# Orion-AI-Lab/KuroSiwo

Hardware: AMD Instinct MI355X
Metric: SAR tiles/sec (224x224, SNUNet-ECAM change-detection train step) (higher is better)
Workload: dtype bf16; 1 GPU; BASELINE.json configs[1]: SNUNet-ECAM CD, 2 dates x 2-ch GRD 224x224, per-GPU batch 32, ce+dice loss, Adam lr 1e-3, fwd+loss+bwd+optimizer; global_batch=32, base_channel=32, parallelism=dp1, hip_streams=3

## Files before the change

include/ksmi.h:

```cpp
#ifndef KSMI_H
#define KSMI_H
#include <stddef.h>
#include <stdint.h>

#ifdef __cplusplus
extern "C" {
#endif

#define KSMI_ABI_VERSION 8
#define KSMI_F32 0
#define KSMI_BF16 1
#define KSMI_E_ARG (-1)
#define KSMI_E_UNSUPPORTED (-2)
#define KSMI_MAX_SRC 6
#define KSMI_MAX_CHUNKS 72

int ksmi_abi_version(void);
const char* ksmi_last_error(void);
int ksmi_set_knob(const char* name, const char* value);
int ksmi_chunk_elems(int dtype);

#define KSMI_OP_CALL 0
#define KSMI_OP_ORDER 1
#define KSMI_OP_WAIT_SIDE 2
// ... 80 lines not shown
  int64_t sK, sN, sD, sT;
  int32_t flip;
  int32_t k_off[KSMI_MAX_CHUNKS];
  int32_t k_len[KSMI_MAX_CHUNKS];
  int32_t use_tap_map;
  int32_t tap_map[16];
  int32_t uniform_kc, k_total;
} ksmi_pack_desc;
int ksmi_pack_weights(const ksmi_pack_desc* d, int dtype, void* stream);
int ksmi_pack_weights_batched(const ksmi_pack_desc* descs_device, int n, int dtype, void* stream);

typedef struct ksmi_wgrad_desc {
  ksmi_src src[KSMI_MAX_SRC];
  int32_t nsrc;
  const void* dy; int32_t dyC; int32_t dy_c_off;
  int32_t B, Hin, Win, Hout, Wout;
  int32_t KH, KW, stride, pad;
  int32_t TH, TW;
  int32_t N;
  int32_t nchunks;
  int32_t nsplit;
  float* partial;
  float* grad; int64_t gK, gN, gT; int32_t accumulate;
  int32_t k_off[KSMI_MAX_CHUNKS];
  int32_t k_len[KSMI_MAX_CHUNKS];
  uint16_t chunk_c0[KSMI_MAX_CHUNKS];
  uint8_t chunk_src[KSMI_MAX_CHUNKS];
  int32_t uniform_kc, k_total;
  int32_t in_sy, in_sx, in_oy, in_ox, in_H, in_W;
  int32_t pad_x_set, pad_x;
  int32_t use_tap_off;
  int32_t tap_off[16];
  float* bias_grad; int32_t bias_accumulate;
} ksmi_wgrad_desc;
size_t ksmi_conv_wgrad_workspace(const ksmi_wgrad_desc* d, int dtype);
int ksmi_conv_wgrad(const ksmi_wgrad_desc* d, int dtype, void* stream);
int ksmi_conv_wgrad_fuses_bias(const ksmi_wgrad_desc* d, int dtype);

int ksmi_conv_first_forward(const float* x_nchw, const float* w, const float* bias, void* out, float* stats,
                            int B, int Cin, int H, int W, int Cout, int dtype, void* stream);
int ksmi_conv_first_forward_raw(const float* x_nchw, const float* x_tail, int c_head, const float* w, const float* bias,
                                void* out, float* stats, int B, int Cin, int H, int W, int Cout, const float* mean,
                                const float* stdv, const float* clamp, int dtype, void* stream);
int ksmi_conv_first_stats_rows(int B, int H, int W);
int ksmi_im2col3x3(const float* x_nchw, void* out, int B, int Cin, int H, int W, int Kpad, int dtype, void* stream);
int ksmi_im2col3x3_raw(const float* x_nchw, const float* x_tail, int c_head, void* out, int B, int Cin, int H, int W,
                       int Kpad, const float* mean, const float* stdv, const float* clamp, int dtype, void* stream);
int ksmi_conv_first_wgrad(const float* x_nchw, const void* dy, float* dw, float* workspace, size_t ws_bytes,
                          int B, int Cin, int H, int W, int Cout, int accumulate, int dtype, void* stream);
size_t ksmi_conv_first_wgrad_workspace(int B, int Cin, int H, int W, int Cout);

int ksmi_bn_finalize(const float* partial, int rows, int Cpad, int C, double count,
                     const float* gamma, const float* beta, float* running_mean, float* running_var,
                     int64_t* num_batches_tracked, float momentum, float eps, int training,
                     float* mean, float* rstd, float* scale, float* shift, void* stream);
int ksmi_bn_add_relu(const void* z, const void* identity, const float* scale, const float* shift, void* out,
                     int64_t npix, int C, int dtype, void* stream);
int ksmi_bnrelu_bwd_reduce(const void* dout, const void* out, const void* z, const float* mean, const float* rstd,
                           float* partial, int rows, int64_t npix, int C, int dtype, void* stream);
int ksmi_reduce_rows(const float* partial, int rows, int K, int Cstride, int C, float* sums,
                     float* dgamma, float* dbeta, int accumulate, void* stream);
typedef struct ksmi_rowsum_desc {
  const float* partial;
  float* dst;
  int32_t rows, K, k, Cstride, C, accumulate;
  int32_t head, next;
} ksmi_rowsum_desc;
int ksmi_reduce_rows_batched(const ksmi_rowsum_desc* descs_device, int n, void* stream);
int ksmi_reduce_rows_batched_wide(const ksmi_rowsum_desc* descs_device, int n, int max_c, void* stream);
int ksmi_bnrelu_bwd_apply(void* dout_g, const void* out, const void* z, const float* mean, const float* rstd,
                          const float* gamma, const float* sums, void* dz, double count,
                          int64_t npix, int C, int dtype, void* stream);
int ksmi_bn_bwd_apply_gated(const void* g, const void* z, const float* mean, const float* rstd, const float* gamma, const float* sums,
                            void* dz, double count, int64_t npix, int C, int dtype, void* stream);
int ksmi_bn_bwd_apply_add(void* r_di, const void* g, const void* i, const float* mean, const float* rstd,
                          const float* gamma, const float* sums, float* partial, int rows, double count,
                          int64_t npix, int C, int dtype, void* stream);
int ksmi_bn_fused_supported(int C, int Cstride, int dtype);
int ksmi_bn_fused_max_rows(void);
int ksmi_bn_fin_add_relu(float* partial, int rows, int Cpad, int C, double count, const float* gamma, const float* beta,
                         float* running_mean, float* running_var, int64_t* num_batches_tracked, float momentum, float eps,
                         float* mean, float* rstd, float* scale, float* shift, const void* z, const void* identity, void* out,
                         void* pooled, int B, int H, int W, int dtype, void* stream);
int ksmi_bn_bwd_fin_apply_gated(float* partial, int rows, int Cstride, float* sums, float* dgamma, float* dbeta, int accumulate,
                                const void* g, const void* z, const float* mean, const float* rstd, const float* gamma, void* dz,
                                double count, int64_t npix, int C, int dtype, void* stream);
int ksmi_bnrelu_bwd_fin_apply(float* partial, int rows, int Cstride, float* sums, float* dgamma, float* dbeta, int accumulate,
                              void* dout_g, const void* out, const void* z, const float* mean, const float* rstd, const float* gamma,
                              void* dz, double count, int64_t npix, int C, int dtype, void* stream);
int ksmi_bn_bwd_fin_apply_add(float* partial, int rows, int Cstride, float* sums, float* dgamma, float* dbeta, int accumulate,
                              void* r_di, const void* g, const void* i, const float* mean, const float* rstd, const float* gamma,
                              float* bias_partial, int bias_rows, double count, int64_t npix, int C, int dtype, void* stream);
int ksmi_channel_sum(const void* x, float* partial, int rows, int64_t npix, int C, int dtype, void* stream);
int ksmi_colsum(const void* x, int64_t rows, int C, float* out, int accumulate, int dtype, void* stream);

int ksmi_maxpool2x2_forward(const void* x, void* y, int B, int H, int W, int C, int dtype, void* stream);
int ksmi_maxpool2x2_backward(const void* x, const void* dy, void* dx, int accumulate,
                             int B, int H, int W, int C, int dtype, void* stream);

int ksmi_ecam_pool(const void* const x[4], float* avg, float* mx, int32_t* argmax,
                   float* workspace, int B, int HW, int C, int dtype, void* stream);
size_t ksmi_ecam_pool_workspace(int B, int HW, int C);
int ksmi_ecam_mlp(const float* avg, const float* mx, const float* ca_fc1, const float* ca_fc2,
                  const float* ca1_fc1, const float* ca1_fc2, float* ca, float* ca1,
                  float* hidden , int B, int C, void* stream);
int ksmi_ecam_final_forward(const void* const x[4], const float* ca, const float* ca1, const float* wf,
                            const float* bias, float* logits, int B, int HW, int C, int ncls, int dtype, void* stream);
int ksmi_ecam_final_backward_reduce(const void* const x[4], const float* dlogits, const float* ca, const float* ca1,
                                    const float* wf, float* dca, float* dca1, float* dwf, float* dbias,
                                    float* workspace, int B, int HW, int C, int ncls, int dtype, void* stream);
size_t ksmi_ecam_bwd_workspace(int B, int HW, int C, int ncls);
int ksmi_ecam_mlp_backward(const float* avg, const float* mx, const float* hidden, const float* ca, const float* ca1,
                           const float* dca, const float* dca1, const float* ca_fc1, const float* ca_fc2,
                           const float* ca1_fc1, const float* ca1_fc2, float* davg, float* dmax,
                           float* g_ca_fc1, float* g_ca_fc2, float* g_ca1_fc1, float* g_ca1_fc2,
                           float* workspace, int B, int C, void* stream);
size_t ksmi_ecam_mlp_bwd_workspace(int B, int C);
int ksmi_ecam_final_backward_dx(void* const dx[4], const float* dlogits, const float* ca, const float* wf,
                                const float* davg, const float* dmax, const int32_t* argmax,
                                int B, int HW, int C, int ncls, int dtype, void* stream);

size_t ksmi_loss_workspace(int B, int HW);
int ksmi_ce_dice_forward(const float* logits, const int64_t* labels, const float* class_w, int with_dice,
                         float* out3, float* workspace, int B, int HW, int ignore_index, void* stream);
int ksmi_ce_dice_backward(const float* logits, const int64_t* labels, const float* class_w, int with_dice,
                          const float* workspace, const float* grad_scale ,
                          float* dlogits, int B, int HW, int ignore_index, void* stream);

#define KSMI_LOSS_DICE 1
#define KSMI_LOSS_LOVASZ 2
#define KSMI_LOSS_FOCAL 3
size_t ksmi_seg_loss_workspace(int kind, int B, int HW);
int ksmi_seg_loss_forward(int kind, const float* logits, const int64_t* labels, const float* class_w, float gamma, float* out3,
                          void* workspace, int B, int HW, int ignore_index, void* stream);
int ksmi_seg_loss_backward(int kind, const float* logits, const int64_t* labels, const float* class_w, float gamma,
                           const void* workspace, const float* grad_scale ,
                           float* dlogits, int B, int HW, int ignore_index, void* stream);

int ksmi_argmax_confusion(const float* logits, const int64_t* labels, int64_t* pred , int64_t* cm,
                          int B, int C, int HW, int ignore_index, void* stream);
int ksmi_argmax_confusion_grouped(const float* logits, const int64_t* labels, int64_t* pred , int64_t* cm ,
                                  const int32_t* slot_a, int64_t* cms_a, const int32_t* slot_b, int64_t* cms_b,
                                  int B, int C, int HW, int ignore_index, void* stream);

int ksmi_adam_step(float* p, const float* g, float* m, float* v, int64_t n, int64_t* step_count,
                   float lr, float beta1, float beta2, float eps, float weight_decay, float grad_scale, void* stream);
int ksmi_adamw_step(float* p, const float* g, float* m, float* v, int64_t n, int64_t* step_count,
                    float lr, float beta1, float beta2, float eps, float weight_decay, float grad_scale, void* stream);
int ksmi_adam_step_mirror(float* p, const float* g, float* m, float* v, int64_t n, int64_t* step_count,
                          float lr, float beta1, float beta2, float eps, float weight_decay, float grad_scale, int decoupled,
                          void* mirror_bf16, void* stream);
int ksmi_sgd_step(float* p, const float* g, float* mom, int64_t n, int64_t* step_count,
                  float lr, float momentum, float weight_decay, float grad_scale, void* stream);

int ksmi_layernorm_forward(const void* x, const float* gamma, const float* beta, void* y, float* mean, float* rstd,
                           int rows, int C, float eps, int dtype, void* stream);
int ksmi_layernorm_bwd_blocks(int rows);
int ksmi_layernorm_backward(const void* dy, const void* x, const float* mean, const float* rstd, const float* gamma,
                            void* dx, int accumulate, float* partial, int rows, int C, int dtype, void* stream);
int ksmi_gelu_forward(const void* x, void* y, int64_t n, int dtype, void* stream);
int ksmi_gelu_backward(const void* dy, const void* x, void* dx, int64_t n, int dtype, void* stream);
int ksmi_gelu_backward_drop(const void* dy, const void* x, void* dx, int64_t n, uint32_t thr, float inv_keep, uint32_t site,
                            const uint32_t* rng_state, int dtype, void* stream);
int ksmi_add(const void* a, const void* b, void* out, int64_t n, int dtype, void* stream);
int ksmi_relu_backward(const void* dy, const void* x, void* dx, int64_t n, int dtype, void* stream);
int ksmi_relu_forward(const void* x, void* y, int64_t n, int dtype, void* stream);
// ... 146 lines not shown
```

kurosiwo_amd/_lib.py:

```python
import ctypes as C
import os

_HERE = os.path.dirname(os.path.abspath(__file__))
LIB_PATH = os.path.join(_HERE, "libksmi.so")

KSMI_F32, KSMI_BF16 = 0, 1
LOSS_DICE, LOSS_LOVASZ, LOSS_FOCAL = 1, 2, 3
MAX_SRC, MAX_CHUNKS = 6, 72
ABI_VERSION = 8


class KsmiError(RuntimeError):
    pass


class Src(C.Structure):
    _fields_ = [("ptr", C.c_void_p), ("scale", C.c_void_p), ("shift", C.c_void_p),
                ("C", C.c_int32), ("c_off", C.c_int32), ("c_len", C.c_int32), ("relu", C.c_int32)]


class Dst(C.Structure):
    _fields_ = [("ptr", C.c_void_p), ("C", C.c_int32), ("c_off", C.c_int32), ("n_begin", C.c_int32),
                ("n_len", C.c_int32), ("accumulate", C.c_int32), ("pad_", C.c_int32)]

# ... 22 lines not shown
                ("nchunks", C.c_int32), ("taps", C.c_int32), ("N", C.c_int32), ("Npad", C.c_int32), ("n_mod", C.c_int32),
                ("sK", C.c_int64), ("sN", C.c_int64), ("sD", C.c_int64), ("sT", C.c_int64),
                ("flip", C.c_int32),
                ("k_off", C.c_int32 * MAX_CHUNKS), ("k_len", C.c_int32 * MAX_CHUNKS),
                ("use_tap_map", C.c_int32), ("tap_map", C.c_int32 * 16), ("uniform_kc", C.c_int32), ("k_total", C.c_int32)]


class TiffInfo(C.Structure):
    _fields_ = [(k, C.c_int32) for k in ("width", "height", "bands", "bits", "sample_format", "compression", "predictor", "tiled",
                                         "big_endian", "bigtiff", "has_geo", "has_nodata")] + [
        ("pixel_scale", C.c_double * 2), ("origin", C.c_double * 2), ("tie_pixel", C.c_double * 2), ("nodata", C.c_double)]


class RowsumDesc(C.Structure):
    _fields_ = [("partial", C.c_void_p), ("dst", C.c_void_p), ("rows", C.c_int32), ("K", C.c_int32), ("k", C.c_int32),
                ("Cstride", C.c_int32), ("C", C.c_int32), ("accumulate", C.c_int32), ("head", C.c_int32), ("next", C.c_int32)]


class WgradDesc(C.Structure):
    _fields_ = [("src", Src * MAX_SRC), ("nsrc", C.c_int32),
                ("dy", C.c_void_p), ("dyC", C.c_int32), ("dy_c_off", C.c_int32),
                ("B", C.c_int32), ("Hin", C.c_int32), ("Win", C.c_int32), ("Hout", C.c_int32), ("Wout", C.c_int32),
                ("KH", C.c_int32), ("KW", C.c_int32), ("stride", C.c_int32), ("pad", C.c_int32),
                ("TH", C.c_int32), ("TW", C.c_int32), ("N", C.c_int32), ("nchunks", C.c_int32), ("nsplit", C.c_int32),
                ("partial", C.c_void_p), ("grad", C.c_void_p),
                ("gK", C.c_int64), ("gN", C.c_int64), ("gT", C.c_int64), ("accumulate", C.c_int32),
                ("k_off", C.c_int32 * MAX_CHUNKS), ("k_len", C.c_int32 * MAX_CHUNKS),
                ("chunk_c0", C.c_uint16 * MAX_CHUNKS), ("chunk_src", C.c_uint8 * MAX_CHUNKS),
                ("uniform_kc", C.c_int32), ("k_total", C.c_int32),
                ("in_sy", C.c_int32), ("in_sx", C.c_int32), ("in_oy", C.c_int32), ("in_ox", C.c_int32), ("in_H", C.c_int32), ("in_W", C.c_int32),
                ("pad_x_set", C.c_int32), ("pad_x", C.c_int32), ("use_tap_off", C.c_int32), ("tap_off", C.c_int32 * 16),
                ("bias_grad", C.c_void_p), ("bias_accumulate", C.c_int32)]


class Op(C.Structure):
    _fields_ = [(k, C.c_int32) for k in ("kind", "sig", "lane", "side", "tag", "a", "b", "nargs")] + [("fn", C.c_void_p), ("args", C.c_void_p)]


OP_CALL, OP_ORDER, OP_WAIT_SIDE = 0, 1, 2

_vp, _i, _i64, _f, _d, _sz = C.c_void_p, C.c_int, C.c_int64, C.c_float, C.c_double, C.c_size_t
_P4 = C.c_void_p * 4

SIGNATURES = {
    "ksmi_abi_version": (_i, []),
    "ksmi_last_kernels": (_i, [C.c_char_p, _i]),
    "ksmi_hbm_probe": (_i, [_i, _vp, _vp, _vp, C.c_size_t, _vp, _vp]),
    "ksmi_last_error": (C.c_char_p, []),
    "ksmi_set_knob": (_i, [C.c_char_p, C.c_char_p]),
    "ksmi_thunk_id": (_i, [C.c_char_p]),
    "ksmi_runner_create": (_vp, []),
    "ksmi_runner_destroy": (_i, [_vp]),
    "ksmi_runner_set_streams": (_i, [_vp, _vp, _vp, _vp, _vp]),
    "ksmi_run_list": (_i, [_vp, _vp, _i, _i, _vp, C.POINTER(C.c_int32)]),
    "ksmi_runner_order": (_i, [_vp, _i, _i]),
    "ksmi_runner_fork_side": (_i, [_vp, _i, _i, C.POINTER(C.c_void_p)]),
    "ksmi_runner_mark_side": (_i, [_vp, _i, _i]),
    "ksmi_runner_wait_side": (_i, [_vp, _i, _i, _i]),
    "ksmi_runner_join": (_i, [_vp]),
    "ksmi_conv_dispatch_info": (_i, [C.POINTER(ConvDesc), _i, C.POINTER(C.c_int32)]),
    "ksmi_chunk_elems": (_i, [_i]),
    "ksmi_conv_grid_m": (_i, [C.POINTER(ConvDesc)]),
    "ksmi_conv_forward": (_i, [C.POINTER(ConvDesc), _i, _vp]),
    "ksmi_pack_weights": (_i, [C.POINTER(PackDesc), _i, _vp]),
    "ksmi_pack_weights_batched": (_i, [_vp, _i, _i, _vp]),
    "ksmi_conv_wgrad_workspace": (_sz, [C.POINTER(WgradDesc), _i]),
    "ksmi_conv_wgrad": (_i, [C.POINTER(WgradDesc), _i, _vp]),
    "ksmi_conv_wgrad_fuses_bias": (_i, [C.POINTER(WgradDesc), _i]),
    "ksmi_conv_stats_rows": (_i, [C.POINTER(ConvDesc), _i]),
    "ksmi_conv_gate_supported": (_i, [C.POINTER(ConvDesc), _i]),
    "ksmi_desc_size": (C.c_size_t, [_i]),
    "ksmi_conv_first_forward": (_i, [_vp, _vp, _vp, _vp, _vp, _i, _i, _i, _i, _i, _i, _vp]),
    "ksmi_conv_first_forward_raw": (_i, [_vp, _vp, _i, _vp, _vp, _vp, _vp, _i, _i, _i, _i, _i, _vp, _vp, _vp, _i, _vp]),
    "ksmi_conv_first_stats_rows": (_i, [_i, _i, _i]),
    "ksmi_im2col3x3": (_i, [_vp, _vp, _i, _i, _i, _i, _i, _i, _vp]),
    "ksmi_im2col3x3_raw": (_i, [_vp, _vp, _i, _vp, _i, _i, _i, _i, _i, _vp, _vp, _vp, _i, _vp]),
    "ksmi_conv_first_wgrad": (_i, [_vp, _vp, _vp, _vp, _sz, _i, _i, _i, _i, _i, _i, _i, _vp]),
    "ksmi_conv_first_wgrad_workspace": (_sz, [_i, _i, _i, _i, _i]),
    "ksmi_bn_finalize": (_i, [_vp, _i, _i, _i, _d, _vp, _vp, _vp, _vp, _vp, _f, _f, _i, _vp, _vp, _vp, _vp, _vp]),
    "ksmi_bn_add_relu": (_i, [_vp, _vp, _vp, _vp, _vp, _i64, _i, _i, _vp]),
    "ksmi_bn_fused_supported": (_i, [_i, _i, _i]),
    "ksmi_bn_fused_max_rows": (_i, []),
    "ksmi_bn_fin_add_relu": (_i, [_vp, _i, _i, _i, _d, _vp, _vp, _vp, _vp, _vp, _f, _f, _vp, _vp, _vp, _vp, _vp, _vp, _vp, _vp, _i, _i, _i, _i, _vp]),
    "ksmi_bn_bwd_fin_apply_gated": (_i, [_vp, _i, _i, _vp, _vp, _vp, _i, _vp, _vp, _vp, _vp, _vp, _vp, _d, _i64, _i, _i, _vp]),
    "ksmi_bnrelu_bwd_fin_apply": (_i, [_vp, _i, _i, _vp, _vp, _vp, _i, _vp, _vp, _vp, _vp, _vp, _vp, _vp, _d, _i64, _i, _i, _vp]),
    "ksmi_bn_bwd_fin_apply_add": (_i, [_vp, _i, _i, _vp, _vp, _vp, _i, _vp, _vp, _vp, _vp, _vp, _vp, _vp, _i, _d, _i64, _i, _i, _vp]),
    "ksmi_bnrelu_bwd_reduce": (_i, [_vp, _vp, _vp, _vp, _vp, _vp, _i, _i64, _i, _i, _vp]),
    "ksmi_reduce_rows": (_i, [_vp, _i, _i, _i, _i, _vp, _vp, _vp, _i, _vp]),
    "ksmi_reduce_rows_batched": (_i, [_vp, _i, _vp]),
    "ksmi_reduce_rows_batched_wide": (_i, [_vp, _i, _i, _vp]),
    "ksmi_bnrelu_bwd_apply": (_i, [_vp, _vp, _vp, _vp, _vp, _vp, _vp, _vp, _d, _i64, _i, _i, _vp]),
    "ksmi_bn_bwd_apply_gated": (_i, [_vp, _vp, _vp, _vp, _vp, _vp, _vp, _d, _i64, _i, _i, _vp]),
    "ksmi_bn_bwd_apply_add": (_i, [_vp, _vp, _vp, _vp, _vp, _vp, _vp, _vp, _i, _d, _i64, _i, _i, _vp]),
    "ksmi_channel_sum": (_i, [_vp, _vp, _i, _i64, _i, _i, _vp]),
    "ksmi_colsum": (_i, [_vp, _i64, _i, _vp, _i, _i, _vp]),
    "ksmi_gather_rows": (_i, [_vp, _vp, _i, _vp, _vp, _i, _i, _i, _i, _i, _i, _vp]),
    "ksmi_scatter_rows": (_i, [_vp, _vp, _vp, _i, _vp, _vp, _i, _i, _i, _i, _i, _vp]),
    "ksmi_batch_sum": (_i, [_vp, _vp, _i, _i64, _i, _i, _vp]),
    "ksmi_mse_workspace": (C.c_size_t, []),
    "ksmi_mse_loss": (_i, [_vp, _vp, _vp, _f, _vp, _vp, _vp, _i64, _i, _vp]),
    "ksmi_maxpool2x2_forward": (_i, [_vp, _vp, _i, _i, _i, _i, _i, _vp]),
    "ksmi_maxpool2x2_backward": (_i, [_vp, _vp, _vp, _i, _i, _i, _i, _i, _i, _vp]),
    "ksmi_ecam_pool": (_i, [_P4, _vp, _vp, _vp, _vp, _i, _i, _i, _i, _vp]),
    "ksmi_ecam_pool_workspace": (_sz, [_i, _i, _i]),
    "ksmi_ecam_mlp": (_i, [_vp, _vp, _vp, _vp, _vp, _vp, _vp, _vp, _vp, _i, _i, _vp]),
    "ksmi_ecam_final_forward": (_i, [_P4, _vp, _vp, _vp, _vp, _vp, _i, _i, _i, _i, _i, _vp]),
    "ksmi_ecam_final_backward_reduce": (_i, [_P4, _vp, _vp, _vp, _vp, _vp, _vp, _vp, _vp, _vp, _i, _i, _i, _i, _i, _vp]),
    "ksmi_ecam_bwd_workspace": (_sz, [_i, _i, _i, _i]),
    "ksmi_ecam_mlp_backward": (_i, [_vp] * 18 + [_i, _i, _vp]),
    "ksmi_ecam_mlp_bwd_workspace": (_sz, [_i, _i]),
    "ksmi_ecam_final_backward_dx": (_i, [_P4, _vp, _vp, _vp, _vp, _vp, _vp, _i, _i, _i, _i, _i, _vp]),
    "ksmi_loss_workspace": (_sz, [_i, _i]),
    "ksmi_ce_dice_forward": (_i, [_vp, _vp, _vp, _i, _vp, _vp, _i, _i, _i, _vp]),
    "ksmi_ce_dice_backward": (_i, [_vp, _vp, _vp, _i, _vp, _vp, _vp, _i, _i, _i, _vp]),
    "ksmi_seg_loss_workspace": (_sz, [_i, _i, _i]),
    "ksmi_seg_loss_forward": (_i, [_i, _vp, _vp, _vp, _f, _vp, _vp, _i, _i, _i, _vp]),
    "ksmi_seg_loss_backward": (_i, [_i, _vp, _vp, _vp, _f, _vp, _vp, _vp, _i, _i, _i, _vp]),
    "ksmi_argmax_confusion": (_i, [_vp, _vp, _vp, _vp, _i, _i, _i, _i, _vp]),
    "ksmi_argmax_confusion_grouped": (_i, [_vp, _vp, _vp, _vp, _vp, _vp, _vp, _vp, _i, _i, _i, _i, _vp]),
    "ksmi_adam_step": (_i, [_vp, _vp, _vp, _vp, _i64, _vp, _f, _f, _f, _f, _f, _f, _vp]),
    "ksmi_adamw_step": (_i, [_vp, _vp, _vp, _vp, _i64, _vp, _f, _f, _f, _f, _f, _f, _vp]),
    "ksmi_adam_step_mirror": (_i, [_vp, _vp, _vp, _vp, _i64, _vp, _f, _f, _f, _f, _f, _f, _i, _vp, _vp]),
    "ksmi_sgd_step": (_i, [_vp, _vp, _vp, _i64, _vp, _f, _f, _f, _f, _vp]),
    "ksmi_layernorm_forward": (_i, [_vp, _vp, _vp, _vp, _vp, _vp, _i, _i, _f, _i, _vp]),
    "ksmi_layernorm_bwd_blocks": (_i, [_i]),
    "ksmi_layernorm_backward": (_i, [_vp, _vp, _vp, _vp, _vp, _vp, _i, _vp, _i, _i, _i, _vp]),
    "ksmi_gelu_forward": (_i, [_vp, _vp, _i64, _i, _vp]),
    "ksmi_gelu_backward": (_i, [_vp, _vp, _vp, _i64, _i, _vp]),
    "ksmi_add": (_i, [_vp, _vp, _vp, _i64, _i, _vp]),
    "ksmi_relu_backward": (_i, [_vp, _vp, _vp, _i64, _i, _vp]),
    "ksmi_relu_forward": (_i, [_vp, _vp, _i64, _i, _vp]),
    "ksmi_sar_preprocess": (_i, [_vp, _vp, _vp, _vp, _i, _i, _i64, C.c_float, _vp]),
    "ksmi_augment_views": (_i, [_vp, _vp, _vp, _vp, _vp, _vp, _i, _i, _i, _i, _f, C.c_uint32, _f, _f, C.c_uint32, _f, _f, C.c_uint32, _i, _i, _i, _i, _vp, _vp]),
    "ksmi_augment_masks": (_i, [_vp, _vp, _vp, _vp, _vp, _i, _i, _i, _i, _vp]),
    "ksmi_dem_slope": (_i, [_vp, _vp, _i, _i, _i, _d, _f, _f, _i, _vp]),
    "ksmi_bmm_f32": (_i, [_vp, _vp, _vp, _vp, _i, _i, _i, _i, _i, C.POINTER(C.c_int64), C.POINTER(C.c_int64), C.POINTER(C.c_int64), C.c_float, _i, _vp]),
    "ksmi_softmax_rows_f32": (_i, [_vp, _vp, _i64, _i, C.c_float, _vp]),
    "ksmi_softmax_rows_backward_f32": (_i, [_vp, _vp, _vp, _i64, _i, C.c_float, _vp]),
    "ksmi_semantic_tokens_forward": (_i, [_vp, _vp, _vp, _vp, _vp, _i, _i, _i, _i, _i, _i, _vp]),
    "ksmi_semantic_tokens_backward": (_i, [_vp, _vp, _vp, _vp, _vp, _vp, _i, _i, _i, _i, _i, _i, _i, _vp]),
    "ksmi_token_cross_forward": (_i, [_vp, _vp, _vp, _vp, _vp, _vp, _vp, _i, _i, _i, _i, _i, _i, C.c_float, _i, _vp]),
    "ksmi_token_cross_bwd_workspace": (_sz, [_i, _i, _i]),
    "ksmi_token_cross_backward": (_i, [_vp, _vp, _vp, _vp, _vp, _vp, _vp, _vp, _vp, _vp, _vp, _i, _i, _vp, _i, _i, _i, _i, _i, _i, C.c_float, _i, _vp]),
    "ksmi_tiff_info_read": (_i, [C.c_char_p, C.POINTER(TiffInfo)]),
    "ksmi_tiff_read_f32": (_i, [C.c_char_p, _vp, _i64, C.POINTER(TiffInfo)]),
    "ksmi_tiff_read_native": (_i, [C.c_char_p, _vp, _i64, C.POINTER(TiffInfo)]),
    "ksmi_tile_batch_read": (_i, [C.POINTER(C.c_char_p), _i, _vp, _i, _i, _i]),
    "ksmi_tile_batch_read_bands": (_i, [C.POINTER(C.c_char_p), _i, _vp, _i, _i, _i, _i]),
    "ksmi_tiles_fill_nodata": (_i, [_vp, _i, _i, _i, _i]),
    "ksmi_cast_bf16": (_i, [_vp, _vp, _i64, _vp]),
    "ksmi_up_gemm_supported": (_i, [_i, _i, _i, _i, _i]),
    "ksmi_up_wgrad_supported": (_i, [_i, _i, _i, _i, _i]),
    "ksmi_up_pack_weight": (_i, [_vp, _vp, _i, _vp]),
    "ksmi_up_pack_weights_batched": (_i, [_vp, _vp, _vp, _i, _vp]),
    "ksmi_up_forward": (_i, [_vp, _vp, _vp, _vp, _i, _i, _i, _i, _vp]),
    "ksmi_up_dgrad": (_i, [_vp, _vp, _vp, _i, _i, _i, _i, _i, _vp]),
    "ksmi_up_wgrad_workspace": (C.c_size_t, [_i, _i, _i, _i]),
    "ksmi_up_wgrad": (_i, [_vp, _vp, _vp, _vp, _i, _i, _i, _i, _i, _vp]),
    "ksmi_gemm_nt": (_i, [_vp, _i, _vp, _i, _vp, _vp, _i, _vp, _i, _i, _i, _i, _vp]),
    "ksmi_gemm_nn": (_i, [_vp, _i, _vp, _i, _vp, _i, _i, _i, _i, _i, _vp]),
    "ksmi_im2col": (_i, [_vp, _vp] + [_i] * 11 + [_i, _i, _vp]),
    "ksmi_col2im": (_i, [_vp, _vp, _i] + [_i] * 11 + [_i, _vp]),
    "ksmi_im2col_tc": (_i, [_vp, _vp] + [_i] * 11 + [_i, _vp]),
    "ksmi_col2im_tc": (_i, [_vp, _vp, _i] + [_i] * 11 + [_i, _vp]),
    "ksmi_weight_to_tc": (_i, [_vp, _vp, _i, _i, _i, _i, _i, _vp]),
    "ksmi_grad_from_tc": (_i, [_vp, _vp, _i, _i, _i, _i, _i, _vp]),
# ... 108 lines not shown
```

kurosiwo_amd/csrc/bnfused.hip:

```cpp
#include <stdlib.h>
#include "common.h"
#include "../../include/ksmi.h"
#include "errors.h"

int ksmi_internal_fold_rows(float* partial, int rows, int K, int Cstride, int C, hipStream_t st);

namespace {

constexpr int kFat = 1024;
constexpr int kMaxC = 512;
constexpr int kMaxRows = 512;

__device__ __forceinline__ void block_rows_sum(const float* __restrict__ partial, int rows, int Cstride, int C, double* red, double* sums) {
  const int Cq = C >> 2, G = Cq * 2;
  const int lpc = kFat / G;
  const int t = threadIdx.x;
  const int g = t % G, rl = t / G;
  if (rl < lpc) {
    const int k = g / Cq, c4 = g - k * Cq;
    const float* p = partial + (size_t)k * Cstride + c4 * 4;
    double a0 = 0.0, a1 = 0.0, a2 = 0.0, a3 = 0.0;
#pragma unroll 4
    for (int r = rl; r < rows; r += lpc) {
      const f32x4 v = *(const f32x4*)(p + (size_t)r * 2 * Cstride);
// ... 20 lines not shown
  float* mean_o; float* rstd_o; float* scale_o; float* shift_o;
};

template <typename T, bool POOL>
__global__ __launch_bounds__(kFat) void bn_fin_add_relu_kernel(FinArgs f, const T* __restrict__ z, const T* __restrict__ idn, T* __restrict__ out,
                                                               T* __restrict__ pooled, int B, int H, int W) {
  constexpr int VEC = ElemTraits<T>::kVec;
  __shared__ double red[kFat * 4];
  __shared__ double sums[2 * kMaxC];
  __shared__ float s_scale[kMaxC], s_shift[kMaxC];
  const int C = f.C;
  block_rows_sum(f.partial, f.rows, f.Cstride, C, red, sums);
  for (int c = threadIdx.x; c < C; c += kFat) {
    const double mean = sums[c] / f.count;
    double var = sums[C + c] / f.count - mean * mean;
    if (var < 0.0) var = 0.0;
    const float rs = (float)(1.0 / sqrt(var + (double)f.eps));
    const float sc = f.gamma[c] * rs;
    const float sh = f.beta[c] - (float)mean * sc;
    s_scale[c] = sc; s_shift[c] = sh;
    if (blockIdx.x == 0) {
      f.mean_o[c] = (float)mean; f.rstd_o[c] = rs; f.scale_o[c] = sc; f.shift_o[c] = sh;
      const double unb = f.count > 1.0 ? var * f.count / (f.count - 1.0) : var;
      f.rmean[c] = (1.f - f.momentum) * f.rmean[c] + f.momentum * (float)mean;
      f.rvar[c] = (1.f - f.momentum) * f.rvar[c] + f.momentum * (float)unb;
    }
  }
  if (blockIdx.x == 0 && threadIdx.x == 0 && f.nbt) *f.nbt += 1;
  __syncthreads();
  const int CV = C / VEC;
  const int64_t stride = (int64_t)gridDim.x * kFat;
  if (!POOL) {
    const int64_t nvec = (int64_t)B * H * W * CV;
    for (int64_t v = (int64_t)blockIdx.x * kFat + threadIdx.x; v < nvec; v += 2 * stride) {
      const int64_t v1 = v + stride;
      const bool two = v1 < nvec;
      const u32x4 rz0 = *(const u32x4*)(z + v * VEC), ri0 = *(const u32x4*)(idn + v * VEC);
      const u32x4 rz1 = *(const u32x4*)(z + (two ? v1 : v) * VEC), ri1 = *(const u32x4*)(idn + (two ? v1 : v) * VEC);
      float a[VEC], b[VEC];
      int c = (int)(v % CV) * VEC;
      vec_unpack<T>(rz0, a); vec_unpack<T>(ri0, b);
#pragma unroll
      for (int j = 0; j < VEC; ++j) a[j] = fmaxf(a[j] * s_scale[c + j] + s_shift[c + j] + b[j], 0.f);
      *(u32x4*)(out + v * VEC) = vec_pack<T>(a);
      if (two) {
        c = (int)(v1 % CV) * VEC;
        vec_unpack<T>(rz1, a); vec_unpack<T>(ri1, b);
#pragma unroll
        for (int j = 0; j < VEC; ++j) a[j] = fmaxf(a[j] * s_scale[c + j] + s_shift[c + j] + b[j], 0.f);
        *(u32x4*)(out + v1 * VEC) = vec_pack<T>(a);
      }
    }
  } else {
    const int Ho = H / 2, Wo = W / 2;
    const int64_t n = (int64_t)B * Ho * Wo * CV;
    for (int64_t v = (int64_t)blockIdx.x * kFat + threadIdx.x; v < n; v += stride) {
      const int cv = (int)(v % CV); int64_t r = v / CV;
      const int ox = (int)(r % Wo); r /= Wo;
      const int oy = (int)(r % Ho); const int b = (int)(r / Ho);
      const int64_t base = (((int64_t)b * H + 2 * oy) * W + 2 * ox) * C + cv * VEC;
      const int64_t offs[4] = {base, base + C, base + (int64_t)W * C, base + (int64_t)W * C + C};
      u32x4 rz[4], ri[4];
#pragma unroll
      for (int q = 0; q < 4; ++q) { rz[q] = *(const u32x4*)(z + offs[q]); ri[q] = *(const u32x4*)(idn + offs[q]); }
      const int c = cv * VEC;
      float m[VEC];
#pragma unroll
      for (int q = 0; q < 4; ++q) {
        float a[VEC], bb[VEC];
        vec_unpack<T>(rz[q], a); vec_unpack<T>(ri[q], bb);
#pragma unroll
        for (int j = 0; j < VEC; ++j) a[j] = fmaxf(a[j] * s_scale[c + j] + s_shift[c + j] + bb[j], 0.f);
        const u32x4 pk = vec_pack<T>(a);
        *(u32x4*)(out + offs[q]) = pk;
        vec_unpack<T>(pk, a);
#pragma unroll
        for (int j = 0; j < VEC; ++j) m[j] = (q == 0 || a[j] > m[j]) ? a[j] : m[j];
      }
      *(u32x4*)(pooled + v * VEC) = vec_pack<T>(m);
    }
  }
}

struct BwdFinArgs {
  const float* partial; int rows, Cstride, C;
  float* sums_o; float* dgamma; float* dbeta; int accumulate;
  const float* mean; const float* rstd; const float* gamma;
};

__device__ __forceinline__ void bwd_finish(const BwdFinArgs& f, double* red, double* sums, float* s_sum, float* s_mean, float* s_rstd, float* s_gamma) {
  const int C = f.C;
  block_rows_sum(f.partial, f.rows, f.Cstride, C, red, sums);
  for (int v = threadIdx.x; v < 2 * C; v += kFat) {
    const float s = (float)sums[v];
    s_sum[v] = s;
    if (blockIdx.x == 0) {
      if (f.sums_o) f.sums_o[v] = s;
      const int k = v / C, c = v - k * C;
      float* tgt = k == 0 ? f.dbeta : f.dgamma;
      if (tgt) tgt[c] = f.accumulate ? tgt[c] + 1.f * s : 1.f * s;
    }
  }
  for (int c = threadIdx.x; c < C; c += kFat) { s_mean[c] = f.mean[c]; s_rstd[c] = f.rstd[c]; s_gamma[c] = f.gamma[c]; }
  __syncthreads();
}

template <typename T, int MODE>
__global__ __launch_bounds__(kFat) void bn_bwd_fin_apply_kernel(BwdFinArgs f, T* __restrict__ g, const T* __restrict__ outp, const T* __restrict__ z,
                                                                T* __restrict__ dz, float inv_n, int64_t nvec) {
  constexpr int VEC = ElemTraits<T>::kVec;
  __shared__ double red[kFat * 4];
  __shared__ double sums[2 * kMaxC];
  __shared__ float s_sum[2 * kMaxC], s_mean[kMaxC], s_rstd[kMaxC], s_gamma[kMaxC];
  bwd_finish(f, red, sums, s_sum, s_mean, s_rstd, s_gamma);
  const int C = f.C, CV = C / VEC;
  const int64_t stride = (int64_t)gridDim.x * kFat;
  for (int64_t v = (int64_t)blockIdx.x * kFat + threadIdx.x; v < nvec; v += 2 * stride) {
    const int64_t v1 = v + stride;
    const bool two = v1 < nvec;
    const int64_t w1 = two ? v1 : v;
    const u32x4 rg0 = *(const u32x4*)(g + v * VEC), rz0 = *(const u32x4*)(z + v * VEC);
    const u32x4 rg1 = *(const u32x4*)(g + w1 * VEC), rz1 = *(const u32x4*)(z + w1 * VEC);
    u32x4 ro0, ro1;
    if (MODE == 1) { ro0 = *(const u32x4*)(outp + v * VEC); ro1 = *(const u32x4*)(outp + w1 * VEC); }
#pragma unroll
    for (int u = 0; u < 2; ++u) {
      if (u == 1 && !two) break;
      const int64_t vv = u ? v1 : v;
      const int c = (int)(vv % CV) * VEC;
      float gg[VEC], zz[VEC], o[VEC];
      vec_unpack<T>(u ? rg1 : rg0, gg); vec_unpack<T>(u ? rz1 : rz0, zz);
      if (MODE == 1) vec_unpack<T>(u ? ro1 : ro0, o);
#pragma unroll
      for (int j = 0; j < VEC; ++j) {
        if (MODE == 1) gg[j] = o[j] > 0.f ? gg[j] : 0.f;
        const float zh = (zz[j] - s_mean[c + j]) * s_rstd[c + j];
        zz[j] = s_gamma[c + j] * s_rstd[c + j] * (gg[j] - s_sum[c + j] * inv_n - zh * s_sum[C + c + j] * inv_n);
      }
      if (MODE == 1) *(u32x4*)(g + vv * VEC) = vec_pack<T>(gg);
      *(u32x4*)(dz + vv * VEC) = vec_pack<T>(zz);
    }
  }
}

template <typename T>
__global__ __launch_bounds__(kFat) void bn_bwd_fin_apply_add_kernel(BwdFinArgs f, T* __restrict__ r, const T* __restrict__ g, const T* __restrict__ iv,
                                                                    float* __restrict__ bias_partial, float inv_n, int64_t npix) {
  constexpr int VEC = ElemTraits<T>::kVec;
  __shared__ double red[kFat * 4];
  __shared__ double sums[2 * kMaxC];
  __shared__ float s_sum[2 * kMaxC], s_mean[kMaxC], s_rstd[kMaxC], s_gamma[kMaxC];
  bwd_finish(f, red, sums, s_sum, s_mean, s_rstd, s_gamma);
  const int C = f.C, CV = C / VEC;
  const int npl = kFat / CV;
  const int cv = threadIdx.x % CV, pl = threadIdx.x / CV;
  const bool active = pl < npl;
  float acc[VEC];
#pragma unroll
  for (int j = 0; j < VEC; ++j) acc[j] = 0.f;
  if (active) {
    float mu[VEC], rs[VEC], k0[VEC], k1[VEC], gr[VEC];
#pragma unroll
    for (int j = 0; j < VEC; ++j) {
      const int c = cv * VEC + j;
      mu[j] = s_mean[c]; rs[j] = s_rstd[c]; gr[j] = s_gamma[c] * s_rstd[c];
      k0[j] = s_sum[c] * inv_n; k1[j] = s_sum[C + c] * inv_n;
    }
    const int64_t per = (npix + gridDim.x - 1) / gridDim.x;
    const int64_t p0 = per * blockIdx.x, p1 = p0 + per < npix ? p0 + per : npix;
    for (int64_t p = p0 + pl; p < p1; p += 2 * npl) {
      const bool two = p + npl < p1;
      const int64_t offs[2] = {p * C + cv * VEC, two ? (p + npl) * C + cv * VEC : p * C + cv * VEC};
      u32x4 raw[2][3];
#pragma unroll
      for (int u = 0; u < 2; ++u) {
        raw[u][0] = *(const u32x4*)(r + offs[u]); raw[u][1] = *(const u32x4*)(g + offs[u]); raw[u][2] = *(const u32x4*)(iv + offs[u]);
      }
#pragma unroll
      for (int u = 0; u < 2; ++u) {
        if (u == 1 && !two) break;
        float rr[VEC], gg[VEC], ii[VEC];
        vec_unpack<T>(raw[u][0], rr); vec_unpack<T>(raw[u][1], gg); vec_unpack<T>(raw[u][2], ii);
#pragma unroll
        for (int j = 0; j < VEC; ++j) {
          const float xh = (ii[j] - mu[j]) * rs[j];
          rr[j] = gg[j] + gr[j] * (rr[j] - k0[j] - xh * k1[j]);
        }
        const u32x4 pk = vec_pack<T>(rr);
        *(u32x4*)(r + offs[u]) = pk;
        vec_unpack<T>(pk, rr);
#pragma unroll
        for (int j = 0; j < VEC; ++j) acc[j] += rr[j];
      }
    }
  }
  float* fred = (float*)red;
  __syncthreads();
#pragma unroll
  for (int j = 0; j < VEC; ++j) fred[(size_t)threadIdx.x * VEC + j] = active ? acc[j] : 0.f;
  __syncthreads();
  for (int c = threadIdx.x; c < C; c += kFat) {
    const int cvv = c / VEC, j = c - cvv * VEC;
    float s = 0.f;
    for (int l = 0; l < npl; ++l) s += fred[((size_t)l * CV + cvv) * VEC + j];
    bias_partial[(size_t)blockIdx.x * C + c] = s;
  }
}

bool fused_ok(int C, int dtype, int Cstride) {
  if (dtype != KSMI_BF16 && dtype != KSMI_F32) return false;
  const int vec = dtype == KSMI_BF16 ? 8 : 4;
  return C >= vec && C % vec == 0 && C % 4 == 0 && C <= kMaxC && Cstride >= C && Cstride % 4 == 0 && C / vec <= 256;
}

int fat_grid(int64_t work_items) {
  static const int cap = ksmi_knob_int("KSMI_BN_FAT_GRID", 256);
  int64_t b = (work_items + kFat - 1) / kFat;
  return (int)(b < 1 ? 1 : (b > cap ? cap : b));
}

}

extern "C" {

int ksmi_bn_fused_supported(int C, int Cstride, int dtype) { return fused_ok(C, dtype, Cstride) ? 1 : 0; }
int ksmi_bn_fused_max_rows(void) { return 256; }

int ksmi_bn_fin_add_relu(float* partial, int rows, int Cpad, int C, double count, const float* gamma, const float* beta,
                         float* running_mean, float* running_var, int64_t* num_batches_tracked, float momentum, float eps,
                         float* mean, float* rstd, float* scale, float* shift, const void* z, const void* identity, void* out,
                         void* pooled, int B, int H, int W, int dtype, void* stream) {
  if (!fused_ok(C, dtype, Cpad) || !partial || rows < 1 || B < 1 || H < 1 || W < 1) return ksmi_fail(KSMI_E_ARG, "bn_fin_add_relu: bad args");
  if (pooled && ((H & 1) || (W & 1))) return ksmi_fail(KSMI_E_ARG, "bn_fin_add_relu: pooling needs even H, W");
  if (rows > kMaxRows) rows = ksmi_internal_fold_rows(partial, rows, 2, Cpad, C, (hipStream_t)stream);
  FinArgs f{partial, rows, Cpad, C, count, gamma, beta, running_mean, running_var, num_batches_tracked, momentum, eps, mean, rstd, scale, shift};
  const int vec = dtype == KSMI_BF16 ? 8 : 4;
  const int64_t items = pooled ? (int64_t)B * (H / 2) * (W / 2) * (C / vec) : ((int64_t)B * H * W * (C / vec) + 1) / 2;
  const dim3 grid(fat_grid(items));
#define KSMI_FAR(TT, PP) hipLaunchKernelGGL((bn_fin_add_relu_kernel<TT, PP>), grid, dim3(kFat), 0, (hipStream_t)stream, f, (const TT*)z, \
                                            (const TT*)identity, (TT*)out, (TT*)pooled, B, H, W)
  if (dtype == KSMI_BF16) { if (pooled) KSMI_FAR(bf16_t, true); else KSMI_FAR(bf16_t, false); }
  else { if (pooled) KSMI_FAR(float, true); else KSMI_FAR(float, false); }
#undef KSMI_FAR
  return ksmi_check_launch("bn_fin_add_relu");
}

static int bwd_apply(int mode, float* partial, int rows, int Cstride, float* sums, float* dgamma, float* dbeta, int accumulate,
                     void* g, const void* outp, const void* z, const float* mean, const float* rstd, const float* gamma, void* dz,
                     double count, int64_t npix, int C, int dtype, void* stream, const char* what) {
  if (!fused_ok(C, dtype, Cstride) || !partial || rows < 1 || npix < 1) return ksmi_fail(KSMI_E_ARG, what);
  if (rows > kMaxRows) rows = ksmi_internal_fold_rows(partial, rows, 2, Cstride, C, (hipStream_t)stream);
  BwdFinArgs f{partial, rows, Cstride, C, sums, dgamma, dbeta, accumulate, mean, rstd, gamma};
  const int vec = dtype == KSMI_BF16 ? 8 : 4;
  const int64_t nvec = npix * C / vec;
  const float inv_n = (float)(1.0 / count);
  const dim3 grid(fat_grid((nvec + 1) / 2));
#define KSMI_BFA(TT, MM) hipLaunchKernelGGL((bn_bwd_fin_apply_kernel<TT, MM>), grid, dim3(kFat), 0, (hipStream_t)stream, f, (TT*)g, \
                                            (const TT*)outp, (const TT*)z, (TT*)dz, inv_n, nvec)
  if (dtype == KSMI_BF16) { if (mode) KSMI_BFA(bf16_t, 1); else KSMI_BFA(bf16_t, 0); }
  else { if (mode) KSMI_BFA(float, 1); else KSMI_BFA(float, 0); }
#undef KSMI_BFA
  return ksmi_check_launch(what);
}

int ksmi_bn_bwd_fin_apply_gated(float* partial, int rows, int Cstride, float* sums, float* dgamma, float* dbeta, int accumulate,
                                const void* g, const void* z, const float* mean, const float* rstd, const float* gamma, void* dz,
                                double count, int64_t npix, int C, int dtype, void* stream) {
  return bwd_apply(0, partial, rows, Cstride, sums, dgamma, dbeta, accumulate, (void*)g, nullptr, z, mean, rstd, gamma, dz, count, npix, C,
                   dtype, stream, "bn_bwd_fin_apply_gated");
}

int ksmi_bnrelu_bwd_fin_apply(float* partial, int rows, int Cstride, float* sums, float* dgamma, float* dbeta, int accumulate,
                              void* dout_g, const void* out, const void* z, const float* mean, const float* rstd, const float* gamma,
                              void* dz, double count, int64_t npix, int C, int dtype, void* stream) {
  return bwd_apply(1, partial, rows, Cstride, sums, dgamma, dbeta, accumulate, dout_g, out, z, mean, rstd, gamma, dz, count, npix, C, dtype,
                   stream, "bnrelu_bwd_fin_apply");
}

int ksmi_bn_bwd_fin_apply_add(float* partial, int rows, int Cstride, float* sums, float* dgamma, float* dbeta, int accumulate,
                              void* r_di, const void* g, const void* i, const float* mean, const float* rstd, const float* gamma,
                              float* bias_partial, int bias_rows, double count, int64_t npix, int C, int dtype, void* stream) {
  if (!fused_ok(C, dtype, Cstride) || !partial || rows < 1 || npix < 1 || bias_rows < 1 || bias_rows > 256 || !bias_partial)
    return ksmi_fail(KSMI_E_ARG, "bn_bwd_fin_apply_add: bad args");
  if (rows > kMaxRows) rows = ksmi_internal_fold_rows(partial, rows, 2, Cstride, C, (hipStream_t)stream);
  BwdFinArgs f{partial, rows, Cstride, C, sums, dgamma, dbeta, accumulate, mean, rstd, gamma};
  const float inv_n = (float)(1.0 / count);
  if (dtype == KSMI_BF16)
    hipLaunchKernelGGL(bn_bwd_fin_apply_add_kernel<bf16_t>, dim3(bias_rows), dim3(kFat), 0, (hipStream_t)stream, f, (bf16_t*)r_di,
                       (const bf16_t*)g, (const bf16_t*)i, bias_partial, inv_n, npix);
  else
    hipLaunchKernelGGL(bn_bwd_fin_apply_add_kernel<float>, dim3(bias_rows), dim3(kFat), 0, (hipStream_t)stream, f, (float*)r_di,
                       (const float*)g, (const float*)i, bias_partial, inv_n, npix);
  return ksmi_check_launch("bn_bwd_fin_apply_add");
}

}
```

kurosiwo_amd/csrc/thunks_gen.h:

```cpp
#pragma once
#include <stddef.h>
#include <stdint.h>
#include <string.h>

typedef int (*ksmi_thunk_fn)(const void* fn, const uint64_t* a, void* stream);
static inline float ksmi_slot_f32(uint64_t v) { uint32_t w = (uint32_t)v; float f; memcpy(&f, &w, 4); return f; }
static inline double ksmi_slot_f64(uint64_t v) { double d; memcpy(&d, &v, 8); return d; }

static int ksmi_thunk_0(const void* fn, const uint64_t* a, void* st) {
  typedef int (*F)(int, void*, void*, void*, float, void*, void*, int, int, int, void*);
  (void)a; return ((F)fn)((int)(int64_t)a[0], (void*)(uintptr_t)a[1], (void*)(uintptr_t)a[2], (void*)(uintptr_t)a[3], ksmi_slot_f32(a[4]), (void*)(uintptr_t)a[5], (void*)(uintptr_t)a[6], (int)(int64_t)a[7], (int)(int64_t)a[8], (int)(int64_t)a[9], st);
}
static int ksmi_thunk_1(const void* fn, const uint64_t* a, void* st) {
  typedef int (*F)(int, void*, void*, void*, float, void*, void*, void*, int, int, int, void*);
  (void)a; return ((F)fn)((int)(int64_t)a[0], (void*)(uintptr_t)a[1], (void*)(uintptr_t)a[2], (void*)(uintptr_t)a[3], ksmi_slot_f32(a[4]), (void*)(uintptr_t)a[5], (void*)(uintptr_t)a[6], (void*)(uintptr_t)a[7], (int)(int64_t)a[8], (int)(int64_t)a[9], (int)(int64_t)a[10], st);
}
static int ksmi_thunk_2(const void* fn, const uint64_t* a, void* st) {
  typedef int (*F)(int, void*, void*, void*, size_t, void*, void*);
  (void)a; return ((F)fn)((int)(int64_t)a[0], (void*)(uintptr_t)a[1], (void*)(uintptr_t)a[2], (void*)(uintptr_t)a[3], (size_t)a[4], (void*)(uintptr_t)a[5], st);
}
static int ksmi_thunk_3(const void* fn, const uint64_t* a, void* st) {
  typedef int (*F)(void*, void*);
  (void)a; return ((F)fn)((void*)(uintptr_t)a[0], st);
}
static int ksmi_thunk_4(const void* fn, const uint64_t* a, void* st) {
  typedef int (*F)(void*, int, void*);
  (void)a; return ((F)fn)((void*)(uintptr_t)a[0], (int)(int64_t)a[1], st);
}
static int ksmi_thunk_5(const void* fn, const uint64_t* a, void* st) {
  typedef int (*F)(void*, int, int, void*);
  (void)a; return ((F)fn)((void*)(uintptr_t)a[0], (int)(int64_t)a[1], (int)(int64_t)a[2], st);
}
static int ksmi_thunk_6(const void* fn, const uint64_t* a, void* st) {
  typedef int (*F)(void*, int, int, int, double, void*, void*, void*, void*, void*, float, float, int, void*, void*, void*, void*, void*);
  (void)a; return ((F)fn)((void*)(uintptr_t)a[0], (int)(int64_t)a[1], (int)(int64_t)a[2], (int)(int64_t)a[3], ksmi_slot_f64(a[4]), (void*)(uintptr_t)a[5], (void*)(uintptr_t)a[6], (void*)(uintptr_t)a[7], (void*)(uintptr_t)a[8], (void*)(uintptr_t)a[9], ksmi_slot_f32(a[10]), ksmi_slot_f32(a[11]), (int)(int64_t)a[12], (void*)(uintptr_t)a[13], (void*)(uintptr_t)a[14], (void*)(uintptr_t)a[15], (void*)(uintptr_t)a[16], st);
}
static int ksmi_thunk_7(const void* fn, const uint64_t* a, void* st) {
  typedef int (*F)(void*, int, int, int, double, void*, void*, void*, void*, void*, float, float, void*, void*, void*, void*, void*, void*, void*, void*, int, int, int, int, void*);
  (void)a; return ((F)fn)((void*)(uintptr_t)a[0], (int)(int64_t)a[1], (int)(int64_t)a[2], (int)(int64_t)a[3], ksmi_slot_f64(a[4]), (void*)(uintptr_t)a[5], (void*)(uintptr_t)a[6], (void*)(uintptr_t)a[7], (void*)(uintptr_t)a[8], (void*)(uintptr_t)a[9], ksmi_slot_f32(a[10]), ksmi_slot_f32(a[11]), (void*)(uintptr_t)a[12], (void*)(uintptr_t)a[13], (void*)(uintptr_t)a[14], (void*)(uintptr_t)a[15], (void*)(uintptr_t)a[16], (void*)(uintptr_t)a[17], (void*)(uintptr_t)a[18], (void*)(uintptr_t)a[19], (int)(int64_t)a[20], (int)(int64_t)a[21], (int)(int64_t)a[22], (int)(int64_t)a[23], st);
}
static int ksmi_thunk_8(const void* fn, const uint64_t* a, void* st) {
  typedef int (*F)(void*, int, int, int, int, void*, void*, void*, int, void*);
  (void)a; return ((F)fn)((void*)(uintptr_t)a[0], (int)(int64_t)a[1], (int)(int64_t)a[2], (int)(int64_t)a[3], (int)(int64_t)a[4], (void*)(uintptr_t)a[5], (void*)(uintptr_t)a[6], (void*)(uintptr_t)a[7], (int)(int64_t)a[8], st);
}
static int ksmi_thunk_9(const void* fn, const uint64_t* a, void* st) {
  typedef int (*F)(void*, int, int, int, int, void*, void*, void*, int, float, void*);
  (void)a; return ((F)fn)((void*)(uintptr_t)a[0], (int)(int64_t)a[1], (int)(int64_t)a[2], (int)(int64_t)a[3], (int)(int64_t)a[4], (void*)(uintptr_t)a[5], (void*)(uintptr_t)a[6], (void*)(uintptr_t)a[7], (int)(int64_t)a[8], ksmi_slot_f32(a[9]), st);
}
static int ksmi_thunk_10(const void* fn, const uint64_t* a, void* st) {
  typedef int (*F)(void*, int, int, void*, void*, void*, int, void*, void*, void*, void*, void*, void*, double, long long, int, int, void*);
  (void)a; return ((F)fn)((void*)(uintptr_t)a[0], (int)(int64_t)a[1], (int)(int64_t)a[2], (void*)(uintptr_t)a[3], (void*)(uintptr_t)a[4], (void*)(uintptr_t)a[5], (int)(int64_t)a[6], (void*)(uintptr_t)a[7], (void*)(uintptr_t)a[8], (void*)(uintptr_t)a[9], (void*)(uintptr_t)a[10], (void*)(uintptr_t)a[11], (void*)(uintptr_t)a[12], ksmi_slot_f64(a[13]), (long long)a[14], (int)(int64_t)a[15], (int)(int64_t)a[16], st);
}
static int ksmi_thunk_11(const void* fn, const uint64_t* a, void* st) {
  typedef int (*F)(void*, int, int, void*, void*, void*, int, void*, void*, void*, void*, void*, void*, void*, double, long long, int, int, void*);
  (void)a; return ((F)fn)((void*)(uintptr_t)a[0], (int)(int64_t)a[1], (int)(int64_t)a[2], (void*)(uintptr_t)a[3], (void*)(uintptr_t)a[4], (void*)(uintptr_t)a[5], (int)(int64_t)a[6], (void*)(uintptr_t)a[7], (void*)(uintptr_t)a[8], (void*)(uintptr_t)a[9], (void*)(uintptr_t)a[10], (void*)(uintptr_t)a[11], (void*)(uintptr_t)a[12], (void*)(uintptr_t)a[13], ksmi_slot_f64(a[14]), (long long)a[15], (int)(int64_t)a[16], (int)(int64_t)a[17], st);
}
static int ksmi_thunk_12(const void* fn, const uint64_t* a, void* st) {
  typedef int (*F)(void*, int, int, void*, void*, void*, int, void*, void*, void*, void*, void*, void*, void*, int, double, long long, int, int, void*);
  (void)a; return ((F)fn)((void*)(uintptr_t)a[0], (int)(int64_t)a[1], (int)(int64_t)a[2], (void*)(uintptr_t)a[3], (void*)(uintptr_t)a[4], (void*)(uintptr_t)a[5], (int)(int64_t)a[6], (void*)(uintptr_t)a[7], (void*)(uintptr_t)a[8], (void*)(uintptr_t)a[9], (void*)(uintptr_t)a[10], (void*)(uintptr_t)a[11], (void*)(uintptr_t)a[12], (void*)(uintptr_t)a[13], (int)(int64_t)a[14], ksmi_slot_f64(a[15]), (long long)a[16], (int)(int64_t)a[17], (int)(int64_t)a[18], st);
}
static int ksmi_thunk_13(const void* fn, const uint64_t* a, void* st) {
  typedef int (*F)(void*, int, void*, int, void*, int, int, int, int, int, void*);
  (void)a; return ((F)fn)((void*)(uintptr_t)a[0], (int)(int64_t)a[1], (void*)(uintptr_t)a[2], (int)(int64_t)a[3], (void*)(uintptr_t)a[4], (int)(int64_t)a[5], (int)(int64_t)a[6], (int)(int64_t)a[7], (int)(int64_t)a[8], (int)(int64_t)a[9], st);
}
static int ksmi_thunk_14(const void* fn, const uint64_t* a, void* st) {
  typedef int (*F)(void*, int, void*, int, void*, void*, int, void*, int, int, int, int, void*);
  (void)a; return ((F)fn)((void*)(uintptr_t)a[0], (int)(int64_t)a[1], (void*)(uintptr_t)a[2], (int)(int64_t)a[3], (void*)(uintptr_t)a[4], (void*)(uintptr_t)a[5], (int)(int64_t)a[6], (void*)(uintptr_t)a[7], (int)(int64_t)a[8], (int)(int64_t)a[9], (int)(int64_t)a[10], (int)(int64_t)a[11], st);
}
static int ksmi_thunk_15(const void* fn, const uint64_t* a, void* st) {
  typedef int (*F)(void*, long long, int, void*, int, int, void*);
  (void)a; return ((F)fn)((void*)(uintptr_t)a[0], (long long)a[1], (int)(int64_t)a[2], (void*)(uintptr_t)a[3], (int)(int64_t)a[4], (int)(int64_t)a[5], st);
}
static int ksmi_thunk_16(const void* fn, const uint64_t* a, void* st) {
  typedef int (*F)(void*, void*, void*);
  (void)a; return ((F)fn)((void*)(uintptr_t)a[0], (void*)(uintptr_t)a[1], st);
}
static int ksmi_thunk_17(const void* fn, const uint64_t* a, void* st) {
  typedef int (*F)(void*, void*, int, void*);
  (void)a; return ((F)fn)((void*)(uintptr_t)a[0], (void*)(uintptr_t)a[1], (int)(int64_t)a[2], st);
}
static int ksmi_thunk_18(const void* fn, const uint64_t* a, void* st) {
  typedef int (*F)(void*, void*, int, int, int, double, float, float, int, void*);
  (void)a; return ((F)fn)((void*)(uintptr_t)a[0], (void*)(uintptr_t)a[1], (int)(int64_t)a[2], (int)(int64_t)a[3], (int)(int64_t)a[4], ksmi_slot_f64(a[5]), ksmi_slot_f32(a[6]), ksmi_slot_f32(a[7]), (int)(int64_t)a[8], st);
}
static int ksmi_thunk_19(const void* fn, const uint64_t* a, void* st) {
  typedef int (*F)(void*, void*, int, int, int, int, void*);
  (void)a; return ((F)fn)((void*)(uintptr_t)a[0], (void*)(uintptr_t)a[1], (int)(int64_t)a[2], (int)(int64_t)a[3], (int)(int64_t)a[4], (int)(int64_t)a[5], st);
}
static int ksmi_thunk_20(const void* fn, const uint64_t* a, void* st) {
  typedef int (*F)(void*, void*, int, int, int, int, int, void*);
  (void)a; return ((F)fn)((void*)(uintptr_t)a[0], (void*)(uintptr_t)a[1], (int)(int64_t)a[2], (int)(int64_t)a[3], (int)(int64_t)a[4], (int)(int64_t)a[5], (int)(int64_t)a[6], st);
}
static int ksmi_thunk_21(const void* fn, const uint64_t* a, void* st) {
  typedef int (*F)(void*, void*, int, int, int, int, int, int, void*);
  (void)a; return ((F)fn)((void*)(uintptr_t)a[0], (void*)(uintptr_t)a[1], (int)(int64_t)a[2], (int)(int64_t)a[3], (int)(int64_t)a[4], (int)(int64_t)a[5], (int)(int64_t)a[6], (int)(int64_t)a[7], st);
}
static int ksmi_thunk_22(const void* fn, const uint64_t* a, void* st) {
  typedef int (*F)(void*, void*, int, int, int, int, int, int, int, int, void*);
  (void)a; return ((F)fn)((void*)(uintptr_t)a[0], (void*)(uintptr_t)a[1], (int)(int64_t)a[2], (int)(int64_t)a[3], (int)(int64_t)a[4], (int)(int64_t)a[5], (int)(int64_t)a[6], (int)(int64_t)a[7], (int)(int64_t)a[8], (int)(int64_t)a[9], st);
}
static int ksmi_thunk_23(const void* fn, const uint64_t* a, void* st) {
  typedef int (*F)(void*, void*, int, int, int, int, int, int, int, int, int, int, int, int, void*);
  (void)a; return ((F)fn)((void*)(uintptr_t)a[0], (void*)(uintptr_t)a[1], (int)(int64_t)a[2], (int)(int64_t)a[3], (int)(int64_t)a[4], (int)(int64_t)a[5], (int)(int64_t)a[6], (int)(int64_t)a[7], (int)(int64_t)a[8], (int)(int64_t)a[9], (int)(int64_t)a[10], (int)(int64_t)a[11], (int)(int64_t)a[12], (int)(int64_t)a[13], st);
}
static int ksmi_thunk_24(const void* fn, const uint64_t* a, void* st) {
  typedef int (*F)(void*, void*, int, int, int, int, int, int, int, int, int, int, int, int, int, void*);
  (void)a; return ((F)fn)((void*)(uintptr_t)a[0], (void*)(uintptr_t)a[1], (int)(int64_t)a[2], (int)(int64_t)a[3], (int)(int64_t)a[4], (int)(int64_t)a[5], (int)(int64_t)a[6], (int)(int64_t)a[7], (int)(int64_t)a[8], (int)(int64_t)a[9], (int)(int64_t)a[10], (int)(int64_t)a[11], (int)(int64_t)a[12], (int)(int64_t)a[13], (int)(int64_t)a[14], st);
}
static int ksmi_thunk_25(const void* fn, const uint64_t* a, void* st) {
  typedef int (*F)(void*, void*, int, int, int, long long, int, void*);
  (void)a; return ((F)fn)((void*)(uintptr_t)a[0], (void*)(uintptr_t)a[1], (int)(int64_t)a[2], (int)(int64_t)a[3], (int)(int64_t)a[4], (long long)a[5], (int)(int64_t)a[6], st);
}
static int ksmi_thunk_26(const void* fn, const uint64_t* a, void* st) {
  typedef int (*F)(void*, void*, int, int, int, long long, int, int, void*);
  (void)a; return ((F)fn)((void*)(uintptr_t)a[0], (void*)(uintptr_t)a[1], (int)(int64_t)a[2], (int)(int64_t)a[3], (int)(int64_t)a[4], (long long)a[5], (int)(int64_t)a[6], (int)(int64_t)a[7], st);
}
static int ksmi_thunk_27(const void* fn, const uint64_t* a, void* st) {
  typedef int (*F)(void*, void*, int, long long, int, int, void*);
  (void)a; return ((F)fn)((void*)(uintptr_t)a[0], (void*)(uintptr_t)a[1], (int)(int64_t)a[2], (long long)a[3], (int)(int64_t)a[4], (int)(int64_t)a[5], st);
}
static int ksmi_thunk_28(const void* fn, const uint64_t* a, void* st) {
  typedef int (*F)(void*, void*, int, void*, int, int, int, int, int, void*, void*, void*, int, void*);
  (void)a; return ((F)fn)((void*)(uintptr_t)a[0], (void*)(uintptr_t)a[1], (int)(int64_t)a[2], (void*)(uintptr_t)a[3], (int)(int64_t)a[4], (int)(int64_t)a[5], (int)(int64_t)a[6], (int)(int64_t)a[7], (int)(int64_t)a[8], (void*)(uintptr_t)a[9], (void*)(uintptr_t)a[10], (void*)(uintptr_t)a[11], (int)(int64_t)a[12], st);
}
static int ksmi_thunk_29(const void* fn, const uint64_t* a, void* st) {
  typedef int (*F)(void*, void*, int, void*, void*, int, int, int, int, int, int, void*);
  (void)a; return ((F)fn)((void*)(uintptr_t)a[0], (void*)(uintptr_t)a[1], (int)(int64_t)a[2], (void*)(uintptr_t)a[3], (void*)(uintptr_t)a[4], (int)(int64_t)a[5], (int)(int64_t)a[6], (int)(int64_t)a[7], (int)(int64_t)a[8], (int)(int64_t)a[9], (int)(int64_t)a[10], st);
}
static int ksmi_thunk_30(const void* fn, const uint64_t* a, void* st) {
  typedef int (*F)(void*, void*, int, void*, void*, void*, void*, int, int, int, int, int, void*, void*, void*, int, void*);
  (void)a; return ((F)fn)((void*)(uintptr_t)a[0], (void*)(uintptr_t)a[1], (int)(int64_t)a[2], (void*)(uintptr_t)a[3], (void*)(uintptr_t)a[4], (void*)(uintptr_t)a[5], (void*)(uintptr_t)a[6], (int)(int64_t)a[7], (int)(int64_t)a[8], (int)(int64_t)a[9], (int)(int64_t)a[10], (int)(int64_t)a[11], (void*)(uintptr_t)a[12], (void*)(uintptr_t)a[13], (void*)(uintptr_t)a[14], (int)(int64_t)a[15], st);
}
static int ksmi_thunk_31(const void* fn, const uint64_t* a, void* st) {
  typedef int (*F)(void*, void*, long long, void*);
  (void)a; return ((F)fn)((void*)(uintptr_t)a[0], (void*)(uintptr_t)a[1], (long long)a[2], st);
}
static int ksmi_thunk_32(const void* fn, const uint64_t* a, void* st) {
  typedef int (*F)(void*, void*, long long, int, void*);
  (void)a; return ((F)fn)((void*)(uintptr_t)a[0], (void*)(uintptr_t)a[1], (long long)a[2], (int)(int64_t)a[3], st);
}
static int ksmi_thunk_33(const void* fn, const uint64_t* a, void* st) {
  typedef int (*F)(void*, void*, long long, int, float, void*);
  (void)a; return ((F)fn)((void*)(uintptr_t)a[0], (void*)(uintptr_t)a[1], (long long)a[2], (int)(int64_t)a[3], ksmi_slot_f32(a[4]), st);
}
static int ksmi_thunk_34(const void* fn, const uint64_t* a, void* st) {
  typedef int (*F)(void*, void*, void*, float, void*, void*, void*, long long, int, void*);
  (void)a; return ((F)fn)((void*)(uintptr_t)a[0], (void*)(uintptr_t)a[1], (void*)(uintptr_t)a[2], ksmi_slot_f32(a[3]), (void*)(uintptr_t)a[4], (void*)(uintptr_t)a[5], (void*)(uintptr_t)a[6], (long long)a[7], (int)(int64_t)a[8], st);
}
static int ksmi_thunk_35(const void* fn, const uint64_t* a, void* st) {
  typedef int (*F)(void*, void*, void*, int, void*);
  (void)a; return ((F)fn)((void*)(uintptr_t)a[0], (void*)(uintptr_t)a[1], (void*)(uintptr_t)a[2], (int)(int64_t)a[3], st);
}
static int ksmi_thunk_36(const void* fn, const uint64_t* a, void* st) {
  typedef int (*F)(void*, void*, void*, int, int, int, int, float, int, void*);
  (void)a; return ((F)fn)((void*)(uintptr_t)a[0], (void*)(uintptr_t)a[1], (void*)(uintptr_t)a[2], (int)(int64_t)a[3], (int)(int64_t)a[4], (int)(int64_t)a[5], (int)(int64_t)a[6], ksmi_slot_f32(a[7]), (int)(int64_t)a[8], st);
}
static int ksmi_thunk_37(const void* fn, const uint64_t* a, void* st) {
  typedef int (*F)(void*, void*, void*, int, int, int, int, int, void*);
  (void)a; return ((F)fn)((void*)(uintptr_t)a[0], (void*)(uintptr_t)a[1], (void*)(uintptr_t)a[2], (int)(int64_t)a[3], (int)(int64_t)a[4], (int)(int64_t)a[5], (int)(int64_t)a[6], (int)(int64_t)a[7], st);
}
static int ksmi_thunk_38(const void* fn, const uint64_t* a, void* st) {
  typedef int (*F)(void*, void*, void*, int, int, int, int, int, float, int, void*);
  (void)a; return ((F)fn)((void*)(uintptr_t)a[0], (void*)(uintptr_t)a[1], (void*)(uintptr_t)a[2], (int)(int64_t)a[3], (int)(int64_t)a[4], (int)(int64_t)a[5], (int)(int64_t)a[6], (int)(int64_t)a[7], ksmi_slot_f32(a[8]), (int)(int64_t)a[9], st);
}
static int ksmi_thunk_39(const void* fn, const uint64_t* a, void* st) {
  typedef int (*F)(void*, void*, void*, int, int, int, int, int, float, unsigned int, float, unsigned int, void*, int, void*);
  (void)a; return ((F)fn)((void*)(uintptr_t)a[0], (void*)(uintptr_t)a[1], (void*)(uintptr_t)a[2], (int)(int64_t)a[3], (int)(int64_t)a[4], (int)(int64_t)a[5], (int)(int64_t)a[6], (int)(int64_t)a[7], ksmi_slot_f32(a[8]), (unsigned int)a[9], ksmi_slot_f32(a[10]), (unsigned int)a[11], (void*)(uintptr_t)a[12], (int)(int64_t)a[13], st);
}
static int ksmi_thunk_40(const void* fn, const uint64_t* a, void* st) {
  typedef int (*F)(void*, void*, void*, int, int, int, int, int, int, void*);
  (void)a; return ((F)fn)((void*)(uintptr_t)a[0], (void*)(uintptr_t)a[1], (void*)(uintptr_t)a[2], (int)(int64_t)a[3], (int)(int64_t)a[4], (int)(int64_t)a[5], (int)(int64_t)a[6], (int)(int64_t)a[7], (int)(int64_t)a[8], st);
}
static int ksmi_thunk_41(const void* fn, const uint64_t* a, void* st) {
  typedef int (*F)(void*, void*, void*, int, int, int, int, int, int, int, void*);
  (void)a; return ((F)fn)((void*)(uintptr_t)a[0], (void*)(uintptr_t)a[1], (void*)(uintptr_t)a[2], (int)(int64_t)a[3], (int)(int64_t)a[4], (int)(int64_t)a[5], (int)(int64_t)a[6], (int)(int64_t)a[7], (int)(int64_t)a[8], (int)(int64_t)a[9], st);
}
static int ksmi_thunk_42(const void* fn, const uint64_t* a, void* st) {
  typedef int (*F)(void*, void*, void*, int, int, int, long long, int, int, void*);
  (void)a; return ((F)fn)((void*)(uintptr_t)a[0], (void*)(uintptr_t)a[1], (void*)(uintptr_t)a[2], (int)(int64_t)a[3], (int)(int64_t)a[4], (int)(int64_t)a[5], (long long)a[6], (int)(int64_t)a[7], (int)(int64_t)a[8], st);
}
static int ksmi_thunk_43(const void* fn, const uint64_t* a, void* st) {
  typedef int (*F)(void*, void*, void*, int, void*, void*, int, int, int, void*);
  (void)a; return ((F)fn)((void*)(uintptr_t)a[0], (void*)(uintptr_t)a[1], (void*)(uintptr_t)a[2], (int)(int64_t)a[3], (void*)(uintptr_t)a[4], (void*)(uintptr_t)a[5], (int)(int64_t)a[6], (int)(int64_t)a[7], (int)(int64_t)a[8], st);
}
static int ksmi_thunk_44(const void* fn, const uint64_t* a, void* st) {
  typedef int (*F)(void*, void*, void*, int, void*, void*, int, int, int, int, int, void*);
  (void)a; return ((F)fn)((void*)(uintptr_t)a[0], (void*)(uintptr_t)a[1], (void*)(uintptr_t)a[2], (int)(int64_t)a[3], (void*)(uintptr_t)a[4], (void*)(uintptr_t)a[5], (int)(int64_t)a[6], (int)(int64_t)a[7], (int)(int64_t)a[8], (int)(int64_t)a[9], (int)(int64_t)a[10], st);
}
static int ksmi_thunk_45(const void* fn, const uint64_t* a, void* st) {
  typedef int (*F)(void*, void*, void*, int, void*, void*, void*, int, int, int, void*);
  (void)a; return ((F)fn)((void*)(uintptr_t)a[0], (void*)(uintptr_t)a[1], (void*)(uintptr_t)a[2], (int)(int64_t)a[3], (void*)(uintptr_t)a[4], (void*)(uintptr_t)a[5], (void*)(uintptr_t)a[6], (int)(int64_t)a[7], (int)(int64_t)a[8], (int)(int64_t)a[9], st);
}
static int ksmi_thunk_46(const void* fn, const uint64_t* a, void* st) {
  typedef int (*F)(void*, void*, void*, long long, int, void*);
  (void)a; return ((F)fn)((void*)(uintptr_t)a[0], (void*)(uintptr_t)a[1], (void*)(uintptr_t)a[2], (long long)a[3], (int)(int64_t)a[4], st);
}
static int ksmi_thunk_47(const void* fn, const uint64_t* a, void* st) {
  typedef int (*F)(void*, void*, void*, long long, int, float, void*);
  (void)a; return ((F)fn)((void*)(uintptr_t)a[0], (void*)(uintptr_t)a[1], (void*)(uintptr_t)a[2], (long long)a[3], (int)(int64_t)a[4], ksmi_slot_f32(a[5]), st);
}
static int ksmi_thunk_48(const void* fn, const uint64_t* a, void* st) {
  typedef int (*F)(void*, void*, void*, long long, int, int, unsigned int, float, unsigned int, unsigned int, float, unsigned int, void*, int, void*);
  (void)a; return ((F)fn)((void*)(uintptr_t)a[0], (void*)(uintptr_t)a[1], (void*)(uintptr_t)a[2], (long long)a[3], (int)(int64_t)a[4], (int)(int64_t)a[5], (unsigned int)a[6], ksmi_slot_f32(a[7]), (unsigned int)a[8], (unsigned int)a[9], ksmi_slot_f32(a[10]), (unsigned int)a[11], (void*)(uintptr_t)a[12], (int)(int64_t)a[13], st);
}
static int ksmi_thunk_49(const void* fn, const uint64_t* a, void* st) {
  typedef int (*F)(void*, void*, void*, long long, void*, float, float, float, float, void*);
  (void)a; return ((F)fn)((void*)(uintptr_t)a[0], (void*)(uintptr_t)a[1], (void*)(uintptr_t)a[2], (long long)a[3], (void*)(uintptr_t)a[4], ksmi_slot_f32(a[5]), ksmi_slot_f32(a[6]), ksmi_slot_f32(a[7]), ksmi_slot_f32(a[8]), st);
}
static int ksmi_thunk_50(const void* fn, const uint64_t* a, void* st) {
  typedef int (*F)(void*, void*, void*, long long, unsigned int, float, unsigned int, void*, int, void*);
  (void)a; return ((F)fn)((void*)(uintptr_t)a[0], (void*)(uintptr_t)a[1], (void*)(uintptr_t)a[2], (long long)a[3], (unsigned int)a[4], ksmi_slot_f32(a[5]), (unsigned int)a[6], (void*)(uintptr_t)a[7], (int)(int64_t)a[8], st);
}
static int ksmi_thunk_51(const void* fn, const uint64_t* a, void* st) {
  typedef int (*F)(void*, void*, void*, void*, int, int, int, int, void*);
  (void)a; return ((F)fn)((void*)(uintptr_t)a[0], (void*)(uintptr_t)a[1], (void*)(uintptr_t)a[2], (void*)(uintptr_t)a[3], (int)(int64_t)a[4], (int)(int64_t)a[5], (int)(int64_t)a[6], (int)(int64_t)a[7], st);
}
static int ksmi_thunk_52(const void* fn, const uint64_t* a, void* st) {
  typedef int (*F)(void*, void*, void*, void*, int, int, int, int, int, void*);
  (void)a; return ((F)fn)((void*)(uintptr_t)a[0], (void*)(uintptr_t)a[1], (void*)(uintptr_t)a[2], (void*)(uintptr_t)a[3], (int)(int64_t)a[4], (int)(int64_t)a[5], (int)(int64_t)a[6], (int)(int64_t)a[7], (int)(int64_t)a[8], st);
}
static int ksmi_thunk_53(const void* fn, const uint64_t* a, void* st) {
  typedef int (*F)(void*, void*, void*, void*, int, int, int, int, int, void*, void*, void*, float, int, void*);
  (void)a; return ((F)fn)((void*)(uintptr_t)a[0], (void*)(uintptr_t)a[1], (void*)(uintptr_t)a[2], (void*)(uintptr_t)a[3], (int)(int64_t)a[4], (int)(int64_t)a[5], (int)(int64_t)a[6], (int)(int64_t)a[7], (int)(int64_t)a[8], (void*)(uintptr_t)a[9], (void*)(uintptr_t)a[10], (void*)(uintptr_t)a[11], ksmi_slot_f32(a[12]), (int)(int64_t)a[13], st);
}
static int ksmi_thunk_54(const void* fn, const uint64_t* a, void* st) {
  typedef int (*F)(void*, void*, void*, void*, int, int, long long, float, void*);
  (void)a; return ((F)fn)((void*)(uintptr_t)a[0], (void*)(uintptr_t)a[1], (void*)(uintptr_t)a[2], (void*)(uintptr_t)a[3], (int)(int64_t)a[4], (int)(int64_t)a[5], (long long)a[6], ksmi_slot_f32(a[7]), st);
}
static int ksmi_thunk_55(const void* fn, const uint64_t* a, void* st) {
  typedef int (*F)(void*, void*, void*, void*, int, long long, int, unsigned int, float, unsigned int, void*, int, void*);
  (void)a; return ((F)fn)((void*)(uintptr_t)a[0], (void*)(uintptr_t)a[1], (void*)(uintptr_t)a[2], (void*)(uintptr_t)a[3], (int)(int64_t)a[4], (long long)a[5], (int)(int64_t)a[6], (unsigned int)a[7], ksmi_slot_f32(a[8]), (unsigned int)a[9], (void*)(uintptr_t)a[10], (int)(int64_t)a[11], st);
}
static int ksmi_thunk_56(const void* fn, const uint64_t* a, void* st) {
  typedef int (*F)(void*, void*, void*, void*, long long, int, int, float, int, void*);
  (void)a; return ((F)fn)((void*)(uintptr_t)a[0], (void*)(uintptr_t)a[1], (void*)(uintptr_t)a[2], (void*)(uintptr_t)a[3], (long long)a[4], (int)(int64_t)a[5], (int)(int64_t)a[6], ksmi_slot_f32(a[7]), (int)(int64_t)a[8], st);
}
static int ksmi_thunk_57(const void* fn, const uint64_t* a, void* st) {
  typedef int (*F)(void*, void*, void*, void*, long long, void*, float, float, float, float, float, float, void*);
  (void)a; return ((F)fn)((void*)(uintptr_t)a[0], (void*)(uintptr_t)a[1], (void*)(uintptr_t)a[2], (void*)(uintptr_t)a[3], (long long)a[4], (void*)(uintptr_t)a[5], ksmi_slot_f32(a[6]), ksmi_slot_f32(a[7]), ksmi_slot_f32(a[8]), ksmi_slot_f32(a[9]), ksmi_slot_f32(a[10]), ksmi_slot_f32(a[11]), st);
}
static int ksmi_thunk_58(const void* fn, const uint64_t* a, void* st) {
  typedef int (*F)(void*, void*, void*, void*, long long, void*, float, float, float, float, float, float, int, void*, void*);
  (void)a; return ((F)fn)((void*)(uintptr_t)a[0], (void*)(uintptr_t)a[1], (void*)(uintptr_t)a[2], (void*)(uintptr_t)a[3], (long long)a[4], (void*)(uintptr_t)a[5], ksmi_slot_f32(a[6]), ksmi_slot_f32(a[7]), ksmi_slot_f32(a[8]), ksmi_slot_f32(a[9]), ksmi_slot_f32(a[10]), ksmi_slot_f32(a[11]), (int)(int64_t)a[12], (void*)(uintptr_t)a[13], st);
}
static int ksmi_thunk_59(const void* fn, const uint64_t* a, void* st) {
  typedef int (*F)(void*, void*, void*, void*, void*, int, int, int, int, void*);
  (void)a; return ((F)fn)((void*)(uintptr_t)a[0], (void*)(uintptr_t)a[1], (void*)(uintptr_t)a[2], (void*)(uintptr_t)a[3], (void*)(uintptr_t)a[4], (int)(int64_t)a[5], (int)(int64_t)a[6], (int)(int64_t)a[7], (int)(int64_t)a[8], st);
}
static int ksmi_thunk_60(const void* fn, const uint64_t* a, void* st) {
  typedef int (*F)(void*, void*, void*, void*, void*, int, int, int, int, int, void*);
  (void)a; return ((F)fn)((void*)(uintptr_t)a[0], (void*)(uintptr_t)a[1], (void*)(uintptr_t)a[2], (void*)(uintptr_t)a[3], (void*)(uintptr_t)a[4], (int)(int64_t)a[5], (int)(int64_t)a[6], (int)(int64_t)a[7], (int)(int64_t)a[8], (int)(int64_t)a[9], st);
}
static int ksmi_thunk_61(const void* fn, const uint64_t* a, void* st) {
  typedef int (*F)(void*, void*, void*, void*, void*, int, int, int, int, int, int, void*);
  (void)a; return ((F)fn)((void*)(uintptr_t)a[0], (void*)(uintptr_t)a[1], (void*)(uintptr_t)a[2], (void*)(uintptr_t)a[3], (void*)(uintptr_t)a[4], (int)(int64_t)a[5], (int)(int64_t)a[6], (int)(int64_t)a[7], (int)(int64_t)a[8], (int)(int64_t)a[9], (int)(int64_t)a[10], st);
}
static int ksmi_thunk_62(const void* fn, const uint64_t* a, void* st) {
  typedef int (*F)(void*, void*, void*, void*, void*, int, int, int, int, unsigned int, float, unsigned int, void*, int, void*);
  (void)a; return ((F)fn)((void*)(uintptr_t)a[0], (void*)(uintptr_t)a[1], (void*)(uintptr_t)a[2], (void*)(uintptr_t)a[3], (void*)(uintptr_t)a[4], (int)(int64_t)a[5], (int)(int64_t)a[6], (int)(int64_t)a[7], (int)(int64_t)a[8], (unsigned int)a[9], ksmi_slot_f32(a[10]), (unsigned int)a[11], (void*)(uintptr_t)a[12], (int)(int64_t)a[13], st);
}
static int ksmi_thunk_63(const void* fn, const uint64_t* a, void* st) {
  typedef int (*F)(void*, void*, void*, void*, void*, int, int, long long, int, void*);
  (void)a; return ((F)fn)((void*)(uintptr_t)a[0], (void*)(uintptr_t)a[1], (void*)(uintptr_t)a[2], (void*)(uintptr_t)a[3], (void*)(uintptr_t)a[4], (int)(int64_t)a[5], (int)(int64_t)a[6], (long long)a[7], (int)(int64_t)a[8], st);
}
static int ksmi_thunk_64(const void* fn, const uint64_t* a, void* st) {
  typedef int (*F)(void*, void*, void*, void*, void*, int, long long, int, int, void*);
  (void)a; return ((F)fn)((void*)(uintptr_t)a[0], (void*)(uintptr_t)a[1], (void*)(uintptr_t)a[2], (void*)(uintptr_t)a[3], (void*)(uintptr_t)a[4], (int)(int64_t)a[5], (long long)a[6], (int)(int64_t)a[7], (int)(int64_t)a[8], st);
}
static int ksmi_thunk_65(const void* fn, const uint64_t* a, void* st) {
  typedef int (*F)(void*, void*, void*, void*, void*, long long, int, int, void*);
  (void)a; return ((F)fn)((void*)(uintptr_t)a[0], (void*)(uintptr_t)a[1], (void*)(uintptr_t)a[2], (void*)(uintptr_t)a[3], (void*)(uintptr_t)a[4], (long long)a[5], (int)(int64_t)a[6], (int)(int64_t)a[7], st);
}
static int ksmi_thunk_66(const void* fn, const uint64_t* a, void* st) {
  typedef int (*F)(void*, void*, void*, void*, void*, void*, int, int, float, int, void*);
  (void)a; return ((F)fn)((void*)(uintptr_t)a[0], (void*)(uintptr_t)a[1], (void*)(uintptr_t)a[2], (void*)(uintptr_t)a[3], (void*)(uintptr_t)a[4], (void*)(uintptr_t)a[5], (int)(int64_t)a[6], (int)(int64_t)a[7], ksmi_slot_f32(a[8]), (int)(int64_t)a[9], st);
}
static int ksmi_thunk_67(const void* fn, const uint64_t* a, void* st) {
  typedef int (*F)(void*, void*, void*, void*, void*, void*, int, int, int, int, float, int, void*);
  (void)a; return ((F)fn)((void*)(uintptr_t)a[0], (void*)(uintptr_t)a[1], (void*)(uintptr_t)a[2], (void*)(uintptr_t)a[3], (void*)(uintptr_t)a[4], (void*)(uintptr_t)a[5], (int)(int64_t)a[6], (int)(int64_t)a[7], (int)(int64_t)a[8], (int)(int64_t)a[9], ksmi_slot_f32(a[10]), (int)(int64_t)a[11], st);
}
static int ksmi_thunk_68(const void* fn, const uint64_t* a, void* st) {
  typedef int (*F)(void*, void*, void*, void*, void*, void*, int, int, int, int, float, unsigned int, float, float, unsigned int, float, float, unsigned int, int, int, int, int, void*, void*);
  (void)a; return ((F)fn)((void*)(uintptr_t)a[0], (void*)(uintptr_t)a[1], (void*)(uintptr_t)a[2], (void*)(uintptr_t)a[3], (void*)(uintptr_t)a[4], (void*)(uintptr_t)a[5], (int)(int64_t)a[6], (int)(int64_t)a[7], (int)(int64_t)a[8], (int)(int64_t)a[9], ksmi_slot_f32(a[10]), (unsigned int)a[11], ksmi_slot_f32(a[12]), ksmi_slot_f32(a[13]), (unsigned int)a[14], ksmi_slot_f32(a[15]), ksmi_slot_f32(a[16]), (unsigned int)a[17], (int)(int64_t)a[18], (int)(int64_t)a[19], (int)(int64_t)a[20], (int)(int64_t)a[21], (void*)(uintptr_t)a[22], st);
}
static int ksmi_thunk_69(const void* fn, const uint64_t* a, void* st) {
  typedef int (*F)(void*, void*, void*, void*, void*, void*, int, int, int, int, int, void*);
  (void)a; return ((F)fn)((void*)(uintptr_t)a[0], (void*)(uintptr_t)a[1], (void*)(uintptr_t)a[2], (void*)(uintptr_t)a[3], (void*)(uintptr_t)a[4], (void*)(uintptr_t)a[5], (int)(int64_t)a[6], (int)(int64_t)a[7], (int)(int64_t)a[8], (int)(int64_t)a[9], (int)(int64_t)a[10], st);
}
static int ksmi_thunk_70(const void* fn, const uint64_t* a, void* st) {
  typedef int (*F)(void*, void*, void*, void*, void*, void*, int, int, int, int, int, int, int, void*);
  (void)a; return ((F)fn)((void*)(uintptr_t)a[0], (void*)(uintptr_t)a[1], (void*)(uintptr_t)a[2], (void*)(uintptr_t)a[3], (void*)(uintptr_t)a[4], (void*)(uintptr_t)a[5], (int)(int64_t)a[6], (int)(int64_t)a[7], (int)(int64_t)a[8], (int)(int64_t)a[9], (int)(int64_t)a[10], (int)(int64_t)a[11], (int)(int64_t)a[12], st);
}
static int ksmi_thunk_71(const void* fn, const uint64_t* a, void* st) {
  typedef int (*F)(void*, void*, void*, void*, void*, void*, int, long long, int, int, void*);
  (void)a; return ((F)fn)((void*)(uintptr_t)a[0], (void*)(uintptr_t)a[1], (void*)(uintptr_t)a[2], (void*)(uintptr_t)a[3], (void*)(uintptr_t)a[4], (void*)(uintptr_t)a[5], (int)(int64_t)a[6], (long long)a[7], (int)(int64_t)a[8], (int)(int64_t)a[9], st);
}
static int ksmi_thunk_72(const void* fn, const uint64_t* a, void* st) {
  typedef int (*F)(void*, void*, void*, void*, void*, void*, int, void*, int, int, int, void*);
  (void)a; return ((F)fn)((void*)(uintptr_t)a[0], (void*)(uintptr_t)a[1], (void*)(uintptr_t)a[2], (void*)(uintptr_t)a[3], (void*)(uintptr_t)a[4], (void*)(uintptr_t)a[5], (int)(int64_t)a[6], (void*)(uintptr_t)a[7], (int)(int64_t)a[8], (int)(int64_t)a[9], (int)(int64_t)a[10], st);
}
static int ksmi_thunk_73(const void* fn, const uint64_t* a, void* st) {
  typedef int (*F)(void*, void*, void*, void*, void*, void*, void*, double, long long, int, int, void*);
  (void)a; return ((F)fn)((void*)(uintptr_t)a[0], (void*)(uintptr_t)a[1], (void*)(uintptr_t)a[2], (void*)(uintptr_t)a[3], (void*)(uintptr_t)a[4], (void*)(uintptr_t)a[5], (void*)(uintptr_t)a[6], ksmi_slot_f64(a[7]), (long long)a[8], (int)(int64_t)a[9], (int)(int64_t)a[10], st);
}
static int ksmi_thunk_74(const void* fn, const uint64_t* a, void* st) {
  typedef int (*F)(void*, void*, void*, void*, void*, void*, void*, int, double, long long, int, int, void*);
  (void)a; return ((F)fn)((void*)(uintptr_t)a[0], (void*)(uintptr_t)a[1], (void*)(uintptr_t)a[2], (void*)(uintptr_t)a[3], (void*)(uintptr_t)a[4], (void*)(uintptr_t)a[5], (void*)(uintptr_t)a[6], (int)(int64_t)a[7], ksmi_slot_f64(a[8]), (long long)a[9], (int)(int64_t)a[10], (int)(int64_t)a[11], st);
}
static int ksmi_thunk_75(const void* fn, const uint64_t* a, void* st) {
  typedef int (*F)(void*, void*, void*, void*, void*, void*, void*, int, int, int, int, int, void*);
  (void)a; return ((F)fn)((void*)(uintptr_t)a[0], (void*)(uintptr_t)a[1], (void*)(uintptr_t)a[2], (void*)(uintptr_t)a[3], (void*)(uintptr_t)a[4], (void*)(uintptr_t)a[5], (void*)(uintptr_t)a[6], (int)(int64_t)a[7], (int)(int64_t)a[8], (int)(int64_t)a[9], (int)(int64_t)a[10], (int)(int64_t)a[11], st);
}
static int ksmi_thunk_76(const void* fn, const uint64_t* a, void* st) {
  typedef int (*F)(void*, void*, void*, void*, void*, void*, void*, int, int, int, int, int, float, int, void*);
  (void)a; return ((F)fn)((void*)(uintptr_t)a[0], (void*)(uintptr_t)a[1], (void*)(uintptr_t)a[2], (void*)(uintptr_t)a[3], (void*)(uintptr_t)a[4], (void*)(uintptr_t)a[5], (void*)(uintptr_t)a[6], (int)(int64_t)a[7], (int)(int64_t)a[8], (int)(int64_t)a[9], (int)(int64_t)a[10], (int)(int64_t)a[11], ksmi_slot_f32(a[12]), (int)(int64_t)a[13], st);
}
static int ksmi_thunk_77(const void* fn, const uint64_t* a, void* st) {
  typedef int (*F)(void*, void*, void*, void*, void*, void*, void*, int, int, int, int, int, float, unsigned int, float, unsigned int, void*, int, void*);
  (void)a; return ((F)fn)((void*)(uintptr_t)a[0], (void*)(uintptr_t)a[1], (void*)(uintptr_t)a[2], (void*)(uintptr_t)a[3], (void*)(uintptr_t)a[4], (void*)(uintptr_t)a[5], (void*)(uintptr_t)a[6], (int)(int64_t)a[7], (int)(int64_t)a[8], (int)(int64_t)a[9], (int)(int64_t)a[10], (int)(int64_t)a[11], ksmi_slot_f32(a[12]), (unsigned int)a[13], ksmi_slot_f32(a[14]), (unsigned int)a[15], (void*)(uintptr_t)a[16], (int)(int64_t)a[17], st);
}
static int ksmi_thunk_78(const void* fn, const uint64_t* a, void* st) {
  typedef int (*F)(void*, void*, void*, void*, void*, void*, void*, int, int, int, int, int, int, float, int, void*);
  (void)a; return ((F)fn)((void*)(uintptr_t)a[0], (void*)(uintptr_t)a[1], (void*)(uintptr_t)a[2], (void*)(uintptr_t)a[3], (void*)(uintptr_t)a[4], (void*)(uintptr_t)a[5], (void*)(uintptr_t)a[6], (int)(int64_t)a[7], (int)(int64_t)a[8], (int)(int64_t)a[9], (int)(int64_t)a[10], (int)(int64_t)a[11], (int)(int64_t)a[12], ksmi_slot_f32(a[13]), (int)(int64_t)a[14], st);
}
static int ksmi_thunk_79(const void* fn, const uint64_t* a, void* st) {
  typedef int (*F)(void*, void*, void*, void*, void*, void*, void*, void*, double, long long, int, float, int, void*);
  (void)a; return ((F)fn)((void*)(uintptr_t)a[0], (void*)(uintptr_t)a[1], (void*)(uintptr_t)a[2], (void*)(uintptr_t)a[3], (void*)(uintptr_t)a[4], (void*)(uintptr_t)a[5], (void*)(uintptr_t)a[6], (void*)(uintptr_t)a[7], ksmi_slot_f64(a[8]), (long long)a[9], (int)(int64_t)a[10], ksmi_slot_f32(a[11]), (int)(int64_t)a[12], st);
}
static int ksmi_thunk_80(const void* fn, const uint64_t* a, void* st) {
  typedef int (*F)(void*, void*, void*, void*, void*, void*, void*, void*, double, long long, int, int, void*);
  (void)a; return ((F)fn)((void*)(uintptr_t)a[0], (void*)(uintptr_t)a[1], (void*)(uintptr_t)a[2], (void*)(uintptr_t)a[3], (void*)(uintptr_t)a[4], (void*)(uintptr_t)a[5], (void*)(uintptr_t)a[6], (void*)(uintptr_t)a[7], ksmi_slot_f64(a[8]), (long long)a[9], (int)(int64_t)a[10], (int)(int64_t)a[11], st);
}
static int ksmi_thunk_81(const void* fn, const uint64_t* a, void* st) {
  typedef int (*F)(void*, void*, void*, void*, void*, void*, void*, void*, int, double, long long, int, int, void*);
  (void)a; return ((F)fn)((void*)(uintptr_t)a[0], (void*)(uintptr_t)a[1], (void*)(uintptr_t)a[2], (void*)(uintptr_t)a[3], (void*)(uintptr_t)a[4], (void*)(uintptr_t)a[5], (void*)(uintptr_t)a[6], (void*)(uintptr_t)a[7], (int)(int64_t)a[8], ksmi_slot_f64(a[9]), (long long)a[10], (int)(int64_t)a[11], (int)(int64_t)a[12], st);
}
static int ksmi_thunk_82(const void* fn, const uint64_t* a, void* st) {
  typedef int (*F)(void*, void*, void*, void*, void*, void*, void*, void*, int, int, int, int, void*);
  (void)a; return ((F)fn)((void*)(uintptr_t)a[0], (void*)(uintptr_t)a[1], (void*)(uintptr_t)a[2], (void*)(uintptr_t)a[3], (void*)(uintptr_t)a[4], (void*)(uintptr_t)a[5], (void*)(uintptr_t)a[6], (void*)(uintptr_t)a[7], (int)(int64_t)a[8], (int)(int64_t)a[9], (int)(int64_t)a[10], (int)(int64_t)a[11], st);
}
static int ksmi_thunk_83(const void* fn, const uint64_t* a, void* st) {
  typedef int (*F)(void*, void*, void*, void*, void*, void*, void*, void*, void*, int, int, void*);
  (void)a; return ((F)fn)((void*)(uintptr_t)a[0], (void*)(uintptr_t)a[1], (void*)(uintptr_t)a[2], (void*)(uintptr_t)a[3], (void*)(uintptr_t)a[4], (void*)(uintptr_t)a[5], (void*)(uintptr_t)a[6], (void*)(uintptr_t)a[7], (void*)(uintptr_t)a[8], (int)(int64_t)a[9], (int)(int64_t)a[10], st);
}
static int ksmi_thunk_84(const void* fn, const uint64_t* a, void* st) {
  typedef int (*F)(void*, void*, void*, void*, void*, void*, void*, void*, void*, void*, int, int, int, int, int, void*);
  (void)a; return ((F)fn)((void*)(uintptr_t)a[0], (void*)(uintptr_t)a[1], (void*)(uintptr_t)a[2], (void*)(uintptr_t)a[3], (void*)(uintptr_t)a[4], (void*)(uintptr_t)a[5], (void*)(uintptr_t)a[6], (void*)(uintptr_t)a[7], (void*)(uintptr_t)a[8], (void*)(uintptr_t)a[9], (int)(int64_t)a[10], (int)(int64_t)a[11], (int)(int64_t)a[12], (int)(int64_t)a[13], (int)(int64_t)a[14], st);
}
static int ksmi_thunk_85(const void* fn, const uint64_t* a, void* st) {
  typedef int (*F)(void*, void*, void*, void*, void*, void*, void*, void*, void*, void*, void*, int, int, void*, int, int, int, int, int, int, float, int, void*);
  (void)a; return ((F)fn)((void*)(uintptr_t)a[0], (void*)(uintptr_t)a[1], (void*)(uintptr_t)a[2], (void*)(uintptr_t)a[3], (void*)(uintptr_t)a[4], (void*)(uintptr_t)a[5], (void*)(uintptr_t)a[6], (void*)(uintptr_t)a[7], (void*)(uintptr_t)a[8], (void*)(uintptr_t)a[9], (void*)(uintptr_t)a[10], (int)(int64_t)a[11], (int)(int64_t)a[12], (void*)(uintptr_t)a[13], (int)(int64_t)a[14], (int)(int64_t)a[15], (int)(int64_t)a[16], (int)(int64_t)a[17], (int)(int64_t)a[18], (int)(int64_t)a[19], ksmi_slot_f32(a[20]), (int)(int64_t)a[21], st);
}
static int ksmi_thunk_86(const void* fn, const uint64_t* a, void* st) {
  typedef int (*F)(void*, void*, void*, void*, void*, void*, void*, void*, void*, void*, void*, void*, void*, void*, void*, void*, void*, void*, int, int, void*);
  (void)a; return ((F)fn)((void*)(uintptr_t)a[0], (void*)(uintptr_t)a[1], (void*)(uintptr_t)a[2], (void*)(uintptr_t)a[3], (void*)(uintptr_t)a[4], (void*)(uintptr_t)a[5], (void*)(uintptr_t)a[6], (void*)(uintptr_t)a[7], (void*)(uintptr_t)a[8], (void*)(uintptr_t)a[9], (void*)(uintptr_t)a[10], (void*)(uintptr_t)a[11], (void*)(uintptr_t)a[12], (void*)(uintptr_t)a[13], (void*)(uintptr_t)a[14], (void*)(uintptr_t)a[15], (void*)(uintptr_t)a[16], (void*)(uintptr_t)a[17], (int)(int64_t)a[18], (int)(int64_t)a[19], st);
}
static int ksmi_thunk_87(const void* fn, const uint64_t* a, void* st) {
  typedef int (*F)(void*, void*, void*, void*, size_t, int, int, int, int, int, int, int, void*);
  (void)a; return ((F)fn)((void*)(uintptr_t)a[0], (void*)(uintptr_t)a[1], (void*)(uintptr_t)a[2], (void*)(uintptr_t)a[3], (size_t)a[4], (int)(int64_t)a[5], (int)(int64_t)a[6], (int)(int64_t)a[7], (int)(int64_t)a[8], (int)(int64_t)a[9], (int)(int64_t)a[10], (int)(int64_t)a[11], st);
}
static int ksmi_thunk_88(const void* fn, const uint64_t* a, void* st) {
  typedef int (*F)(void*, size_t, void*);
  (void)a; return ((F)fn)((void*)(uintptr_t)a[0], (size_t)a[1], st);
}

static const int ksmi_n_thunks = 89;
static const char* const ksmi_thunk_sigs[] = {"ipppfppiii", "ipppfpppiii", "ipppzp", "p", "pi", "pii", "piiidpppppffipppp", "piiidpppppffppppppppiiii", "piiiipppi", "piiiipppif", "piipppippppppdlii", "piipppipppppppdlii", "piipppipppppppidlii", "pipipiiiii", "pipippipiiii", "plipii", "pp", "ppi", "ppiiidffi", "ppiiii", "ppiiiii", "ppiiiiii", "ppiiiiiiii", "ppiiiiiiiiiiii", "ppiiiiiiiiiiiii", "ppiiili", "ppiiilii", "ppilii", "ppipiiiiipppi", "ppippiiiiii", "ppippppiiiiipppi", "ppl", "ppli", "pplif", "pppfpppli", "pppi", "pppiiiifi", "pppiiiii", "pppiiiiifi", "pppiiiiifufupi", "pppiiiiii", "pppiiiiiii", "pppiiilii", "pppippiii", "pppippiiiii", "pppipppiii", "pppli", "ppplif", "pppliiufuufupi", "ppplpffff", "ppplufupi", "ppppiiii", "ppppiiiii", "ppppiiiiipppfi", "ppppiilf", "ppppiliufupi", "ppppliifi", "pppplpffffff", "pppplpffffffip", "pppppiiii", "pppppiiiii", "pppppiiiiii", "pppppiiiiufupi", "pppppiili", "pppppilii", "ppppplii", "ppppppiifi", "ppppppiiiifi", "ppppppiiiifuffuffuiiiip", "ppppppiiiii", "ppppppiiiiiii", "ppppppilii", "ppppppipiii", "pppppppdlii", "pppppppidlii", "pppppppiiiii", "pppppppiiiiifi", "pppppppiiiiifufupi", "pppppppiiiiiifi", "ppppppppdlifi", "ppppppppdlii", "ppppppppidlii", "ppppppppiiii", "pppppppppii", "ppppppppppiiiii", "pppppppppppiipiiiiiifi", "ppppppppppppppppppii", "ppppziiiiiii", "pz"};
static const ksmi_thunk_fn ksmi_thunks[] = {ksmi_thunk_0, ksmi_thunk_1, ksmi_thunk_2, ksmi_thunk_3, ksmi_thunk_4, ksmi_thunk_5, ksmi_thunk_6, ksmi_thunk_7, ksmi_thunk_8, ksmi_thunk_9, ksmi_thunk_10, ksmi_thunk_11, ksmi_thunk_12, ksmi_thunk_13, ksmi_thunk_14, ksmi_thunk_15, ksmi_thunk_16, ksmi_thunk_17, ksmi_thunk_18, ksmi_thunk_19, ksmi_thunk_20, ksmi_thunk_21, ksmi_thunk_22, ksmi_thunk_23, ksmi_thunk_24, ksmi_thunk_25, ksmi_thunk_26, ksmi_thunk_27, ksmi_thunk_28, ksmi_thunk_29, ksmi_thunk_30, ksmi_thunk_31, ksmi_thunk_32, ksmi_thunk_33, ksmi_thunk_34, ksmi_thunk_35, ksmi_thunk_36, ksmi_thunk_37, ksmi_thunk_38, ksmi_thunk_39, ksmi_thunk_40, ksmi_thunk_41, ksmi_thunk_42, ksmi_thunk_43, ksmi_thunk_44, ksmi_thunk_45, ksmi_thunk_46, ksmi_thunk_47, ksmi_thunk_48, ksmi_thunk_49, ksmi_thunk_50, ksmi_thunk_51, ksmi_thunk_52, ksmi_thunk_53, ksmi_thunk_54, ksmi_thunk_55, ksmi_thunk_56, ksmi_thunk_57, ksmi_thunk_58, ksmi_thunk_59, ksmi_thunk_60, ksmi_thunk_61, ksmi_thunk_62, ksmi_thunk_63, ksmi_thunk_64, ksmi_thunk_65, ksmi_thunk_66, ksmi_thunk_67, ksmi_thunk_68, ksmi_thunk_69, ksmi_thunk_70, ksmi_thunk_71, ksmi_thunk_72, ksmi_thunk_73, ksmi_thunk_74, ksmi_thunk_75, ksmi_thunk_76, ksmi_thunk_77, ksmi_thunk_78, ksmi_thunk_79, ksmi_thunk_80, ksmi_thunk_81, ksmi_thunk_82, ksmi_thunk_83, ksmi_thunk_84, ksmi_thunk_85, ksmi_thunk_86, ksmi_thunk_87, ksmi_thunk_88};
```

kurosiwo_amd/snunet_plan.py:

```python
import ctypes as C
import os

import torch

from . import _lib
from .plan_base import PlanBase, _Saved
from .runtime import Act, SrcSpec, conv_npad, conv_stats_rows, make_conv, make_pack, make_wgrad, packed_weight_numel
from .snunet import BN_EPS, BN_MOMENTUM


class SNUNetPlan(PlanBase):
    side_wgrad = True
    two_lanes = True
    bn_fused = os.environ.get("KSMI_BN_FUSED", "1") != "0"
    im2col_late = os.environ.get("KSMI_IM2COL_LATE", "1") != "0"
    up_gemm = os.environ.get("KSMI_UP_GEMM", "1") != "0"
    up_wgrad64 = os.environ.get("KSMI_UP_WGRAD64", "1") != "0"
    up_wgrad128 = os.environ.get("KSMI_UP_WGRAD128", "1") != "0"
    pack_kind = "pack_weights_batched"

    def __init__(self, model, B, H, W, dtype, training, with_backward, tail=0, sync_bn=False):
        self._init_lists(model, dtype, with_backward)
        self.B, self.H, self.W = B, H, W
        from . import distributed as _D
        self.sync_bn = bool(sync_bn) and training
        self.bn_world = _D.world_size() if self.sync_bn else 1
        if self.sync_bn:
            self.bn_fused = False
        self.training = training
        self._up_packs = []
        self._rowsums = []
        n, c = model.base_channel, model.in_channels
        self.n = n
        f = [n, 2 * n, 4 * n, 8 * n, 16 * n]
        self.tail = tail
        self.xA = torch.empty((B, c - tail, H, W), dtype=torch.float32, device=self.dev)
        self.xB = torch.empty_like(self.xA)
        self.xtail = torch.empty((B, tail, H, W), dtype=torch.float32, device=self.dev) if tail else None
        self.logits = torch.empty((B, 3, H, W), dtype=torch.float32, device=self.dev)
        self.dlogits = torch.empty_like(self.logits) if with_backward else None
        self.bwd_builders = []

        def A(name, lvl, ch):
            return Act(name, B, H >> lvl, W >> lvl, ch, dtype, self.dev)

        L = self._lane
        L(0); x0_0A, p0A = self._block("conv0_0", "A", [self.xA], A("x0_0A", 0, f[0]), first=True, pool="p0A")
        self._handover(0, 1, back=(1, 0))
        L(1); x0_0B, p0B = self._block("conv0_0", "B", [self.xB], A("x0_0B", 0, f[0]), first=True, pool="p0B")
        L(0); x1_0A, p1A = self._block("conv1_0", "A", [self._pool_at(x0_0A, p0A, "p0A")], A("x1_0A", 1, f[1]), pool="p1A")
        self._handover(0, 1, back=(1, 0))
        L(1); x1_0B, p1B = self._block("conv1_0", "B", [self._pool_at(x0_0B, p0B, "p0B")], A("x1_0B", 1, f[1]), pool="p1B")
        L(0); x2_0A, p2A = self._block("conv2_0", "A", [self._pool_at(x1_0A, p1A, "p1A")], A("x2_0A", 2, f[2]), pool="p2A")
        self._handover(0, 1, back=(1, 0))
        L(1); x2_0B, p2B = self._block("conv2_0", "B", [self._pool_at(x1_0B, p1B, "p1B")], A("x2_0B", 2, f[2]), pool="p2B")
        L(0); x3_0A = self._block("conv3_0", "A", [self._pool_at(x2_0A, p2A, "p2A")], A("x3_0A", 3, f[3]))
        self._handover(0, 1, back=(1, 0))
        L(1); x3_0B, p3B = self._block("conv3_0", "B", [self._pool_at(x2_0B, p2B, "p2B")], A("x3_0B", 3, f[3]), pool="p3B")
        x4_0B = self._block("conv4_0", "B", [self._pool_at(x3_0B, p3B, "p3B")], A("x4_0B", 4, f[4]))
        self._handover(1, 0, back=(0, 1))

        self._handover(0, 1, back=(1, 0))
        L(0); x0_1 = self._block("conv0_1", "", [x0_0A, x0_0B, self._up("Up1_0", x1_0B)], A("x0_1", 0, f[0]))
        L(1); x1_1 = self._block("conv1_1", "", [x1_0A, x1_0B, self._up("Up2_0", x2_0B)], A("x1_1", 1, f[1]))
        u1_1 = self._up("Up1_1", x1_1)
        self._handover(1, 0, back=(0, 1))
        L(0); x0_2 = self._block("conv0_2", "", [x0_0A, x0_0B, x0_1, u1_1], A("x0_2", 0, f[0]))
        L(1); x2_1 = self._block("conv2_1", "", [x2_0A, x2_0B, self._up("Up3_0", x3_0B)], A("x2_1", 2, f[2]))
        x1_2 = self._block("conv1_2", "", [x1_0A, x1_0B, x1_1, self._up("Up2_1", x2_1)], A("x1_2", 1, f[1]))
        u1_2 = self._up("Up1_2", x1_2)
        self._handover(1, 0, back=(0, 1))
        L(0); x0_3 = self._block("conv0_3", "", [x0_0A, x0_0B, x0_1, x0_2, u1_2], A("x0_3", 0, f[0]))
        L(1); x3_1 = self._block("conv3_1", "", [x3_0A, x3_0B, self._up("Up4_0", x4_0B)], A("x3_1", 3, f[3]))
        x2_2 = self._block("conv2_2", "", [x2_0A, x2_0B, x2_1, self._up("Up3_1", x3_1)], A("x2_2", 2, f[2]))
        x1_3 = self._block("conv1_3", "", [x1_0A, x1_0B, x1_1, x1_2, self._up("Up2_2", x2_2)], A("x1_3", 1, f[1]))
        u1_3 = self._up("Up1_3", x1_3)
        self._handover(1, 0, back=(0, 1))
        L(0); x0_4 = self._block("conv0_4", "", [x0_0A, x0_0B, x0_1, x0_2, x0_3, u1_3], A("x0_4", 0, f[0]))
        self._head([x0_1, x0_2, x0_3, x0_4])
        self.acts = {a.name: a for a in (x0_0A, x0_0B, x1_0A, x1_0B, x3_0B, x4_0B, x0_1, x1_1, x0_2, x0_3, x0_4, x1_3, x3_1)}

        if with_backward:
            for lane, build in reversed(self.bwd_builders):
                self._lane(lane)
                build()
            self._lane(0)
        self._finish()

    def _before_pack_table(self):
        if self._rowsums:
            nr = len(self._rowsums)
            arr_r = (_lib.RowsumDesc * nr)(*[r for r, _ in self._rowsums])
            raw_r = bytes(C.string_at(C.addressof(arr_r), C.sizeof(arr_r)))
            rtable = torch.frombuffer(bytearray(raw_r), dtype=torch.uint8).to(self.dev)
            self.keep.append(rtable)
            self.bwd.add("ksmi_reduce_rows_batched", lambda: (rtable.data_ptr(), nr))
            self._mark(*[k for _, k in self._rowsums])
        for i in range(0, len(self._up_packs), 16):
            grp = self._up_packs[i:i + 16]
            wt_a = (C.c_void_p * len(grp))(*[w.data_ptr() for w, _, _ in grp])
            wb_a = (C.c_void_p * len(grp))(*[b.data_ptr() for _, b, _ in grp])
            c_a = (C.c_int * len(grp))(*[c for _, _, c in grp])
            self.keep += [wt_a, wb_a, c_a]
            self.packs.add("ksmi_up_pack_weights_batched", lambda wt_a=wt_a, wb_a=wb_a, c_a=c_a, k=len(grp): (wt_a, wb_a, c_a, k),
                           {"kind": "up_pack_weight", "bytes": sum(4 * c * c * 6 for _, _, c in grp), "flops": 0})

# ... 167 lines not shown
                                   B, 2 * H, 2 * W, H, W, 2, 2, 2, 0, Cc, self.dtype)
                w2 = self._packed(wkey, t2, 4, Cc, Cc, 4, Cc * 4, 0, 1, 0)
                d2.wpk = w2.data_ptr()
                self._conv(self.bwd, d2, "dgrad")
            if up_wgrad_gemm:
                six = self._side_ix(wkey)
                sW = self._sname("wgrad" + ("_s2" if six else ""))
                self.need(sW, self.lib.ksmi_up_wgrad_workspace(B, H, W, Cc))
                a_w = self._acc_param(wkey)
                self.bwd.add("ksmi_up_wgrad", lambda: (x.t.data_ptr(), gy.data_ptr(), self.scr(sW), self.m._g(wkey).data_ptr(), a_w, B, H, W, Cc),
                             {"kind": "up_gemm_wgrad", "bytes": B * H * W * Cc * 5 * es + 16 * Cc * Cc, "flops": 2 * B * H * W * Cc * 4 * Cc,
                              "tag": f"{wkey} K={Cc} N={4 * Cc} {H}x{W}", "side": True, "side_ix": six})
                self._mark(wkey)
            else:
                dw, ws = make_wgrad(s2, x.t, Cc, 0, Cc, self.m._g(wkey), 4, Cc * 4, 1, self._acc_param(wkey),
                                    B, 2 * H, 2 * W, H, W, 2, 2, 2, 0, self.dtype)
                self._wgrad(dw, ws, wkey)
            if not fused_bias:
                npix = B * 4 * H * W
                rows = self._rows(npix)
                pb = torch.empty(rows * Cc, dtype=torch.float32, device=self.dev)
                self.bwd.add("ksmi_channel_sum", lambda: (gy.data_ptr(), pb.data_ptr(), rows, npix, Cc, self.dt))
                self._rowsum_at_end(bkey, pb, rows, 1, 0, Cc, Cc)
        self.bwd_builders.append((self.fwd.cur_lane, build_bwd))
        return y

    def _block(self, name, branch, sources, out, first=False, pool=None):
        m, B, H, W, Cc = self.m, out.B, out.H, out.W, out.C
        npix = B * H * W
        dtype, dt, training = self.dtype, self.dt, self.training
        self._level(H)
        i_act = Act(f"{name}{branch}.i", B, H, W, Cc, dtype, self.dev)
        z_act = Act(f"{name}{branch}.z", B, H, W, Cc, dtype, self.dev)
        sv1, sv2 = _Saved(Cc, self.dev), _Saved(Cc, self.dev)
        self.keep += [i_act, z_act, sv1, sv2]
        P = lambda s: m._p(f"{name}.{s}").data_ptr()
        G = lambda s: m._g(f"{name}.{s}").data_ptr()
        Bf = lambda s: m._b(f"{name}.{s}").data_ptr()
        Npad = conv_npad(Cc)
        sS, sR = self._sname("stats"), self._sname("red")
        stats = (lambda: self.scr(sS)) if training else (lambda: None)

        if first:
            x_img = sources[0]
            chead, cin = x_img.shape[1], m.in_channels
            x_tail = self.xtail.data_ptr() if self.tail else None
            kc = 32 if dtype == torch.bfloat16 else 16
            Kpad = -(-(cin * 9) // kc) * kc
            rows1, cpad1, Ktot = self.lib.ksmi_conv_first_stats_rows(B, H, W), Cc, cin
            self.need(sS, rows1 * 2 * Cc * 4)
            raw = m._raw_ptrs(self.dev)
            self.fwd.add("ksmi_conv_first_forward_raw", lambda: (x_img.data_ptr(), x_tail, chead, P("conv1.weight"), P("conv1.bias"),
                                                                 i_act.t.data_ptr(), stats(), B, cin, H, W, Cc, *raw, dt))
            if self.with_backward:
                col = torch.empty((B, H, W, Kpad), dtype=dtype, device=self.dev)
                self.keep.append(col)
                im2col_args = lambda: (x_img.data_ptr(), x_tail, chead, col.data_ptr(), B, cin, H, W, Kpad, *raw, dt)
                if not self.im2col_late:
                    self.fwd.add("ksmi_im2col3x3_raw", im2col_args)
                src1 = [SrcSpec(col, Kpad)]
        else:
            srcs = [SrcSpec(a.t, a.C) for a in sources]
            Ktot = sum(a.C for a in sources)
            d1, t1 = make_conv(srcs, [(i_act.t, Cc, 0, 0, Cc, 0)], i_act.t, m._p(f"{name}.conv1.bias"), None,
                               B, H, W, H, W, 3, 3, 1, 1, Cc, dtype)
            w1 = self._packed(f"{name}.conv1.weight", t1, 9, Cc, Cc, 9, Ktot * 9, 0, 1, 0)
            d1.wpk = w1.data_ptr()
            rows1, cpad1 = conv_stats_rows(d1, dtype), Npad
            if training:
                self.need(sS, rows1 * 2 * Npad * 4)
                self.patch(d1, "stats", sS)
            self._conv(self.fwd, d1)

        gcount = float(npix * self.bn_world)

        def bn_fin(bn, sv, rows, cpad):
            nbt = m._c(f"{name}.{bn}.num_batches_tracked").data_ptr()
            if self.sync_bn:
                self.fwd.add_allreduce(lambda rows=rows, cpad=cpad: self._bufs[sS][:rows * 2 * cpad * 4].view(torch.float32))
            self.fwd.add("ksmi_bn_finalize", lambda: (stats(), rows, cpad, Cc, gcount, P(f"{bn}.weight"), P(f"{bn}.bias"),
                                                      Bf(f"{bn}.running_mean"), Bf(f"{bn}.running_var"), nbt,
                                                      BN_MOMENTUM, BN_EPS, 1 if training else 0,
                                                      sv.mean, sv.rstd, sv.scale, sv.shift))
        bn_fin("bn1", sv1, rows1, cpad1)

        src2 = [SrcSpec(i_act.t, Cc, scale=sv1.scale_t, shift=sv1.shift_t, relu=1)]
        d2, t2 = make_conv(src2, [(z_act.t, Cc, 0, 0, Cc, 0)], z_act.t, m._p(f"{name}.conv2.bias"), None,
                           B, H, W, H, W, 3, 3, 1, 1, Cc, dtype)
        w2 = self._packed(f"{name}.conv2.weight", t2, 9, Cc, Cc, 9, Cc * 9, 0, 1, 0)
        d2.wpk = w2.data_ptr()
        rows2 = conv_stats_rows(d2, dtype)
        if training:
            self.need(sS, rows2 * 2 * Npad * 4)
            self.patch(d2, "stats", sS)
        self._conv(self.fwd, d2)
        fused = training and self.bn_fused and bool(self.lib.ksmi_bn_fused_supported(Cc, Npad, dt))
        pooled = None
        if fused:
            if pool is not None:
                pooled = Act(pool, B, H // 2, W // 2, Cc, dtype, self.dev)
            nbt2 = m._c(f"{name}.bn2.num_batches_tracked").data_ptr()
            pp = pooled.t.data_ptr() if pooled is not None else None
            self.fwd.add("ksmi_bn_fin_add_relu", lambda: (stats(), rows2, Npad, Cc, float(npix), P("bn2.weight"), P("bn2.bias"),
                                                          Bf("bn2.running_mean"), Bf("bn2.running_var"), nbt2, BN_MOMENTUM, BN_EPS,
                                                          sv2.mean, sv2.rstd, sv2.scale, sv2.shift, z_act.t.data_ptr(), i_act.t.data_ptr(),
                                                          out.t.data_ptr(), pp, B, H, W, dt),
                         {"kind": "bn_fin_add_relu", "bytes": npix * Cc * self._es() * (3.25 if pooled is not None else 3), "flops": 0})
        else:
            bn_fin("bn2", sv2, rows2, Npad)
            self.fwd.add("ksmi_bn_add_relu", lambda: (z_act.t.data_ptr(), i_act.t.data_ptr(), sv2.scale, sv2.shift,
                                                      out.t.data_ptr(), npix, Cc, dt))

        def build_bwd():
            self._level(H)
            gated = self._emit_dgrad(out, gate=(out.t, z_act.t, sv2)) if os.environ.get("KSMI_NO_GATE") is None else self._emit_dgrad(out)
            gated = gated if isinstance(gated, tuple) else None
            rows = self._rows(npix)
            self.need(sR, rows * 2 * Cc * 4)
            sums1 = torch.zeros((2, Cc), dtype=torch.float32, device=self.dev)
            sums2 = torch.zeros((2, Cc), dtype=torch.float32, device=self.dev)
            dz = torch.empty_like(z_act.t)
            r = torch.empty_like(i_act.t)
            self.keep += [sums1, sums2, dz, r]
            gout = out.grad().data_ptr()
            s1p, s2p = sums1.data_ptr(), sums2.data_ptr()
            a_bn2 = self._acc_param(f"{name}.bn2")
            es = self._es()
            if gated is not None:
                gst, grows, gpad = gated
                if fused and self.lib.ksmi_bn_fused_supported(Cc, gpad, dt):
                    self.bwd.add("ksmi_bn_bwd_fin_apply_gated", lambda: (gst.data_ptr(), grows, gpad, s2p, G("bn2.weight"), G("bn2.bias"), a_bn2,
                                                                         gout, z_act.t.data_ptr(), sv2.mean, sv2.rstd, P("bn2.weight"),
                                                                         dz.data_ptr(), float(npix), npix, Cc, dt),
                                 {"kind": "bn_bwd_fin_apply_gated", "bytes": npix * Cc * es * 3, "flops": 0})
                    self._mark(f"{name}.bn2.weight", f"{name}.bn2.bias")
                else:
                    self.bwd.add("ksmi_reduce_rows", lambda: (gst.data_ptr(), grows, 2, gpad, Cc, s2p, G("bn2.weight"), G("bn2.bias"), a_bn2))
                    self._mark(f"{name}.bn2.weight", f"{name}.bn2.bias")
                    if self.sync_bn:
                        self.bwd.add_allreduce(lambda: sums2)
                    self.bwd.add("ksmi_bn_bwd_apply_gated", lambda: (gout, z_act.t.data_ptr(), sv2.mean, sv2.rstd, P("bn2.weight"), s2p,
                                                                     dz.data_ptr(), gcount, npix, Cc, dt))
            else:
                self.bwd.add("ksmi_bnrelu_bwd_reduce", lambda: (gout, out.t.data_ptr(), z_act.t.data_ptr(), sv2.mean, sv2.rstd,
                                                                self.scr(sR), rows, npix, Cc, dt))
                if fused:
                    self.bwd.add("ksmi_bnrelu_bwd_fin_apply", lambda: (self.scr(sR), rows, Cc, s2p, G("bn2.weight"), G("bn2.bias"), a_bn2,
                                                                       gout, out.t.data_ptr(), z_act.t.data_ptr(), sv2.mean, sv2.rstd,
                                                                       P("bn2.weight"), dz.data_ptr(), float(npix), npix, Cc, dt),
                                 {"kind": "bnrelu_bwd_fin_apply", "bytes": npix * Cc * es * 5, "flops": 0})
                    self._mark(f"{name}.bn2.weight", f"{name}.bn2.bias")
                else:
                    self.bwd.add("ksmi_reduce_rows", lambda: (self.scr(sR), rows, 2, Cc, Cc, s2p, G("bn2.weight"), G("bn2.bias"), a_bn2))
                    self._mark(f"{name}.bn2.weight", f"{name}.bn2.bias")
                    if self.sync_bn:
                        self.bwd.add_allreduce(lambda: sums2)
                    self.bwd.add("ksmi_bnrelu_bwd_apply", lambda: (gout, out.t.data_ptr(), z_act.t.data_ptr(), sv2.mean, sv2.rstd,
                                                                   P("bn2.weight"), s2p, dz.data_ptr(), gcount, npix, Cc, dt))
            if training:
                self._rowsum_at_end(f"{name}.conv2.bias", None, 0, 1, 0, Cc, Cc)
            else:
                pz = torch.empty(rows * Cc, dtype=torch.float32, device=self.dev)
                self.bwd.add("ksmi_channel_sum", lambda: (dz.data_ptr(), pz.data_ptr(), rows, npix, Cc, dt))
                self._rowsum_at_end(f"{name}.conv2.bias", pz, rows, 1, 0, Cc, Cc)
            dg2, tg2 = make_conv([SrcSpec(dz, Cc)], [(r, Cc, 0, 0, Cc, 0)], dz, None, None, B, H, W, H, W, 3, 3, 1, 1, Cc, dtype,
                                 mask=(i_act.t, sv1.t[0], sv1.t[1], sv1.t[2], sv1.t[3]))
            wg2 = self._packed(f"{name}.conv2.weight", tg2, 9, Cc, Cc, Cc * 9, 9, 0, 1, 1)
            dg2.wpk = wg2.data_ptr()
            rows_g = conv_stats_rows(dg2, dtype)
# ... 107 lines not shown
```

Before: 2261 tiles/s.

## Fuse bn1 finalize with BN+ReLU apply into materialized activation for conv2

Adds a kernel that finalizes bn1 batch statistics and, in the same launch, writes the normalized ReLU activation to a new buffer. At the selected pyramid levels (default 0,2,3,4), conv2 reads this plain activation instead of applying scale/shift/ReLU on the fly inside its input loader. The aim is to take per-tap normalization work out of the conv2 inner loop, where it is repeated for each of the nine 3x3 taps. In exchange it costs one extra read and write of the activation and more memory per block; backward still needs to handle the stored activation correctly.

```diff
diff --git a/include/ksmi.h b/include/ksmi.h
--- a/include/ksmi.h
+++ b/include/ksmi.h
@@ -186,6 +186,10 @@
                          float* running_mean, float* running_var, int64_t* num_batches_tracked, float momentum, float eps,
                          float* mean, float* rstd, float* scale, float* shift, const void* z, const void* identity, void* out,
                          void* pooled, int B, int H, int W, int dtype, void* stream);
+int ksmi_bn_fin_apply_relu(float* partial, int rows, int Cpad, int C, double count, const float* gamma, const float* beta,
+                           float* running_mean, float* running_var, int64_t* num_batches_tracked, float momentum, float eps,
+                           float* mean, float* rstd, float* scale, float* shift, const void* x, void* a, int64_t npix, int dtype,
+                           void* stream);
 int ksmi_bn_bwd_fin_apply_gated(float* partial, int rows, int Cstride, float* sums, float* dgamma, float* dbeta, int accumulate,
                                 const void* g, const void* z, const float* mean, const float* rstd, const float* gamma, void* dz,
                                 double count, int64_t npix, int C, int dtype, void* stream);
diff --git a/kurosiwo_amd/_lib.py b/kurosiwo_amd/_lib.py
--- a/kurosiwo_amd/_lib.py
+++ b/kurosiwo_amd/_lib.py
@@ -128,6 +128,7 @@
     "ksmi_bn_fused_supported": (_i, [_i, _i, _i]),
     "ksmi_bn_fused_max_rows": (_i, []),
     "ksmi_bn_fin_add_relu": (_i, [_vp, _i, _i, _i, _d, _vp, _vp, _vp, _vp, _vp, _f, _f, _vp, _vp, _vp, _vp, _vp, _vp, _vp, _vp, _i, _i, _i, _i, _vp]),
+    "ksmi_bn_fin_apply_relu": (_i, [_vp, _i, _i, _i, _d, _vp, _vp, _vp, _vp, _vp, _f, _f, _vp, _vp, _vp, _vp, _vp, _vp, _i64, _i, _vp]),
     "ksmi_bn_bwd_fin_apply_gated": (_i, [_vp, _i, _i, _vp, _vp, _vp, _i, _vp, _vp, _vp, _vp, _vp, _vp, _d, _i64, _i, _i, _vp]),
     "ksmi_bnrelu_bwd_fin_apply": (_i, [_vp, _i, _i, _vp, _vp, _vp, _i, _vp, _vp, _vp, _vp, _vp, _vp, _vp, _d, _i64, _i, _i, _vp]),
     "ksmi_bn_bwd_fin_apply_add": (_i, [_vp, _i, _i, _vp, _vp, _vp, _i, _vp, _vp, _vp, _vp, _vp, _vp, _vp, _i, _d, _i64, _i, _i, _vp]),
diff --git a/kurosiwo_amd/csrc/bnfused.hip b/kurosiwo_amd/csrc/bnfused.hip
--- a/kurosiwo_amd/csrc/bnfused.hip
+++ b/kurosiwo_amd/csrc/bnfused.hip
@@ -126,6 +126,60 @@
   }
 }
 
+template <typename T>
+__global__ __launch_bounds__(kFat) void bn_fin_apply_relu_kernel(FinArgs f, const T* __restrict__ x, T* __restrict__ a, int64_t nvec) {
+  constexpr int VEC = ElemTraits<T>::kVec;
+  __shared__ double red[kFat * 4];
+  __shared__ double sums[2 * kMaxC];
+  __shared__ float s_scale[kMaxC], s_shift[kMaxC];
+  const int C = f.C;
+  block_rows_sum(f.partial, f.rows, f.Cstride, C, red, sums);
+  for (int c = threadIdx.x; c < C; c += kFat) {
+    const double mean = sums[c] / f.count;
+    double var = sums[C + c] / f.count - mean * mean;
+    if (var < 0.0) var = 0.0;
+    const float rs = (float)(1.0 / sqrt(var + (double)f.eps));
+    const float sc = f.gamma[c] * rs;
+    const float sh = f.beta[c] - (float)mean * sc;
+    s_scale[c] = sc; s_shift[c] = sh;
+    if (blockIdx.x == 0) {
+      f.mean_o[c] = (float)mean; f.rstd_o[c] = rs; f.scale_o[c] = sc; f.shift_o[c] = sh;
+      const double unb = f.count > 1.0 ? var * f.count / (f.count - 1.0) : var;
+      f.rmean[c] = (1.f - f.momentum) * f.rmean[c] + f.momentum * (float)mean;
+      f.rvar[c] = (1.f - f.momentum) * f.rvar[c] + f.momentum * (float)unb;
+    }
+  }
+  if (blockIdx.x == 0 && threadIdx.x == 0 && f.nbt) *f.nbt += 1;
+  __syncthreads();
+  const int CV = C / VEC;
+  const int64_t stride = (int64_t)gridDim.x * kFat;
+  for (int64_t v = (int64_t)blockIdx.x * kFat + threadIdx.x; v < nvec; v += 2 * stride) {
+    const int64_t v1 = v + stride;
+    const bool two = v1 < nvec;
+    const u32x4 r0 = *(const u32x4*)(x + v * VEC);
+    const u32x4 r1 = *(const u32x4*)(x + (two ? v1 : v) * VEC);
+    float xv[VEC];
+    int c = (int)(v % CV) * VEC;
+    vec_unpack<T>(r0, xv);
+#pragma unroll
+    for (int j = 0; j < VEC; ++j) {
+      xv[j] = xv[j] * s_scale[c + j] + s_shift[c + j];
+      xv[j] = fmaxf(xv[j], 0.f);
+    }
+    *(u32x4*)(a + v * VEC) = vec_pack<T>(xv);
+    if (two) {
+      c = (int)(v1 % CV) * VEC;
+      vec_unpack<T>(r1, xv);
+#pragma unroll
+      for (int j = 0; j < VEC; ++j) {
+        xv[j] = xv[j] * s_scale[c + j] + s_shift[c + j];
+        xv[j] = fmaxf(xv[j], 0.f);
+      }
+      *(u32x4*)(a + v1 * VEC) = vec_pack<T>(xv);
+    }
+  }
+}
+
 struct BwdFinArgs {
   const float* partial; int rows, Cstride, C;
   float* sums_o; float* dgamma; float* dbeta; int accumulate;
@@ -289,6 +343,23 @@
   return ksmi_check_launch("bn_fin_add_relu");
 }
 
+int ksmi_bn_fin_apply_relu(float* partial, int rows, int Cpad, int C, double count, const float* gamma, const float* beta,
+                           float* running_mean, float* running_var, int64_t* num_batches_tracked, float momentum, float eps,
+                           float* mean, float* rstd, float* scale, float* shift, const void* x, void* a, int64_t npix, int dtype,
+                           void* stream) {
+  if (!fused_ok(C, dtype, Cpad) || !partial || rows < 1 || npix < 1 || !x || !a) return ksmi_fail(KSMI_E_ARG, "bn_fin_apply_relu: bad args");
+  rows = ksmi_internal_fold_rows(partial, rows, 2, Cpad, C, (hipStream_t)stream);
+  FinArgs f{partial, rows, Cpad, C, count, gamma, beta, running_mean, running_var, num_batches_tracked, momentum, eps, mean, rstd, scale, shift};
+  const int vec = dtype == KSMI_BF16 ? 8 : 4;
+  const int64_t nvec = npix * (C / vec);
+  const dim3 grid(fat_grid((nvec + 1) / 2));
+  if (dtype == KSMI_BF16)
+    hipLaunchKernelGGL(bn_fin_apply_relu_kernel<bf16_t>, grid, dim3(kFat), 0, (hipStream_t)stream, f, (const bf16_t*)x, (bf16_t*)a, nvec);
+  else
+    hipLaunchKernelGGL(bn_fin_apply_relu_kernel<float>, grid, dim3(kFat), 0, (hipStream_t)stream, f, (const float*)x, (float*)a, nvec);
+  return ksmi_check_launch("bn_fin_apply_relu");
+}
+
 static int bwd_apply(int mode, float* partial, int rows, int Cstride, float* sums, float* dgamma, float* dbeta, int accumulate,
                      void* g, const void* outp, const void* z, const float* mean, const float* rstd, const float* gamma, void* dz,
                      double count, int64_t npix, int C, int dtype, void* stream, const char* what) {
diff --git a/kurosiwo_amd/csrc/thunks_gen.h b/kurosiwo_amd/csrc/thunks_gen.h
--- a/kurosiwo_amd/csrc/thunks_gen.h
+++ b/kurosiwo_amd/csrc/thunks_gen.h
@@ -36,334 +36,338 @@
   (void)a; return ((F)fn)((void*)(uintptr_t)a[0], (int)(int64_t)a[1], (int)(int64_t)a[2], (int)(int64_t)a[3], ksmi_slot_f64(a[4]), (void*)(uintptr_t)a[5], (void*)(uintptr_t)a[6], (void*)(uintptr_t)a[7], (void*)(uintptr_t)a[8], (void*)(uintptr_t)a[9], ksmi_slot_f32(a[10]), ksmi_slot_f32(a[11]), (int)(int64_t)a[12], (void*)(uintptr_t)a[13], (void*)(uintptr_t)a[14], (void*)(uintptr_t)a[15], (void*)(uintptr_t)a[16], st);
 }
 static int ksmi_thunk_7(const void* fn, const uint64_t* a, void* st) {
+  typedef int (*F)(void*, int, int, int, double, void*, void*, void*, void*, void*, float, float, void*, void*, void*, void*, void*, void*, long long, int, void*);
+  (void)a; return ((F)fn)((void*)(uintptr_t)a[0], (int)(int64_t)a[1], (int)(int64_t)a[2], (int)(int64_t)a[3], ksmi_slot_f64(a[4]), (void*)(uintptr_t)a[5], (void*)(uintptr_t)a[6], (void*)(uintptr_t)a[7], (void*)(uintptr_t)a[8], (void*)(uintptr_t)a[9], ksmi_slot_f32(a[10]), ksmi_slot_f32(a[11]), (void*)(uintptr_t)a[12], (void*)(uintptr_t)a[13], (void*)(uintptr_t)a[14], (void*)(uintptr_t)a[15], (void*)(uintptr_t)a[16], (void*)(uintptr_t)a[17], (long long)a[18], (int)(int64_t)a[19], st);
+}
+static int ksmi_thunk_8(const void* fn, const uint64_t* a, void* st) {
   typedef int (*F)(void*, int, int, int, double, void*, void*, void*, void*, void*, float, float, void*, void*, void*, void*, void*, void*, void*, void*, int, int, int, int, void*);
   (void)a; return ((F)fn)((void*)(uintptr_t)a[0], (int)(int64_t)a[1], (int)(int64_t)a[2], (int)(int64_t)a[3], ksmi_slot_f64(a[4]), (void*)(uintptr_t)a[5], (void*)(uintptr_t)a[6], (void*)(uintptr_t)a[7], (void*)(uintptr_t)a[8], (void*)(uintptr_t)a[9], ksmi_slot_f32(a[10]), ksmi_slot_f32(a[11]), (void*)(uintptr_t)a[12], (void*)(uintptr_t)a[13], (void*)(uintptr_t)a[14], (void*)(uintptr_t)a[15], (void*)(uintptr_t)a[16], (void*)(uintptr_t)a[17], (void*)(uintptr_t)a[18], (void*)(uintptr_t)a[19], (int)(int64_t)a[20], (int)(int64_t)a[21], (int)(int64_t)a[22], (int)(int64_t)a[23], st);
 }
-static int ksmi_thunk_8(const void* fn, const uint64_t* a, void* st) {
+static int ksmi_thunk_9(const void* fn, const uint64_t* a, void* st) {
   typedef int (*F)(void*, int, int, int, int, void*, void*, void*, int, void*);
   (void)a; return ((F)fn)((void*)(uintptr_t)a[0], (int)(int64_t)a[1], (int)(int64_t)a[2], (int)(int64_t)a[3], (int)(int64_t)a[4], (void*)(uintptr_t)a[5], (void*)(uintptr_t)a[6], (void*)(uintptr_t)a[7], (int)(int64_t)a[8], st);
 }
-static int ksmi_thunk_9(const void* fn, const uint64_t* a, void* st) {
+static int ksmi_thunk_10(const void* fn, const uint64_t* a, void* st) {
   typedef int (*F)(void*, int, int, int, int, void*, void*, void*, int, float, void*);
   (void)a; return ((F)fn)((void*)(uintptr_t)a[0], (int)(int64_t)a[1], (int)(int64_t)a[2], (int)(int64_t)a[3], (int)(int64_t)a[4], (void*)(uintptr_t)a[5], (void*)(uintptr_t)a[6], (void*)(uintptr_t)a[7], (int)(int64_t)a[8], ksmi_slot_f32(a[9]), st);
 }
-static int ksmi_thunk_10(const void* fn, const uint64_t* a, void* st) {
+static int ksmi_thunk_11(const void* fn, const uint64_t* a, void* st) {
   typedef int (*F)(void*, int, int, void*, void*, void*, int, void*, void*, void*, void*, void*, void*, double, long long, int, int, void*);
   (void)a; return ((F)fn)((void*)(uintptr_t)a[0], (int)(int64_t)a[1], (int)(int64_t)a[2], (void*)(uintptr_t)a[3], (void*)(uintptr_t)a[4], (void*)(uintptr_t)a[5], (int)(int64_t)a[6], (void*)(uintptr_t)a[7], (void*)(uintptr_t)a[8], (void*)(uintptr_t)a[9], (void*)(uintptr_t)a[10], (void*)(uintptr_t)a[11], (void*)(uintptr_t)a[12], ksmi_slot_f64(a[13]), (long long)a[14], (int)(int64_t)a[15], (int)(int64_t)a[16], st);
 }
-static int ksmi_thunk_11(const void* fn, const uint64_t* a, void* st) {
+static int ksmi_thunk_12(const void* fn, const uint64_t* a, void* st) {
   typedef int (*F)(void*, int, int, void*, void*, void*, int, void*, void*, void*, void*, void*, void*, void*, double, long long, int, int, void*);
   (void)a; return ((F)fn)((void*)(uintptr_t)a[0], (int)(int64_t)a[1], (int)(int64_t)a[2], (void*)(uintptr_t)a[3], (void*)(uintptr_t)a[4], (void*)(uintptr_t)a[5], (int)(int64_t)a[6], (void*)(uintptr_t)a[7], (void*)(uintptr_t)a[8], (void*)(uintptr_t)a[9], (void*)(uintptr_t)a[10], (void*)(uintptr_t)a[11], (void*)(uintptr_t)a[12], (void*)(uintptr_t)a[13], ksmi_slot_f64(a[14]), (long long)a[15], (int)(int64_t)a[16], (int)(int64_t)a[17], st);
 }
-static int ksmi_thunk_12(const void* fn, const uint64_t* a, void* st) {
+static int ksmi_thunk_13(const void* fn, const uint64_t* a, void* st) {
   typedef int (*F)(void*, int, int, void*, void*, void*, int, void*, void*, void*, void*, void*, void*, void*, int, double, long long, int, int, void*);
   (void)a; return ((F)fn)((void*)(uintptr_t)a[0], (int)(int64_t)a[1], (int)(int64_t)a[2], (void*)(uintptr_t)a[3], (void*)(uintptr_t)a[4], (void*)(uintptr_t)a[5], (int)(int64_t)a[6], (void*)(uintptr_t)a[7], (void*)(uintptr_t)a[8], (void*)(uintptr_t)a[9], (void*)(uintptr_t)a[10], (void*)(uintptr_t)a[11], (void*)(uintptr_t)a[12], (void*)(uintptr_t)a[13], (int)(int64_t)a[14], ksmi_slot_f64(a[15]), (long long)a[16], (int)(int64_t)a[17], (int)(int64_t)a[18], st);
 }
-static int ksmi_thunk_13(const void* fn, const uint64_t* a, void* st) {
+static int ksmi_thunk_14(const void* fn, const uint64_t* a, void* st) {
   typedef int (*F)(void*, int, void*, int, void*, int, int, int, int, int, void*);
   (void)a; return ((F)fn)((void*)(uintptr_t)a[0], (int)(int64_t)a[1], (void*)(uintptr_t)a[2], (int)(int64_t)a[3], (void*)(uintptr_t)a[4], (int)(int64_t)a[5], (int)(int64_t)a[6], (int)(int64_t)a[7], (int)(int64_t)a[8], (int)(int64_t)a[9], st);
 }
-static int ksmi_thunk_14(const void* fn, const uint64_t* a, void* st) {
+static int ksmi_thunk_15(const void* fn, const uint64_t* a, void* st) {
   typedef int (*F)(void*, int, void*, int, void*, void*, int, void*, int, int, int, int, void*);
   (void)a; return ((F)fn)((void*)(uintptr_t)a[0], (int)(int64_t)a[1], (void*)(uintptr_t)a[2], (int)(int64_t)a[3], (void*)(uintptr_t)a[4], (void*)(uintptr_t)a[5], (int)(int64_t)a[6], (void*)(uintptr_t)a[7], (int)(int64_t)a[8], (int)(int64_t)a[9], (int)(int64_t)a[10], (int)(int64_t)a[11], st);
 }
-static int ksmi_thunk_15(const void* fn, const uint64_t* a, void* st) {
+static int ksmi_thunk_16(const void* fn, const uint64_t* a, void* st) {
   typedef int (*F)(void*, long long, int, void*, int, int, void*);
   (void)a; return ((F)fn)((void*)(uintptr_t)a[0], (long long)a[1], (int)(int64_t)a[2], (void*)(uintptr_t)a[3], (int)(int64_t)a[4], (int)(int64_t)a[5], st);
 }
-static int ksmi_thunk_16(const void* fn, const uint64_t* a, void* st) {
+static int ksmi_thunk_17(const void* fn, const uint64_t* a, void* st) {
   typedef int (*F)(void*, void*, void*);
   (void)a; return ((F)fn)((void*)(uintptr_t)a[0], (void*)(uintptr_t)a[1], st);
 }
-static int ksmi_thunk_17(const void* fn, const uint64_t* a, void* st) {
+static int ksmi_thunk_18(const void* fn, const uint64_t* a, void* st) {
   typedef int (*F)(void*, void*, int, void*);
   (void)a; return ((F)fn)((void*)(uintptr_t)a[0], (void*)(uintptr_t)a[1], (int)(int64_t)a[2], st);
 }
-static int ksmi_thunk_18(const void* fn, const uint64_t* a, void* st) {
+static int ksmi_thunk_19(const void* fn, const uint64_t* a, void* st) {
   typedef int (*F)(void*, void*, int, int, int, double, float, float, int, void*);
   (void)a; return ((F)fn)((void*)(uintptr_t)a[0], (void*)(uintptr_t)a[1], (int)(int64_t)a[2], (int)(int64_t)a[3], (int)(int64_t)a[4], ksmi_slot_f64(a[5]), ksmi_slot_f32(a[6]), ksmi_slot_f32(a[7]), (int)(int64_t)a[8], st);
 }
-static int ksmi_thunk_19(const void* fn, const uint64_t* a, void* st) {
+static int ksmi_thunk_20(const void* fn, const uint64_t* a, void* st) {
   typedef int (*F)(void*, void*, int, int, int, int, void*);
   (void)a; return ((F)fn)((void*)(uintptr_t)a[0], (void*)(uintptr_t)a[1], (int)(int64_t)a[2], (int)(int64_t)a[3], (int)(int64_t)a[4], (int)(int64_t)a[5], st);
 }
-static int ksmi_thunk_20(const void* fn, const uint64_t* a, void* st) {
+static int ksmi_thunk_21(const void* fn, const uint64_t* a, void* st) {
   typedef int (*F)(void*, void*, int, int, int, int, int, void*);
   (void)a; return ((F)fn)((void*)(uintptr_t)a[0], (void*)(uintptr_t)a[1], (int)(int64_t)a[2], (int)(int64_t)a[3], (int)(int64_t)a[4], (int)(int64_t)a[5], (int)(int64_t)a[6], st);
 }
-static int ksmi_thunk_21(const void* fn, const uint64_t* a, void* st) {
+static int ksmi_thunk_22(const void* fn, const uint64_t* a, void* st) {
   typedef int (*F)(void*, void*, int, int, int, int, int, int, void*);
   (void)a; return ((F)fn)((void*)(uintptr_t)a[0], (void*)(uintptr_t)a[1], (int)(int64_t)a[2], (int)(int64_t)a[3], (int)(int64_t)a[4], (int)(int64_t)a[5], (int)(int64_t)a[6], (int)(int64_t)a[7], st);
 }
-static int ksmi_thunk_22(const void* fn, const uint64_t* a, void* st) {
+static int ksmi_thunk_23(const void* fn, const uint64_t* a, void* st) {
   typedef int (*F)(void*, void*, int, int, int, int, int, int, int, int, void*);
   (void)a; return ((F)fn)((void*)(uintptr_t)a[0], (void*)(uintptr_t)a[1], (int)(int64_t)a[2], (int)(int64_t)a[3], (int)(int64_t)a[4], (int)(int64_t)a[5], (int)(int64_t)a[6], (int)(int64_t)a[7], (int)(int64_t)a[8], (int)(int64_t)a[9], st);
 }
-static int ksmi_thunk_23(const void* fn, const uint64_t* a, void* st) {
+static int ksmi_thunk_24(const void* fn, const uint64_t* a, void* st) {
   typedef int (*F)(void*, void*, int, int, int, int, int, int, int, int, int, int, int, int, void*);
   (void)a; return ((F)fn)((void*)(uintptr_t)a[0], (void*)(uintptr_t)a[1], (int)(int64_t)a[2], (int)(int64_t)a[3], (int)(int64_t)a[4], (int)(int64_t)a[5], (int)(int64_t)a[6], (int)(int64_t)a[7], (int)(int64_t)a[8], (int)(int64_t)a[9], (int)(int64_t)a[10], (int)(int64_t)a[11], (int)(int64_t)a[12], (int)(int64_t)a[13], st);
 }
-static int ksmi_thunk_24(const void* fn, const uint64_t* a, void* st) {
+static int ksmi_thunk_25(const void* fn, const uint64_t* a, void* st) {
   typedef int (*F)(void*, void*, int, int, int, int, int, int, int, int, int, int, int, int, int, void*);
   (void)a; return ((F)fn)((void*)(uintptr_t)a[0], (void*)(uintptr_t)a[1], (int)(int64_t)a[2], (int)(int64_t)a[3], (int)(int64_t)a[4], (int)(int64_t)a[5], (int)(int64_t)a[6], (int)(int64_t)a[7], (int)(int64_t)a[8], (int)(int64_t)a[9], (int)(int64_t)a[10], (int)(int64_t)a[11], (int)(int64_t)a[12], (int)(int64_t)a[13], (int)(int64_t)a[14], st);
 }
-static int ksmi_thunk_25(const void* fn, const uint64_t* a, void* st) {
+static int ksmi_thunk_26(const void* fn, const uint64_t* a, void* st) {
   typedef int (*F)(void*, void*, int, int, int, long long, int, void*);
   (void)a; return ((F)fn)((void*)(uintptr_t)a[0], (void*)(uintptr_t)a[1], (int)(int64_t)a[2], (int)(int64_t)a[3], (int)(int64_t)a[4], (long long)a[5], (int)(int64_t)a[6], st);
 }
-static int ksmi_thunk_26(const void* fn, const uint64_t* a, void* st) {
+static int ksmi_thunk_27(const void* fn, const uint64_t* a, void* st) {
   typedef int (*F)(void*, void*, int, int, int, long long, int, int, void*);
   (void)a; return ((F)fn)((void*)(uintptr_t)a[0], (void*)(uintptr_t)a[1], (int)(int64_t)a[2], (int)(int64_t)a[3], (int)(int64_t)a[4], (long long)a[5], (int)(int64_t)a[6], (int)(int64_t)a[7], st);
 }
-static int ksmi_thunk_27(const void* fn, const uint64_t* a, void* st) {
+static int ksmi_thunk_28(const void* fn, const uint64_t* a, void* st) {
   typedef int (*F)(void*, void*, int, long long, int, int, void*);
   (void)a; return ((F)fn)((void*)(uintptr_t)a[0], (void*)(uintptr_t)a[1], (int)(int64_t)a[2], (long long)a[3], (int)(int64_t)a[4], (int)(int64_t)a[5], st);
 }
-static int ksmi_thunk_28(const void* fn, const uint64_t* a, void* st) {
+static int ksmi_thunk_29(const void* fn, const uint64_t* a, void* st) {
   typedef int (*F)(void*, void*, int, void*, int, int, int, int, int, void*, void*, void*, int, void*);
   (void)a; return ((F)fn)((void*)(uintptr_t)a[0], (void*)(uintptr_t)a[1], (int)(int64_t)a[2], (void*)(uintptr_t)a[3], (int)(int64_t)a[4], (int)(int64_t)a[5], (int)(int64_t)a[6], (int)(int64_t)a[7], (int)(int64_t)a[8], (void*)(uintptr_t)a[9], (void*)(uintptr_t)a[10], (void*)(uintptr_t)a[11], (int)(int64_t)a[12], st);
 }
-static int ksmi_thunk_29(const void* fn, const uint64_t* a, void* st) {
+static int ksmi_thunk_30(const void* fn, const uint64_t* a, void* st) {
   typedef int (*F)(void*, void*, int, void*, void*, int, int, int, int, int, int, void*);
   (void)a; return ((F)fn)((void*)(uintptr_t)a[0], (void*)(uintptr_t)a[1], (int)(int64_t)a[2], (void*)(uintptr_t)a[3], (void*)(uintptr_t)a[4], (int)(int64_t)a[5], (int)(int64_t)a[6], (int)(int64_t)a[7], (int)(int64_t)a[8], (int)(int64_t)a[9], (int)(int64_t)a[10], st);
 }
-static int ksmi_thunk_30(const void* fn, const uint64_t* a, void* st) {
+static int ksmi_thunk_31(const void* fn, const uint64_t* a, void* st) {
   typedef int (*F)(void*, void*, int, void*, void*, void*, void*, int, int, int, int, int, void*, void*, void*, int, void*);
   (void)a; return ((F)fn)((void*)(uintptr_t)a[0], (void*)(uintptr_t)a[1], (int)(int64_t)a[2], (void*)(uintptr_t)a[3], (void*)(uintptr_t)a[4], (void*)(uintptr_t)a[5], (void*)(uintptr_t)a[6], (int)(int64_t)a[7], (int)(int64_t)a[8], (int)(int64_t)a[9], (int)(int64_t)a[10], (int)(int64_t)a[11], (void*)(uintptr_t)a[12], (void*)(uintptr_t)a[13], (void*)(uintptr_t)a[14], (int)(int64_t)a[15], st);
 }
-static int ksmi_thunk_31(const void* fn, const uint64_t* a, void* st) {
+static int ksmi_thunk_32(const void* fn, const uint64_t* a, void* st) {
   typedef int (*F)(void*, void*, long long, void*);
   (void)a; return ((F)fn)((void*)(uintptr_t)a[0], (void*)(uintptr_t)a[1], (long long)a[2], st);
 }
-static int ksmi_thunk_32(const void* fn, const uint64_t* a, void* st) {
+static int ksmi_thunk_33(const void* fn, const uint64_t* a, void* st) {
   typedef int (*F)(void*, void*, long long, int, void*);
   (void)a; return ((F)fn)((void*)(uintptr_t)a[0], (void*)(uintptr_t)a[1], (long long)a[2], (int)(int64_t)a[3], st);
 }
-static int ksmi_thunk_33(const void* fn, const uint64_t* a, void* st) {
+static int ksmi_thunk_34(const void* fn, const uint64_t* a, void* st) {
   typedef int (*F)(void*, void*, long long, int, float, void*);
   (void)a; return ((F)fn)((void*)(uintptr_t)a[0], (void*)(uintptr_t)a[1], (long long)a[2], (int)(int64_t)a[3], ksmi_slot_f32(a[4]), st);
 }
-static int ksmi_thunk_34(const void* fn, const uint64_t* a, void* st) {
+static int ksmi_thunk_35(const void* fn, const uint64_t* a, void* st) {
   typedef int (*F)(void*, void*, void*, float, void*, void*, void*, long long, int, void*);
   (void)a; return ((F)fn)((void*)(uintptr_t)a[0], (void*)(uintptr_t)a[1], (void*)(uintptr_t)a[2], ksmi_slot_f32(a[3]), (void*)(uintptr_t)a[4], (void*)(uintptr_t)a[5], (void*)(uintptr_t)a[6], (long long)a[7], (int)(int64_t)a[8], st);
 }
-static int ksmi_thunk_35(const void* fn, const uint64_t* a, void* st) {
+static int ksmi_thunk_36(const void* fn, const uint64_t* a, void* st) {
   typedef int (*F)(void*, void*, void*, int, void*);
   (void)a; return ((F)fn)((void*)(uintptr_t)a[0], (void*)(uintptr_t)a[1], (void*)(uintptr_t)a[2], (int)(int64_t)a[3], st);
 }
-static int ksmi_thunk_36(const void* fn, const uint64_t* a, void* st) {
+static int ksmi_thunk_37(const void* fn, const uint64_t* a, void* st) {
   typedef int (*F)(void*, void*, void*, int, int, int, int, float, int, void*);
   (void)a; return ((F)fn)((void*)(uintptr_t)a[0], (void*)(uintptr_t)a[1], (void*)(uintptr_t)a[2], (int)(int64_t)a[3], (int)(int64_t)a[4], (int)(int64_t)a[5], (int)(int64_t)a[6], ksmi_slot_f32(a[7]), (int)(int64_t)a[8], st);
 }
-static int ksmi_thunk_37(const void* fn, const uint64_t* a, void* st) {
+static int ksmi_thunk_38(const void* fn, const uint64_t* a, void* st) {
   typedef int (*F)(void*, void*, void*, int, int, int, int, int, void*);
   (void)a; return ((F)fn)((void*)(uintptr_t)a[0], (void*)(uintptr_t)a[1], (void*)(uintptr_t)a[2], (int)(int64_t)a[3], (int)(int64_t)a[4], (int)(int64_t)a[5], (int)(int64_t)a[6], (int)(int64_t)a[7], st);
 }
-static int ksmi_thunk_38(const void* fn, const uint64_t* a, void* st) {
+static int ksmi_thunk_39(const void* fn, const uint64_t* a, void* st) {
   typedef int (*F)(void*, void*, void*, int, int, int, int, int, float, int, void*);
   (void)a; return ((F)fn)((void*)(uintptr_t)a[0], (void*)(uintptr_t)a[1], (void*)(uintptr_t)a[2], (int)(int64_t)a[3], (int)(int64_t)a[4], (int)(int64_t)a[5], (int)(int64_t)a[6], (int)(int64_t)a[7], ksmi_slot_f32(a[8]), (int)(int64_t)a[9], st);
 }
-static int ksmi_thunk_39(const void* fn, const uint64_t* a, void* st) {
+static int ksmi_thunk_40(const void* fn, const uint64_t* a, void* st) {
   typedef int (*F)(void*, void*, void*, int, int, int, int, int, float, unsigned int, float, unsigned int, void*, int, void*);
   (void)a; return ((F)fn)((void*)(uintptr_t)a[0], (void*)(uintptr_t)a[1], (void*)(uintptr_t)a[2], (int)(int64_t)a[3], (int)(int64_t)a[4], (int)(int64_t)a[5], (int)(int64_t)a[6], (int)(int64_t)a[7], ksmi_slot_f32(a[8]), (unsigned int)a[9], ksmi_slot_f32(a[10]), (unsigned int)a[11], (void*)(uintptr_t)a[12], (int)(int64_t)a[13], st);
 }
-static int ksmi_thunk_40(const void* fn, const uint64_t* a, void* st) {
+static int ksmi_thunk_41(const void* fn, const uint64_t* a, void* st) {
   typedef int (*F)(void*, void*, void*, int, int, int, int, int, int, void*);
   (void)a; return ((F)fn)((void*)(uintptr_t)a[0], (void*)(uintptr_t)a[1], (void*)(uintptr_t)a[2], (int)(int64_t)a[3], (int)(int64_t)a[4], (int)(int64_t)a[5], (int)(int64_t)a[6], (int)(int64_t)a[7], (int)(int64_t)a[8], st);
 }
-static int ksmi_thunk_41(const void* fn, const uint64_t* a, void* st) {
+static int ksmi_thunk_42(const void* fn, const uint64_t* a, void* st) {
   typedef int (*F)(void*, void*, void*, int, int, int, int, int, int, int, void*);
   (void)a; return ((F)fn)((void*)(uintptr_t)a[0], (void*)(uintptr_t)a[1], (void*)(uintptr_t)a[2], (int)(int64_t)a[3], (int)(int64_t)a[4], (int)(int64_t)a[5], (int)(int64_t)a[6], (int)(int64_t)a[7], (int)(int64_t)a[8], (int)(int64_t)a[9], st);
 }
-static int ksmi_thunk_42(const void* fn, const uint64_t* a, void* st) {
+static int ksmi_thunk_43(const void* fn, const uint64_t* a, void* st) {
   typedef int (*F)(void*, void*, void*, int, int, int, long long, int, int, void*);
   (void)a; return ((F)fn)((void*)(uintptr_t)a[0], (void*)(uintptr_t)a[1], (void*)(uintptr_t)a[2], (int)(int64_t)a[3], (int)(int64_t)a[4], (int)(int64_t)a[5], (long long)a[6], (int)(int64_t)a[7], (int)(int64_t)a[8], st);
 }
-static int ksmi_thunk_43(const void* fn, const uint64_t* a, void* st) {
+static int ksmi_thunk_44(const void* fn, const uint64_t* a, void* st) {
   typedef int (*F)(void*, void*, void*, int, void*, void*, int, int, int, void*);
   (void)a; return ((F)fn)((void*)(uintptr_t)a[0], (void*)(uintptr_t)a[1], (void*)(uintptr_t)a[2], (int)(int64_t)a[3], (void*)(uintptr_t)a[4], (void*)(uintptr_t)a[5], (int)(int64_t)a[6], (int)(int64_t)a[7], (int)(int64_t)a[8], st);
 }
-static int ksmi_thunk_44(const void* fn, const uint64_t* a, void* st) {
+static int ksmi_thunk_45(const void* fn, const uint64_t* a, void* st) {
   typedef int (*F)(void*, void*, void*, int, void*, void*, int, int, int, int, int, void*);
   (void)a; return ((F)fn)((void*)(uintptr_t)a[0], (void*)(uintptr_t)a[1], (void*)(uintptr_t)a[2], (int)(int64_t)a[3], (void*)(uintptr_t)a[4], (void*)(uintptr_t)a[5], (int)(int64_t)a[6], (int)(int64_t)a[7], (int)(int64_t)a[8], (int)(int64_t)a[9], (int)(int64_t)a[10], st);
 }
-static int ksmi_thunk_45(const void* fn, const uint64_t* a, void* st) {
+static int ksmi_thunk_46(const void* fn, const uint64_t* a, void* st) {
   typedef int (*F)(void*, void*, void*, int, void*, void*, void*, int, int, int, void*);
   (void)a; return ((F)fn)((void*)(uintptr_t)a[0], (void*)(uintptr_t)a[1], (void*)(uintptr_t)a[2], (int)(int64_t)a[3], (void*)(uintptr_t)a[4], (void*)(uintptr_t)a[5], (void*)(uintptr_t)a[6], (int)(int64_t)a[7], (int)(int64_t)a[8], (int)(int64_t)a[9], st);
 }
-static int ksmi_thunk_46(const void* fn, const uint64_t* a, void* st) {
+static int ksmi_thunk_47(const void* fn, const uint64_t* a, void* st) {
   typedef int (*F)(void*, void*, void*, long long, int, void*);
   (void)a; return ((F)fn)((void*)(uintptr_t)a[0], (void*)(uintptr_t)a[1], (void*)(uintptr_t)a[2], (long long)a[3], (int)(int64_t)a[4], st);
 }
-static int ksmi_thunk_47(const void* fn, const uint64_t* a, void* st) {
+static int ksmi_thunk_48(const void* fn, const uint64_t* a, void* st) {
   typedef int (*F)(void*, void*, void*, long long, int, float, void*);
   (void)a; return ((F)fn)((void*)(uintptr_t)a[0], (void*)(uintptr_t)a[1], (void*)(uintptr_t)a[2], (long long)a[3], (int)(int64_t)a[4], ksmi_slot_f32(a[5]), st);
 }
-static int ksmi_thunk_48(const void* fn, const uint64_t* a, void* st) {
+static int ksmi_thunk_49(const void* fn, const uint64_t* a, void* st) {
   typedef int (*F)(void*, void*, void*, long long, int, int, unsigned int, float, unsigned int, unsigned int, float, unsigned int, void*, int, void*);
   (void)a; return ((F)fn)((void*)(uintptr_t)a[0], (void*)(uintptr_t)a[1], (void*)(uintptr_t)a[2], (long long)a[3], (int)(int64_t)a[4], (int)(int64_t)a[5], (unsigned int)a[6], ksmi_slot_f32(a[7]), (unsigned int)a[8], (unsigned int)a[9], ksmi_slot_f32(a[10]), (unsigned int)a[11], (void*)(uintptr_t)a[12], (int)(int64_t)a[13], st);
 }
-static int ksmi_thunk_49(const void* fn, const uint64_t* a, void* st) {
+static int ksmi_thunk_50(const void* fn, const uint64_t* a, void* st) {
   typedef int (*F)(void*, void*, void*, long long, void*, float, float, float, float, void*);
   (void)a; return ((F)fn)((void*)(uintptr_t)a[0], (void*)(uintptr_t)a[1], (void*)(uintptr_t)a[2], (long long)a[3], (void*)(uintptr_t)a[4], ksmi_slot_f32(a[5]), ksmi_slot_f32(a[6]), ksmi_slot_f32(a[7]), ksmi_slot_f32(a[8]), st);
 }
-static int ksmi_thunk_50(const void* fn, const uint64_t* a, void* st) {
+static int ksmi_thunk_51(const void* fn, const uint64_t* a, void* st) {
   typedef int (*F)(void*, void*, void*, long long, unsigned int, float, unsigned int, void*, int, void*);
   (void)a; return ((F)fn)((void*)(uintptr_t)a[0], (void*)(uintptr_t)a[1], (void*)(uintptr_t)a[2], (long long)a[3], (unsigned int)a[4], ksmi_slot_f32(a[5]), (unsigned int)a[6], (void*)(uintptr_t)a[7], (int)(int64_t)a[8], st);
 }
-static int ksmi_thunk_51(const void* fn, const uint64_t* a, void* st) {
+static int ksmi_thunk_52(const void* fn, const uint64_t* a, void* st) {
   typedef int (*F)(void*, void*, void*, void*, int, int, int, int, void*);
   (void)a; return ((F)fn)((void*)(uintptr_t)a[0], (void*)(uintptr_t)a[1], (void*)(uintptr_t)a[2], (void*)(uintptr_t)a[3], (int)(int64_t)a[4], (int)(int64_t)a[5], (int)(int64_t)a[6], (int)(int64_t)a[7], st);
 }
-static int ksmi_thunk_52(const void* fn, const uint64_t* a, void* st) {
+static int ksmi_thunk_53(const void* fn, const uint64_t* a, void* st) {
   typedef int (*F)(void*, void*, void*, void*, int, int, int, int, int, void*);
   (void)a; return ((F)fn)((void*)(uintptr_t)a[0], (void*)(uintptr_t)a[1], (void*)(uintptr_t)a[2], (void*)(uintptr_t)a[3], (int)(int64_t)a[4], (int)(int64_t)a[5], (int)(int64_t)a[6], (int)(int64_t)a[7], (int)(int64_t)a[8], st);
 }
-static int ksmi_thunk_53(const void* fn, const uint64_t* a, void* st) {
+static int ksmi_thunk_54(const void* fn, const uint64_t* a, void* st) {
   typedef int (*F)(void*, void*, void*, void*, int, int, int, int, int, void*, void*, void*, float, int, void*);
   (void)a; return ((F)fn)((void*)(uintptr_t)a[0], (void*)(uintptr_t)a[1], (void*)(uintptr_t)a[2], (void*)(uintptr_t)a[3], (int)(int64_t)a[4], (int)(int64_t)a[5], (int)(int64_t)a[6], (int)(int64_t)a[7], (int)(int64_t)a[8], (void*)(uintptr_t)a[9], (void*)(uintptr_t)a[10], (void*)(uintptr_t)a[11], ksmi_slot_f32(a[12]), (int)(int64_t)a[13], st);
 }
-static int ksmi_thunk_54(const void* fn, const uint64_t* a, void* st) {
+static int ksmi_thunk_55(const void* fn, const uint64_t* a, void* st) {
   typedef int (*F)(void*, void*, void*, void*, int, int, long long, float, void*);
   (void)a; return ((F)fn)((void*)(uintptr_t)a[0], (void*)(uintptr_t)a[1], (void*)(uintptr_t)a[2], (void*)(uintptr_t)a[3], (int)(int64_t)a[4], (int)(int64_t)a[5], (long long)a[6], ksmi_slot_f32(a[7]), st);
 }
-static int ksmi_thunk_55(const void* fn, const uint64_t* a, void* st) {
+static int ksmi_thunk_56(const void* fn, const uint64_t* a, void* st) {
   typedef int (*F)(void*, void*, void*, void*, int, long long, int, unsigned int, float, unsigned int, void*, int, void*);
   (void)a; return ((F)fn)((void*)(uintptr_t)a[0], (void*)(uintptr_t)a[1], (void*)(uintptr_t)a[2], (void*)(uintptr_t)a[3], (int)(int64_t)a[4], (long long)a[5], (int)(int64_t)a[6], (unsigned int)a[7], ksmi_slot_f32(a[8]), (unsigned int)a[9], (void*)(uintptr_t)a[10], (int)(int64_t)a[11], st);
 }
-static int ksmi_thunk_56(const void* fn, const uint64_t* a, void* st) {
+static int ksmi_thunk_57(const void* fn, const uint64_t* a, void* st) {
   typedef int (*F)(void*, void*, void*, void*, long long, int, int, float, int, void*);
   (void)a; return ((F)fn)((void*)(uintptr_t)a[0], (void*)(uintptr_t)a[1], (void*)(uintptr_t)a[2], (void*)(uintptr_t)a[3], (long long)a[4], (int)(int64_t)a[5], (int)(int64_t)a[6], ksmi_slot_f32(a[7]), (int)(int64_t)a[8], st);
 }
-static int ksmi_thunk_57(const void* fn, const uint64_t* a, void* st) {
+static int ksmi_thunk_58(const void* fn, const uint64_t* a, void* st) {
   typedef int (*F)(void*, void*, void*, void*, long long, void*, float, float, float, float, float, float, void*);
   (void)a; return ((F)fn)((void*)(uintptr_t)a[0], (void*)(uintptr_t)a[1], (void*)(uintptr_t)a[2], (void*)(uintptr_t)a[3], (long long)a[4], (void*)(uintptr_t)a[5], ksmi_slot_f32(a[6]), ksmi_slot_f32(a[7]), ksmi_slot_f32(a[8]), ksmi_slot_f32(a[9]), ksmi_slot_f32(a[10]), ksmi_slot_f32(a[11]), st);
 }
-static int ksmi_thunk_58(const void* fn, const uint64_t* a, void* st) {
+static int ksmi_thunk_59(const void* fn, const uint64_t* a, void* st) {
   typedef int (*F)(void*, void*, void*, void*, long long, void*, float, float, float, float, float, float, int, void*, void*);
   (void)a; return ((F)fn)((void*)(uintptr_t)a[0], (void*)(uintptr_t)a[1], (void*)(uintptr_t)a[2], (void*)(uintptr_t)a[3], (long long)a[4], (void*)(uintptr_t)a[5], ksmi_slot_f32(a[6]), ksmi_slot_f32(a[7]), ksmi_slot_f32(a[8]), ksmi_slot_f32(a[9]), ksmi_slot_f32(a[10]), ksmi_slot_f32(a[11]), (int)(int64_t)a[12], (void*)(uintptr_t)a[13], st);
 }
-static int ksmi_thunk_59(const void* fn, const uint64_t* a, void* st) {
+static int ksmi_thunk_60(const void* fn, const uint64_t* a, void* st) {
   typedef int (*F)(void*, void*, void*, void*, void*, int, int, int, int, void*);
   (void)a; return ((F)fn)((void*)(uintptr_t)a[0], (void*)(uintptr_t)a[1], (void*)(uintptr_t)a[2], (void*)(uintptr_t)a[3], (void*)(uintptr_t)a[4], (int)(int64_t)a[5], (int)(int64_t)a[6], (int)(int64_t)a[7], (int)(int64_t)a[8], st);
 }
-static int ksmi_thunk_60(const void* fn, const uint64_t* a, void* st) {
+static int ksmi_thunk_61(const void* fn, const uint64_t* a, void* st) {
   typedef int (*F)(void*, void*, void*, void*, void*, int, int, int, int, int, void*);
   (void)a; return ((F)fn)((void*)(uintptr_t)a[0], (void*)(uintptr_t)a[1], (void*)(uintptr_t)a[2], (void*)(uintptr_t)a[3], (void*)(uintptr_t)a[4], (int)(int64_t)a[5], (int)(int64_t)a[6], (int)(int64_t)a[7], (int)(int64_t)a[8], (int)(int64_t)a[9], st);
 }
-static int ksmi_thunk_61(const void* fn, const uint64_t* a, void* st) {
+static int ksmi_thunk_62(const void* fn, const uint64_t* a, void* st) {
   typedef int (*F)(void*, void*, void*, void*, void*, int, int, int, int, int, int, void*);
   (void)a; return ((F)fn)((void*)(uintptr_t)a[0], (void*)(uintptr_t)a[1], (void*)(uintptr_t)a[2], (void*)(uintptr_t)a[3], (void*)(uintptr_t)a[4], (int)(int64_t)a[5], (int)(int64_t)a[6], (int)(int64_t)a[7], (int)(int64_t)a[8], (int)(int64_t)a[9], (int)(int64_t)a[10], st);
 }
-static int ksmi_thunk_62(const void* fn, const uint64_t* a, void* st) {
+static int ksmi_thunk_63(const void* fn, const uint64_t* a, void* st) {
   typedef int (*F)(void*, void*, void*, void*, void*, int, int, int, int, unsigned int, float, unsigned int, void*, int, void*);
   (void)a; return ((F)fn)((void*)(uintptr_t)a[0], (void*)(uintptr_t)a[1], (void*)(uintptr_t)a[2], (void*)(uintptr_t)a[3], (void*)(uintptr_t)a[4], (int)(int64_t)a[5], (int)(int64_t)a[6], (int)(int64_t)a[7], (int)(int64_t)a[8], (unsigned int)a[9], ksmi_slot_f32(a[10]), (unsigned int)a[11], (void*)(uintptr_t)a[12], (int)(int64_t)a[13], st);
 }
-static int ksmi_thunk_63(const void* fn, const uint64_t* a, void* st) {
+static int ksmi_thunk_64(const void* fn, const uint64_t* a, void* st) {
   typedef int (*F)(void*, void*, void*, void*, void*, int, int, long long, int, void*);
   (void)a; return ((F)fn)((void*)(uintptr_t)a[0], (void*)(uintptr_t)a[1], (void*)(uintptr_t)a[2], (void*)(uintptr_t)a[3], (void*)(uintptr_t)a[4], (int)(int64_t)a[5], (int)(int64_t)a[6], (long long)a[7], (int)(int64_t)a[8], st);
 }
-static int ksmi_thunk_64(const void* fn, const uint64_t* a, void* st) {
+static int ksmi_thunk_65(const void* fn, const uint64_t* a, void* st) {
   typedef int (*F)(void*, void*, void*, void*, void*, int, long long, int, int, void*);
   (void)a; return ((F)fn)((void*)(uintptr_t)a[0], (void*)(uintptr_t)a[1], (void*)(uintptr_t)a[2], (void*)(uintptr_t)a[3], (void*)(uintptr_t)a[4], (int)(int64_t)a[5], (long long)a[6], (int)(int64_t)a[7], (int)(int64_t)a[8], st);
 }
-static int ksmi_thunk_65(const void* fn, const uint64_t* a, void* st) {
+static int ksmi_thunk_66(const void* fn, const uint64_t* a, void* st) {
   typedef int (*F)(void*, void*, void*, void*, void*, long long, int, int, void*);
   (void)a; return ((F)fn)((void*)(uintptr_t)a[0], (void*)(uintptr_t)a[1], (void*)(uintptr_t)a[2], (void*)(uintptr_t)a[3], (void*)(uintptr_t)a[4], (long long)a[5], (int)(int64_t)a[6], (int)(int64_t)a[7], st);
 }
-static int ksmi_thunk_66(const void* fn, const uint64_t* a, void* st) {
+static int ksmi_thunk_67(const void* fn, const uint64_t* a, void* st) {
   typedef int (*F)(void*, void*, void*, void*, void*, void*, int, int, float, int, void*);
   (void)a; return ((F)fn)((void*)(uintptr_t)a[0], (void*)(uintptr_t)a[1], (void*)(uintptr_t)a[2], (void*)(uintptr_t)a[3], (void*)(uintptr_t)a[4], (void*)(uintptr_t)a[5], (int)(int64_t)a[6], (int)(int64_t)a[7], ksmi_slot_f32(a[8]), (int)(int64_t)a[9], st);
 }
-static int ksmi_thunk_67(const void* fn, const uint64_t* a, void* st) {
+static int ksmi_thunk_68(const void* fn, const uint64_t* a, void* st) {
   typedef int (*F)(void*, void*, void*, void*, void*, void*, int, int, int, int, float, int, void*);
   (void)a; return ((F)fn)((void*)(uintptr_t)a[0], (void*)(uintptr_t)a[1], (void*)(uintptr_t)a[2], (void*)(uintptr_t)a[3], (void*)(uintptr_t)a[4], (void*)(uintptr_t)a[5], (int)(int64_t)a[6], (int)(int64_t)a[7], (int)(int64_t)a[8], (int)(int64_t)a[9], ksmi_slot_f32(a[10]), (int)(int64_t)a[11], st);
 }
-static int ksmi_thunk_68(const void* fn, const uint64_t* a, void* st) {
+static int ksmi_thunk_69(const void* fn, const uint64_t* a, void* st) {
   typedef int (*F)(void*, void*, void*, void*, void*, void*, int, int, int, int, float, unsigned int, float, float, unsigned int, float, float, unsigned int, int, int, int, int, void*, void*);
   (void)a; return ((F)fn)((void*)(uintptr_t)a[0], (void*)(uintptr_t)a[1], (void*)(uintptr_t)a[2], (void*)(uintptr_t)a[3], (void*)(uintptr_t)a[4], (void*)(uintptr_t)a[5], (int)(int64_t)a[6], (int)(int64_t)a[7], (int)(int64_t)a[8], (int)(int64_t)a[9], ksmi_slot_f32(a[10]), (unsigned int)a[11], ksmi_slot_f32(a[12]), ksmi_slot_f32(a[13]), (unsigned int)a[14], ksmi_slot_f32(a[15]), ksmi_slot_f32(a[16]), (unsigned int)a[17], (int)(int64_t)a[18], (int)(int64_t)a[19], (int)(int64_t)a[20], (int)(int64_t)a[21], (void*)(uintptr_t)a[22], st);
 }
-static int ksmi_thunk_69(const void* fn, const uint64_t* a, void* st) {
+static int ksmi_thunk_70(const void* fn, const uint64_t* a, void* st) {
   typedef int (*F)(void*, void*, void*, void*, void*, void*, int, int, int, int, int, void*);
   (void)a; return ((F)fn)((void*)(uintptr_t)a[0], (void*)(uintptr_t)a[1], (void*)(uintptr_t)a[2], (void*)(uintptr_t)a[3], (void*)(uintptr_t)a[4], (void*)(uintptr_t)a[5], (int)(int64_t)a[6], (int)(int64_t)a[7], (int)(int64_t)a[8], (int)(int64_t)a[9], (int)(int64_t)a[10], st);
 }
-static int ksmi_thunk_70(const void* fn, const uint64_t* a, void* st) {
+static int ksmi_thunk_71(const void* fn, const uint64_t* a, void* st) {
   typedef int (*F)(void*, void*, void*, void*, void*, void*, int, int, int, int, int, int, int, void*);
   (void)a; return ((F)fn)((void*)(uintptr_t)a[0], (void*)(uintptr_t)a[1], (void*)(uintptr_t)a[2], (void*)(uintptr_t)a[3], (void*)(uintptr_t)a[4], (void*)(uintptr_t)a[5], (int)(int64_t)a[6], (int)(int64_t)a[7], (int)(int64_t)a[8], (int)(int64_t)a[9], (int)(int64_t)a[10], (int)(int64_t)a[11], (int)(int64_t)a[12], st);
 }
-static int ksmi_thunk_71(const void* fn, const uint64_t* a, void* st) {
+static int ksmi_thunk_72(const void* fn, const uint64_t* a, void* st) {
   typedef int (*F)(void*, void*, void*, void*, void*, void*, int, long long, int, int, void*);
   (void)a; return ((F)fn)((void*)(uintptr_t)a[0], (void*)(uintptr_t)a[1], (void*)(uintptr_t)a[2], (void*)(uintptr_t)a[3], (void*)(uintptr_t)a[4], (void*)(uintptr_t)a[5], (int)(int64_t)a[6], (long long)a[7], (int)(int64_t)a[8], (int)(int64_t)a[9], st);
 }
-static int ksmi_thunk_72(const void* fn, const uint64_t* a, void* st) {
+static int ksmi_thunk_73(const void* fn, const uint64_t* a, void* st) {
   typedef int (*F)(void*, void*, void*, void*, void*, void*, int, void*, int, int, int, void*);
   (void)a; return ((F)fn)((void*)(uintptr_t)a[0], (void*)(uintptr_t)a[1], (void*)(uintptr_t)a[2], (void*)(uintptr_t)a[3], (void*)(uintptr_t)a[4], (void*)(uintptr_t)a[5], (int)(int64_t)a[6], (void*)(uintptr_t)a[7], (int)(int64_t)a[8], (int)(int64_t)a[9], (int)(int64_t)a[10], st);
 }
-static int ksmi_thunk_73(const void* fn, const uint64_t* a, void* st) {
+static int ksmi_thunk_74(const void* fn, const uint64_t* a, void* st) {
   typedef int (*F)(void*, void*, void*, void*, void*, void*, void*, double, long long, int, int, void*);
   (void)a; return ((F)fn)((void*)(uintptr_t)a[0], (void*)(uintptr_t)a[1], (void*)(uintptr_t)a[2], (void*)(uintptr_t)a[3], (void*)(uintptr_t)a[4], (void*)(uintptr_t)a[5], (void*)(uintptr_t)a[6], ksmi_slot_f64(a[7]), (long long)a[8], (int)(int64_t)a[9], (int)(int64_t)a[10], st);
 }
-static int ksmi_thunk_74(const void* fn, const uint64_t* a, void* st) {
+static int ksmi_thunk_75(const void* fn, const uint64_t* a, void* st) {
   typedef int (*F)(void*, void*, void*, void*, void*, void*, void*, int, double, long long, int, int, void*);
   (void)a; return ((F)fn)((void*)(uintptr_t)a[0], (void*)(uintptr_t)a[1], (void*)(uintptr_t)a[2], (void*)(uintptr_t)a[3], (void*)(uintptr_t)a[4], (void*)(uintptr_t)a[5], (void*)(uintptr_t)a[6], (int)(int64_t)a[7], ksmi_slot_f64(a[8]), (long long)a[9], (int)(int64_t)a[10], (int)(int64_t)a[11], st);
 }
-static int ksmi_thunk_75(const void* fn, const uint64_t* a, void* st) {
+static int ksmi_thunk_76(const void* fn, const uint64_t* a, void* st) {
   typedef int (*F)(void*, void*, void*, void*, void*, void*, void*, int, int, int, int, int, void*);
   (void)a; return ((F)fn)((void*)(uintptr_t)a[0], (void*)(uintptr_t)a[1], (void*)(uintptr_t)a[2], (void*)(uintptr_t)a[3], (void*)(uintptr_t)a[4], (void*)(uintptr_t)a[5], (void*)(uintptr_t)a[6], (int)(int64_t)a[7], (int)(int64_t)a[8], (int)(int64_t)a[9], (int)(int64_t)a[10], (int)(int64_t)a[11], st);
 }
-static int ksmi_thunk_76(const void* fn, const uint64_t* a, void* st) {
+static int ksmi_thunk_77(const void* fn, const uint64_t* a, void* st) {
   typedef int (*F)(void*, void*, void*, void*, void*, void*, void*, int, int, int, int, int, float, int, void*);
   (void)a; return ((F)fn)((void*)(uintptr_t)a[0], (void*)(uintptr_t)a[1], (void*)(uintptr_t)a[2], (void*)(uintptr_t)a[3], (void*)(uintptr_t)a[4], (void*)(uintptr_t)a[5], (void*)(uintptr_t)a[6], (int)(int64_t)a[7], (int)(int64_t)a[8], (int)(int64_t)a[9], (int)(int64_t)a[10], (int)(int64_t)a[11], ksmi_slot_f32(a[12]), (int)(int64_t)a[13], st);
 }
-static int ksmi_thunk_77(const void* fn, const uint64_t* a, void* st) {
+static int ksmi_thunk_78(const void* fn, const uint64_t* a, void* st) {
   typedef int (*F)(void*, void*, void*, void*, void*, void*, void*, int, int, int, int, int, float, unsigned int, float, unsigned int, void*, int, void*);
   (void)a; return ((F)fn)((void*)(uintptr_t)a[0], (void*)(uintptr_t)a[1], (void*)(uintptr_t)a[2], (void*)(uintptr_t)a[3], (void*)(uintptr_t)a[4], (void*)(uintptr_t)a[5], (void*)(uintptr_t)a[6], (int)(int64_t)a[7], (int)(int64_t)a[8], (int)(int64_t)a[9], (int)(int64_t)a[10], (int)(int64_t)a[11], ksmi_slot_f32(a[12]), (unsigned int)a[13], ksmi_slot_f32(a[14]), (unsigned int)a[15], (void*)(uintptr_t)a[16], (int)(int64_t)a[17], st);
 }
-static int ksmi_thunk_78(const void* fn, const uint64_t* a, void* st) {
+static int ksmi_thunk_79(const void* fn, const uint64_t* a, void* st) {
   typedef int (*F)(void*, void*, void*, void*, void*, void*, void*, int, int, int, int, int, int, float, int, void*);
   (void)a; return ((F)fn)((void*)(uintptr_t)a[0], (void*)(uintptr_t)a[1], (void*)(uintptr_t)a[2], (void*)(uintptr_t)a[3], (void*)(uintptr_t)a[4], (void*)(uintptr_t)a[5], (void*)(uintptr_t)a[6], (int)(int64_t)a[7], (int)(int64_t)a[8], (int)(int64_t)a[9], (int)(int64_t)a[10], (int)(int64_t)a[11], (int)(int64_t)a[12], ksmi_slot_f32(a[13]), (int)(int64_t)a[14], st);
 }
-static int ksmi_thunk_79(const void* fn, const uint64_t* a, void* st) {
+static int ksmi_thunk_80(const void* fn, const uint64_t* a, void* st) {
   typedef int (*F)(void*, void*, void*, void*, void*, void*, void*, void*, double, long long, int, float, int, void*);
   (void)a; return ((F)fn)((void*)(uintptr_t)a[0], (void*)(uintptr_t)a[1], (void*)(uintptr_t)a[2], (void*)(uintptr_t)a[3], (void*)(uintptr_t)a[4], (void*)(uintptr_t)a[5], (void*)(uintptr_t)a[6], (void*)(uintptr_t)a[7], ksmi_slot_f64(a[8]), (long long)a[9], (int)(int64_t)a[10], ksmi_slot_f32(a[11]), (int)(int64_t)a[12], st);
 }
-static int ksmi_thunk_80(const void* fn, const uint64_t* a, void* st) {
+static int ksmi_thunk_81(const void* fn, const uint64_t* a, void* st) {
   typedef int (*F)(void*, void*, void*, void*, void*, void*, void*, void*, double, long long, int, int, void*);
   (void)a; return ((F)fn)((void*)(uintptr_t)a[0], (void*)(uintptr_t)a[1], (void*)(uintptr_t)a[2], (void*)(uintptr_t)a[3], (void*)(uintptr_t)a[4], (void*)(uintptr_t)a[5], (void*)(uintptr_t)a[6], (void*)(uintptr_t)a[7], ksmi_slot_f64(a[8]), (long long)a[9], (int)(int64_t)a[10], (int)(int64_t)a[11], st);
 }
-static int ksmi_thunk_81(const void* fn, const uint64_t* a, void* st) {
+static int ksmi_thunk_82(const void* fn, const uint64_t* a, void* st) {
   typedef int (*F)(void*, void*, void*, void*, void*, void*, void*, void*, int, double, long long, int, int, void*);
   (void)a; return ((F)fn)((void*)(uintptr_t)a[0], (void*)(uintptr_t)a[1], (void*)(uintptr_t)a[2], (void*)(uintptr_t)a[3], (void*)(uintptr_t)a[4], (void*)(uintptr_t)a[5], (void*)(uintptr_t)a[6], (void*)(uintptr_t)a[7], (int)(int64_t)a[8], ksmi_slot_f64(a[9]), (long long)a[10], (int)(int64_t)a[11], (int)(int64_t)a[12], st);
 }
-static int ksmi_thunk_82(const void* fn, const uint64_t* a, void* st) {
+static int ksmi_thunk_83(const void* fn, const uint64_t* a, void* st) {
   typedef int (*F)(void*, void*, void*, void*, void*, void*, void*, void*, int, int, int, int, void*);
   (void)a; return ((F)fn)((void*)(uintptr_t)a[0], (void*)(uintptr_t)a[1], (void*)(uintptr_t)a[2], (void*)(uintptr_t)a[3], (void*)(uintptr_t)a[4], (void*)(uintptr_t)a[5], (void*)(uintptr_t)a[6], (void*)(uintptr_t)a[7], (int)(int64_t)a[8], (int)(int64_t)a[9], (int)(int64_t)a[10], (int)(int64_t)a[11], st);
 }
-static int ksmi_thunk_83(const void* fn, const uint64_t* a, void* st) {
+static int ksmi_thunk_84(const void* fn, const uint64_t* a, void* st) {
   typedef int (*F)(void*, void*, void*, void*, void*, void*, void*, void*, void*, int, int, void*);
   (void)a; return ((F)fn)((void*)(uintptr_t)a[0], (void*)(uintptr_t)a[1], (void*)(uintptr_t)a[2], (void*)(uintptr_t)a[3], (void*)(uintptr_t)a[4], (void*)(uintptr_t)a[5], (void*)(uintptr_t)a[6], (void*)(uintptr_t)a[7], (void*)(uintptr_t)a[8], (int)(int64_t)a[9], (int)(int64_t)a[10], st);
 }
-static int ksmi_thunk_84(const void* fn, const uint64_t* a, void* st) {
+static int ksmi_thunk_85(const void* fn, const uint64_t* a, void* st) {
   typedef int (*F)(void*, void*, void*, void*, void*, void*, void*, void*, void*, void*, int, int, int, int, int, void*);
   (void)a; return ((F)fn)((void*)(uintptr_t)a[0], (void*)(uintptr_t)a[1], (void*)(uintptr_t)a[2], (void*)(uintptr_t)a[3], (void*)(uintptr_t)a[4], (void*)(uintptr_t)a[5], (void*)(uintptr_t)a[6], (void*)(uintptr_t)a[7], (void*)(uintptr_t)a[8], (void*)(uintptr_t)a[9], (int)(int64_t)a[10], (int)(int64_t)a[11], (int)(int64_t)a[12], (int)(int64_t)a[13], (int)(int64_t)a[14], st);
 }
-static int ksmi_thunk_85(const void* fn, const uint64_t* a, void* st) {
+static int ksmi_thunk_86(const void* fn, const uint64_t* a, void* st) {
   typedef int (*F)(void*, void*, void*, void*, void*, void*, void*, void*, void*, void*, void*, int, int, void*, int, int, int, int, int, int, float, int, void*);
   (void)a; return ((F)fn)((void*)(uintptr_t)a[0], (void*)(uintptr_t)a[1], (void*)(uintptr_t)a[2], (void*)(uintptr_t)a[3], (void*)(uintptr_t)a[4], (void*)(uintptr_t)a[5], (void*)(uintptr_t)a[6], (void*)(uintptr_t)a[7], (void*)(uintptr_t)a[8], (void*)(uintptr_t)a[9], (void*)(uintptr_t)a[10], (int)(int64_t)a[11], (int)(int64_t)a[12], (void*)(uintptr_t)a[13], (int)(int64_t)a[14], (int)(int64_t)a[15], (int)(int64_t)a[16], (int)(int64_t)a[17], (int)(int64_t)a[18], (int)(int64_t)a[19], ksmi_slot_f32(a[20]), (int)(int64_t)a[21], st);
 }
-static int ksmi_thunk_86(const void* fn, const uint64_t* a, void* st) {
+static int ksmi_thunk_87(const void* fn, const uint64_t* a, void* st) {
   typedef int (*F)(void*, void*, void*, void*, void*, void*, void*, void*, void*, void*, void*, void*, void*, void*, void*, void*, void*, void*, int, int, void*);
   (void)a; return ((F)fn)((void*)(uintptr_t)a[0], (void*)(uintptr_t)a[1], (void*)(uintptr_t)a[2], (void*)(uintptr_t)a[3], (void*)(uintptr_t)a[4], (void*)(uintptr_t)a[5], (void*)(uintptr_t)a[6], (void*)(uintptr_t)a[7], (void*)(uintptr_t)a[8], (void*)(uintptr_t)a[9], (void*)(uintptr_t)a[10], (void*)(uintptr_t)a[11], (void*)(uintptr_t)a[12], (void*)(uintptr_t)a[13], (void*)(uintptr_t)a[14], (void*)(uintptr_t)a[15], (void*)(uintptr_t)a[16], (void*)(uintptr_t)a[17], (int)(int64_t)a[18], (int)(int64_t)a[19], st);
 }
-static int ksmi_thunk_87(const void* fn, const uint64_t* a, void* st) {
+static int ksmi_thunk_88(const void* fn, const uint64_t* a, void* st) {
   typedef int (*F)(void*, void*, void*, void*, size_t, int, int, int, int, int, int, int, void*);
   (void)a; return ((F)fn)((void*)(uintptr_t)a[0], (void*)(uintptr_t)a[1], (void*)(uintptr_t)a[2], (void*)(uintptr_t)a[3], (size_t)a[4], (int)(int64_t)a[5], (int)(int64_t)a[6], (int)(int64_t)a[7], (int)(int64_t)a[8], (int)(int64_t)a[9], (int)(int64_t)a[10], (int)(int64_t)a[11], st);
 }
-static int ksmi_thunk_88(const void* fn, const uint64_t* a, void* st) {
+static int ksmi_thunk_89(const void* fn, const uint64_t* a, void* st) {
   typedef int (*F)(void*, size_t, void*);
   (void)a; return ((F)fn)((void*)(uintptr_t)a[0], (size_t)a[1], st);
 }
 
-static const int ksmi_n_thunks = 89;
-static const char* const ksmi_thunk_sigs[] = {"ipppfppiii", "ipppfpppiii", "ipppzp", "p", "pi", "pii", "piiidpppppffipppp", "piiidpppppffppppppppiiii", "piiiipppi", "piiiipppif", "piipppippppppdlii", "piipppipppppppdlii", "piipppipppppppidlii", "pipipiiiii", "pipippipiiii", "plipii", "pp", "ppi", "ppiiidffi", "ppiiii", "ppiiiii", "ppiiiiii", "ppiiiiiiii", "ppiiiiiiiiiiii", "ppiiiiiiiiiiiii", "ppiiili", "ppiiilii", "ppilii", "ppipiiiiipppi", "ppippiiiiii", "ppippppiiiiipppi", "ppl", "ppli", "pplif", "pppfpppli", "pppi", "pppiiiifi", "pppiiiii", "pppiiiiifi", "pppiiiiifufupi", "pppiiiiii", "pppiiiiiii", "pppiiilii", "pppippiii", "pppippiiiii", "pppipppiii", "pppli", "ppplif", "pppliiufuufupi", "ppplpffff", "ppplufupi", "ppppiiii", "ppppiiiii", "ppppiiiiipppfi", "ppppiilf", "ppppiliufupi", "ppppliifi", "pppplpffffff", "pppplpffffffip", "pppppiiii", "pppppiiiii", "pppppiiiiii", "pppppiiiiufupi", "pppppiili", "pppppilii", "ppppplii", "ppppppiifi", "ppppppiiiifi", "ppppppiiiifuffuffuiiiip", "ppppppiiiii", "ppppppiiiiiii", "ppppppilii", "ppppppipiii", "pppppppdlii", "pppppppidlii", "pppppppiiiii", "pppppppiiiiifi", "pppppppiiiiifufupi", "pppppppiiiiiifi", "ppppppppdlifi", "ppppppppdlii", "ppppppppidlii", "ppppppppiiii", "pppppppppii", "ppppppppppiiiii", "pppppppppppiipiiiiiifi", "ppppppppppppppppppii", "ppppziiiiiii", "pz"};
-static const ksmi_thunk_fn ksmi_thunks[] = {ksmi_thunk_0, ksmi_thunk_1, ksmi_thunk_2, ksmi_thunk_3, ksmi_thunk_4, ksmi_thunk_5, ksmi_thunk_6, ksmi_thunk_7, ksmi_thunk_8, ksmi_thunk_9, ksmi_thunk_10, ksmi_thunk_11, ksmi_thunk_12, ksmi_thunk_13, ksmi_thunk_14, ksmi_thunk_15, ksmi_thunk_16, ksmi_thunk_17, ksmi_thunk_18, ksmi_thunk_19, ksmi_thunk_20, ksmi_thunk_21, ksmi_thunk_22, ksmi_thunk_23, ksmi_thunk_24, ksmi_thunk_25, ksmi_thunk_26, ksmi_thunk_27, ksmi_thunk_28, ksmi_thunk_29, ksmi_thunk_30, ksmi_thunk_31, ksmi_thunk_32, ksmi_thunk_33, ksmi_thunk_34, ksmi_thunk_35, ksmi_thunk_36, ksmi_thunk_37, ksmi_thunk_38, ksmi_thunk_39, ksmi_thunk_40, ksmi_thunk_41, ksmi_thunk_42, ksmi_thunk_43, ksmi_thunk_44, ksmi_thunk_45, ksmi_thunk_46, ksmi_thunk_47, ksmi_thunk_48, ksmi_thunk_49, ksmi_thunk_50, ksmi_thunk_51, ksmi_thunk_52, ksmi_thunk_53, ksmi_thunk_54, ksmi_thunk_55, ksmi_thunk_56, ksmi_thunk_57, ksmi_thunk_58, ksmi_thunk_59, ksmi_thunk_60, ksmi_thunk_61, ksmi_thunk_62, ksmi_thunk_63, ksmi_thunk_64, ksmi_thunk_65, ksmi_thunk_66, ksmi_thunk_67, ksmi_thunk_68, ksmi_thunk_69, ksmi_thunk_70, ksmi_thunk_71, ksmi_thunk_72, ksmi_thunk_73, ksmi_thunk_74, ksmi_thunk_75, ksmi_thunk_76, ksmi_thunk_77, ksmi_thunk_78, ksmi_thunk_79, ksmi_thunk_80, ksmi_thunk_81, ksmi_thunk_82, ksmi_thunk_83, ksmi_thunk_84, ksmi_thunk_85, ksmi_thunk_86, ksmi_thunk_87, ksmi_thunk_88};
+static const int ksmi_n_thunks = 90;
+static const char* const ksmi_thunk_sigs[] = {"ipppfppiii", "ipppfpppiii", "ipppzp", "p", "pi", "pii", "piiidpppppffipppp", "piiidpppppffppppppli", "piiidpppppffppppppppiiii", "piiiipppi", "piiiipppif", "piipppippppppdlii", "piipppipppppppdlii", "piipppipppppppidlii", "pipipiiiii", "pipippipiiii", "plipii", "pp", "ppi", "ppiiidffi", "ppiiii", "ppiiiii", "ppiiiiii", "ppiiiiiiii", "ppiiiiiiiiiiii", "ppiiiiiiiiiiiii", "ppiiili", "ppiiilii", "ppilii", "ppipiiiiipppi", "ppippiiiiii", "ppippppiiiiipppi", "ppl", "ppli", "pplif", "pppfpppli", "pppi", "pppiiiifi", "pppiiiii", "pppiiiiifi", "pppiiiiifufupi", "pppiiiiii", "pppiiiiiii", "pppiiilii", "pppippiii", "pppippiiiii", "pppipppiii", "pppli", "ppplif", "pppliiufuufupi", "ppplpffff", "ppplufupi", "ppppiiii", "ppppiiiii", "ppppiiiiipppfi", "ppppiilf", "ppppiliufupi", "ppppliifi", "pppplpffffff", "pppplpffffffip", "pppppiiii", "pppppiiiii", "pppppiiiiii", "pppppiiiiufupi", "pppppiili", "pppppilii", "ppppplii", "ppppppiifi", "ppppppiiiifi", "ppppppiiiifuffuffuiiiip", "ppppppiiiii", "ppppppiiiiiii", "ppppppilii", "ppppppipiii", "pppppppdlii", "pppppppidlii", "pppppppiiiii", "pppppppiiiiifi", "pppppppiiiiifufupi", "pppppppiiiiiifi", "ppppppppdlifi", "ppppppppdlii", "ppppppppidlii", "ppppppppiiii", "pppppppppii", "ppppppppppiiiii", "pppppppppppiipiiiiiifi", "ppppppppppppppppppii", "ppppziiiiiii", "pz"};
+static const ksmi_thunk_fn ksmi_thunks[] = {ksmi_thunk_0, ksmi_thunk_1, ksmi_thunk_2, ksmi_thunk_3, ksmi_thunk_4, ksmi_thunk_5, ksmi_thunk_6, ksmi_thunk_7, ksmi_thunk_8, ksmi_thunk_9, ksmi_thunk_10, ksmi_thunk_11, ksmi_thunk_12, ksmi_thunk_13, ksmi_thunk_14, ksmi_thunk_15, ksmi_thunk_16, ksmi_thunk_17, ksmi_thunk_18, ksmi_thunk_19, ksmi_thunk_20, ksmi_thunk_21, ksmi_thunk_22, ksmi_thunk_23, ksmi_thunk_24, ksmi_thunk_25, ksmi_thunk_26, ksmi_thunk_27, ksmi_thunk_28, ksmi_thunk_29, ksmi_thunk_30, ksmi_thunk_31, ksmi_thunk_32, ksmi_thunk_33, ksmi_thunk_34, ksmi_thunk_35, ksmi_thunk_36, ksmi_thunk_37, ksmi_thunk_38, ksmi_thunk_39, ksmi_thunk_40, ksmi_thunk_41, ksmi_thunk_42, ksmi_thunk_43, ksmi_thunk_44, ksmi_thunk_45, ksmi_thunk_46, ksmi_thunk_47, ksmi_thunk_48, ksmi_thunk_49, ksmi_thunk_50, ksmi_thunk_51, ksmi_thunk_52, ksmi_thunk_53, ksmi_thunk_54, ksmi_thunk_55, ksmi_thunk_56, ksmi_thunk_57, ksmi_thunk_58, ksmi_thunk_59, ksmi_thunk_60, ksmi_thunk_61, ksmi_thunk_62, ksmi_thunk_63, ksmi_thunk_64, ksmi_thunk_65, ksmi_thunk_66, ksmi_thunk_67, ksmi_thunk_68, ksmi_thunk_69, ksmi_thunk_70, ksmi_thunk_71, ksmi_thunk_72, ksmi_thunk_73, ksmi_thunk_74, ksmi_thunk_75, ksmi_thunk_76, ksmi_thunk_77, ksmi_thunk_78, ksmi_thunk_79, ksmi_thunk_80, ksmi_thunk_81, ksmi_thunk_82, ksmi_thunk_83, ksmi_thunk_84, ksmi_thunk_85, ksmi_thunk_86, ksmi_thunk_87, ksmi_thunk_88, ksmi_thunk_89};
diff --git a/kurosiwo_amd/snunet_plan.py b/kurosiwo_amd/snunet_plan.py
--- a/kurosiwo_amd/snunet_plan.py
+++ b/kurosiwo_amd/snunet_plan.py
@@ -17,11 +17,25 @@
     up_gemm = os.environ.get("KSMI_UP_GEMM", "1") != "0"
     up_wgrad64 = os.environ.get("KSMI_UP_WGRAD64", "1") != "0"
     up_wgrad128 = os.environ.get("KSMI_UP_WGRAD128", "1") != "0"
+    bn1_pass = os.environ.get("KSMI_BN1_PASS", "0,2,3,4")
     pack_kind = "pack_weights_batched"
+
+    @staticmethod
+    def _parse_levels(s):
+        s = str(s).strip().lower()
+        if s in ("", "0", "off", "none"):
+            return frozenset()
+        if s == "all":
+            return frozenset(range(5))
+        lv = frozenset(int(t[1:] if t.startswith("l") else t) for t in s.replace(" ", "").split(",") if t)
+        if not lv <= frozenset(range(5)):
+            raise ValueError(f"KSMI_BN1_PASS: levels are 0..4, 'all' or '0' (got {s!r})")
+        return lv
 
     def __init__(self, model, B, H, W, dtype, training, with_backward, tail=0, sync_bn=False):
         self._init_lists(model, dtype, with_backward)
         self.B, self.H, self.W = B, H, W
+        self.bn1_levels = self._parse_levels(self.bn1_pass)
         from . import distributed as _D
         self.sync_bn = bool(sync_bn) and training
         self.bn_world = _D.world_size() if self.sync_bn else 1
@@ -355,9 +369,23 @@
                                                       Bf(f"{bn}.running_mean"), Bf(f"{bn}.running_var"), nbt,
                                                       BN_MOMENTUM, BN_EPS, 1 if training else 0,
                                                       sv.mean, sv.rstd, sv.scale, sv.shift))
-        bn_fin("bn1", sv1, rows1, cpad1)
-
-        src2 = [SrcSpec(i_act.t, Cc, scale=sv1.scale_t, shift=sv1.shift_t, relu=1)]
+        lvl = {self.H >> k: k for k in range(5)}.get(H)
+        if (lvl in self.bn1_levels and training and dtype == torch.bfloat16
+                and bool(self.lib.ksmi_bn_fused_supported(Cc, cpad1, dt))):
+            a_act = Act(f"{name}{branch}.a", B, H, W, Cc, dtype, self.dev)
+            self.keep.append(a_act)
+            nbt1 = m._c(f"{name}.bn1.num_batches_tracked").data_ptr()
+            if self.sync_bn:
+                self.fwd.add_allreduce(lambda: self._bufs[sS][:rows1 * 2 * cpad1 * 4].view(torch.float32))
+            self.fwd.add("ksmi_bn_fin_apply_relu", lambda: (stats(), rows1, cpad1, Cc, gcount, P("bn1.weight"), P("bn1.bias"),
+                                                            Bf("bn1.running_mean"), Bf("bn1.running_var"), nbt1, BN_MOMENTUM, BN_EPS,
+                                                            sv1.mean, sv1.rstd, sv1.scale, sv1.shift, i_act.t.data_ptr(),
+                                                            a_act.t.data_ptr(), npix, dt),
+                         {"kind": "bn_fin_apply_relu", "bytes": npix * Cc * self._es() * 2, "flops": 0})
+            src2 = [SrcSpec(a_act.t, Cc)]
+        else:
+            bn_fin("bn1", sv1, rows1, cpad1)
+            src2 = [SrcSpec(i_act.t, Cc, scale=sv1.scale_t, shift=sv1.shift_t, relu=1)]
         d2, t2 = make_conv(src2, [(z_act.t, Cc, 0, 0, Cc, 0)], z_act.t, m._p(f"{name}.conv2.bias"), None,
                            B, H, W, H, W, 3, 3, 1, 1, Cc, dtype)
         w2 = self._packed(f"{name}.conv2.weight", t2, 9, Cc, Cc, 9, Cc * 9, 0, 1, 0)
```

Result: no change. 2268 tiles/s, median of 3 (+0.3%).
